# DataCTE/SDXL-Training-Improvements

Hardware: AMD Instinct MI355X
Metric: images/sec/node SDXL-base 1024^2 bf16 fwd+bwd (higher is better)
Workload: dtype bf16; 1 GPU; method=ddpm v_prediction + zero_terminal_snr + MinSNR(5), SDXL-base UNet fwd+bwd, batch 4/GPU, 1024^2 (latent 128x128); global_batch=4, parallelism=dp1, weights=synthetic (counter-hash init of the 2,567,463,684-parameter SDXL-base UNet)

## Files before the change

include/sdxlstep_diag.h:

```cpp
#ifndef SDXLSTEP_DIAG_H
#define SDXLSTEP_DIAG_H
#include "sdxlstep.h"
#ifdef __cplusplus
extern "C" {
#endif

SDXL_API int sdxl_probe_layout(void* out_dev, void* stream);
SDXL_API int sdxl_set_gemm_mode(int mode);
SDXL_API int sdxl_debug_act_checksums(sdxl_handle* h, unsigned long long* out_host, int cap, int* n_out, int grads);

SDXL_API int sdxl_op_exchange_shadow(void* buf, size_t bytes, int workgroups, int lds_bytes, float busy_us, void* stream);

SDXL_API int sdxl_op_gemm_ld(int form, const void* A, const void* B, void* C, int M, int N, int K, long lda, long ldb, long ldc, const void* bias,
                    const void* resid, long ldr, int cfg, void* stream);
SDXL_API int sdxl_op_linear_dgrad_delta(const void* dy, const void* w, const void* o, const void* addend, void* d_o, float* delta, int B, int Nq,
                               int N, int K, void* stream);

SDXL_API int sdxl_op_sampler_step(float* x, const void* pred, void* x_in, int B, int H, int W, const sdxl_sampler_step* s, void* stream);

SDXL_API int sdxl_op_cond_dgrad(int n, const void* const* A, const long* lda, const void* const* W, const long* ldb, const int* K, float* C,
                       long ldc, int M, int N, void* stream);

SDXL_API int sdxl_debug_cond_operands(sdxl_handle* h, int which, int g, int* n_groups, size_t* a_ws_byte_off, long* lda, size_t* w_elem_off,
                             long* ldb, int* K);

SDXL_API int sdxl_op_lora_merge(const void* base, const void* A, const void* B, void* w, int out, int in, int rank, float scale, void* stream);
SDXL_API int sdxl_op_lora_project(const float* dw, const void* A, const void* B, float* dA, float* dB, int out, int in, int rank, float scale,
                         void* stream);
SDXL_API int sdxl_op_lora_merge_layout(const void* base, const void* A, const void* B, void* w, int out, int in, int rank, float scale, int kind,
                              int cg, int native_rows, void* stream);
SDXL_API int sdxl_op_lora_project_layout(const float* dw, const void* A, const void* B, float* dA, float* dB, int out, int in, int rank,
                                float scale, int kind, int cg, int native_rows, void* stream);
SDXL_API int sdxl_op_lora_grad(const void* x, long ldx, const void* dy, long ldy, const void* A, const void* B, float* dA, float* dB, int M, int out,
                               int in, int rank, float scale, int accumulate, void* stream);

typedef struct sdxl_gemm_desc {
  int form, taps, M, N, K, splitk, group, cfg, geglu, geglu_group, Hm, Wm, Hs, Ws, sm, sd, up2, emit_bf16, delta, bias_grad;
} sdxl_gemm_desc;
typedef struct sdxl_gemm_route { int kernel, cfg, fast, post; } sdxl_gemm_route;
SDXL_API int sdxl_debug_gemm_route(const sdxl_gemm_desc* problem, sdxl_gemm_route* out);

SDXL_API int sdxl_op_linear_dgrad_ln_bwd(const void* dy, const void* w, const void* x, const float* stats, const void* gamma, const void* addend,
                                void* dx, void* dy_out, float* pcol, int M, int N, int K, void* stream);

SDXL_API int sdxl_set_knob(int id, int value);
SDXL_API int sdxl_set_sk_mode(int mode, int workers);
SDXL_API int sdxl_sk_error(void* stream, unsigned* out);
SDXL_API int sdxl_ln_error(unsigned* out);
SDXL_API int sdxl_op_pl_prefetch_b(int form, const void* B, int M, int N, int K, long ldb, int parts, void* stream);
SDXL_API int sdxl_op_gemm_sk(int n, const int* form, const void* const* A, const void* const* B, void* const* C, const int* M,
                    const int* N, const int* K, const void* const* bias, const void* const* resid, const int* accumulate,
                    void* stream);
SDXL_API int sdxl_op_conv3x3_s2_fwd(const void* x, const void* w, const void* bias, void* xplanar, void* y, int B, int H, int W, int Cin,
                           int Cout, void* stream);
SDXL_API int sdxl_op_conv3x3_s2_wgrad(const void* dy, const void* xplanar, float* dw, float* dbias, int accumulate, int B, int H, int W, int Cin,
                             int Cout, int splitk, void* stream);

#ifdef __cplusplus
}
#endif
#endif
```

sdxl-training-improvements_amd/csrc/attention.hip:

```cpp
#include "attn_tiles.h"

#include <type_traits>

#if defined(ATTN_DIAG) && (ATTN_DIAG & 256)
__device__ unsigned long long g_attn_wg[4096 * 3];
extern "C" __attribute__((visibility("default"))) int sdxl_debug_attn_wg(unsigned long long* out) {
  if (hipDeviceSynchronize() != hipSuccess) return 2;
  return hipMemcpyFromSymbol(out, HIP_SYMBOL(g_attn_wg), sizeof(unsigned long long) * 4096 * 3) == hipSuccess ? 0 : 2;
}
#endif
#if defined(ATTN_DIAG) && (ATTN_DIAG & 128)
__device__ unsigned long long g_attn_stamps[4 * 4 * 6];
extern "C" __attribute__((visibility("default"))) int sdxl_debug_attn_stamps(unsigned long long* out) {
  if (hipDeviceSynchronize() != hipSuccess) return 2;
  return hipMemcpyFromSymbol(out, HIP_SYMBOL(g_attn_stamps), sizeof(unsigned long long) * 96) == hipSuccess ? 0 : 2;
}
#endif
__global__ __launch_bounds__(256, 3) void attn_fwd_kernel(const AttnP p) {
#if defined(ATTN_DIAG) && (ATTN_DIAG & 256)
  const unsigned long long wg_t0 = __builtin_amdgcn_s_memrealtime();
#endif
  __shared__ __attribute__((aligned(16))) bf16 sm[4 * TILE_ELEMS];
  const int tid = threadIdx.x, lane = tid & 63, wave = __builtin_amdgcn_readfirstlane(tid >> 6), l16 = lane & 15, g = lane >> 4;
  int qblk, bh;
// ... 159 lines not shown
    else tile(nfull, std::true_type{}, std::true_type{});
  }
  {
    const bool bad = !(lrow[0] < 1e30f) || !(lrow[1] < 1e30f);
    if (__syncthreads_or(bad ? 1 : 0)) {
#pragma unroll
      for (int i = 0; i < 4; ++i)
#pragma unroll
        for (int j = 0; j < 2; ++j) ot[i][j] = (f32x4){0.f, 0.f, 0.f, 0.f};
      mrow[0] = mrow[1] = 0.f;
      lrow[0] = lrow[1] = 0.f;
      buf = 0;
      tile_dma(ksrc, 0, p.Nk, sm, wave);
      tile_dma(vsrc, 0, p.Nk, sm + TILE_ELEMS, wave);
      for (int t = 0; t < nfull; ++t) tile(t, std::false_type{}, std::false_type{});
      if (nfull < ntiles) tile(nfull, std::true_type{}, std::false_type{});
    }
  }
#if defined(ATTN_DIAG) && (ATTN_DIAG & 128)
  acc_ph[4] = __builtin_amdgcn_s_memrealtime() - rt0;
  if (lane == 0 && qblk < 4 && bh == 5)
    for (int i = 0; i < 6; ++i) g_attn_stamps[(qblk * 4 + wave) * 6 + i] = acc_ph[i];
#endif
#pragma unroll
  for (int qb = 0; qb < 2; ++qb) {
    float l = sum_over_g(lrow[qb]);
    float inv = 1.f / l;
    int q = q0 + qb * 16 + l16;
    if (q < p.Nq) {
      bf16* orow = p.O + ((long)b * p.Nq + q) * p.ldo + h * HD;
#pragma unroll
      for (int db = 0; db < 4; ++db) {
        bf16x4 o;
        o[0] = (bf16)(ot[db][qb][0] * inv); o[1] = (bf16)(ot[db][qb][1] * inv);
        o[2] = (bf16)(ot[db][qb][2] * inv); o[3] = (bf16)(ot[db][qb][3] * inv);
        *(bf16x4*)(orow + db * 16 + g * 4) = o;
      }
      if (g == 0 && p.LSE) p.LSE[(long)bh * p.Nq + q] = mrow[qb] * (1.f / LOG2E) + logf(l);
    }
  }
#if defined(ATTN_DIAG) && (ATTN_DIAG & 256)
  if (threadIdx.x == 0) {
    const int id = blockIdx.x;
    if (id < 4096) {
      unsigned hwid, xcc;
      asm volatile("s_getreg_b32 %0, hwreg(HW_REG_HW_ID)" : "=s"(hwid));
      asm volatile("s_getreg_b32 %0, hwreg(HW_REG_XCC_ID)" : "=s"(xcc));
      g_attn_wg[id * 3] = wg_t0; g_attn_wg[id * 3 + 1] = __builtin_amdgcn_s_memrealtime(); g_attn_wg[id * 3 + 2] = ((unsigned long long)xcc << 32) | hwid;
    }
  }
#endif
}

template <bool WRITE_DELTA>
__device__ __forceinline__ void attn_bwd_dq_body(const AttnP& p, bf16* sm, const int bx, const int bh) {
  const int tid = threadIdx.x, lane = tid & 63, wave = __builtin_amdgcn_readfirstlane(tid >> 6), l16 = lane & 15, g = lane >> 4;
  const int b = bh / p.H, h = bh - b * p.H;
  const int q0 = bx * 128 + wave * 32;
  const bf16* Qb = p.Q + (long)b * p.Nq * p.ldq + h * HD;
  const bf16* dOb = p.dO + (long)b * p.Nq * p.lddo + h * HD;
  const bf16* Ob = p.O + (long)b * p.Nq * p.ldo + h * HD;
  const bf16* Kb = p.K + (long)b * p.Nk * p.ldk + h * HD;
  const bf16* Vb = p.V + (long)b * p.Nk * p.ldv + h * HD;

  bf16x8 qf[2][2], df[2][2];
  float lse2[2], delta[2];
#pragma unroll
  for (int qb = 0; qb < 2; ++qb) {
    int q = q0 + qb * 16 + l16;
    bool ok = q < p.Nq;
    float dl = 0.f;
#pragma unroll
    for (int ks = 0; ks < 2; ++ks) {
      qf[qb][ks] = ok ? *(const bf16x8*)(Qb + (long)q * p.ldq + ks * 32 + g * 8) : z8();
      df[qb][ks] = ok ? *(const bf16x8*)(dOb + (long)q * p.lddo + ks * 32 + g * 8) : z8();
      bf16x8 of = ok ? *(const bf16x8*)(Ob + (long)q * p.ldo + ks * 32 + g * 8) : z8();
#pragma unroll
      for (int e = 0; e < 8; ++e) dl += (float)df[qb][ks][e] * (float)of[e];
    }
    dl = sum_over_g(dl);
    lse2[qb] = ok ? p.LSE[(long)bh * p.Nq + q] * LOG2E : 0.f;
    delta[qb] = dl;
    if (WRITE_DELTA && ok && g == 0) p.Delta[(long)bh * p.Nq + q] = dl;
  }
  f32x4 dq[4][2];
#pragma unroll
  for (int i = 0; i < 4; ++i)
#pragma unroll
    for (int j = 0; j < 2; ++j) dq[i][j] = (f32x4){0.f, 0.f, 0.f, 0.f};
  const float c = SCALE * LOG2E;
#pragma unroll
  for (int qb = 0; qb < 2; ++qb) { qf[qb][0] = scale8(qf[qb][0], c); qf[qb][1] = scale8(qf[qb][1], c); }

  const int ntiles = (p.Nk + 63) / 64;
  const TileSrc ksrc = tile_src(Kb, p.ldk, wave, lane), vsrc = tile_src(Vb, p.ldv, wave, lane);
  tile_dma(ksrc, 0, p.Nk, sm, wave);
  tile_dma(vsrc, 0, p.Nk, sm + TILE_ELEMS, wave);
#pragma unroll
  for (int qb = 0; qb < 2; ++qb) { landed(qf[qb][0]); landed(qf[qb][1]); landed(df[qb][0]); landed(df[qb][1]); landed(lse2[qb]); landed(delta[qb]); }
  int buf = 0;
  auto tile = [&](int t, auto MASKC) {
    constexpr bool MASK = decltype(MASKC)::value;
    asm volatile("s_waitcnt vmcnt(0)" ::: "memory");
    __syncthreads();
    if (t + 1 < ntiles) {
      tile_dma(ksrc, t + 1, p.Nk, sm + ((buf ^ 1) * 2) * TILE_ELEMS, wave);
      tile_dma(vsrc, t + 1, p.Nk, sm + ((buf ^ 1) * 2 + 1) * TILE_ELEMS, wave);
    }
    const bf16* Kt = sm + (buf * 2) * TILE_ELEMS;
    const bf16* Vt = Kt + TILE_ELEMS;
    bf16x8 kf[4][2], vf[4][2];
#pragma unroll
    for (int kb = 0; kb < 4; ++kb) {
      kf[kb][0] = ld_frag(Kt, kb * 16 + l16, g * 8); kf[kb][1] = ld_frag(Kt, kb * 16 + l16, 32 + g * 8);
      vf[kb][0] = ld_frag(Vt, kb * 16 + l16, g * 8); vf[kb][1] = ld_frag(Vt, kb * 16 + l16, 32 + g * 8);
    }
    f32x4 st[4][2], dp[4][2];
#pragma unroll
    for (int kb = 0; kb < 4; ++kb)
#pragma unroll
      for (int qb = 0; qb < 2; ++qb) {
        f32x4 a = (f32x4){-lse2[qb], -lse2[qb], -lse2[qb], -lse2[qb]};
        a = __builtin_amdgcn_mfma_f32_16x16x32_bf16(kf[kb][0], qf[qb][0], a, 0, 0, 0);
        a = __builtin_amdgcn_mfma_f32_16x16x32_bf16(kf[kb][1], qf[qb][1], a, 0, 0, 0);
        st[kb][qb] = a;
        f32x4 d = (f32x4){-delta[qb], -delta[qb], -delta[qb], -delta[qb]};
        d = __builtin_amdgcn_mfma_f32_16x16x32_bf16(vf[kb][0], df[qb][0], d, 0, 0, 0);
        d = __builtin_amdgcn_mfma_f32_16x16x32_bf16(vf[kb][1], df[qb][1], d, 0, 0, 0);
        dp[kb][qb] = d;
      }
    bf16x8 ktr[4][2];
#pragma unroll
    for (int db = 0; db < 4; ++db)
#pragma unroll
      for (int t2 = 0; t2 < 2; ++t2) ktr[db][t2] = tr_frag(Kt, t2, db * 16, l16, g);
    __builtin_amdgcn_sched_barrier(0);
    bf16x8 dsf[2][2];
#pragma unroll
    for (int qb = 0; qb < 2; ++qb) {
#pragma unroll
      for (int kb = 0; kb < 4; ++kb)
#pragma unroll
        for (int hh = 0; hh < 2; ++hh) {
          const f32x2 arg = (f32x2){st[kb][qb][2 * hh], st[kb][qb][2 * hh + 1]};
          f32x2 pr = (f32x2){__builtin_amdgcn_exp2f(arg[0]), __builtin_amdgcn_exp2f(arg[1])};
          if (MASK) {
            if (t * 64 + kb * 16 + g * 4 + 2 * hh >= p.Nk) pr[0] = 0.f;
            if (t * 64 + kb * 16 + g * 4 + 2 * hh + 1 >= p.Nk) pr[1] = 0.f;
          }
          const f32x2 ds = pr * (f32x2){dp[kb][qb][2 * hh], dp[kb][qb][2 * hh + 1]};
          st[kb][qb][2 * hh] = ds[0]; st[kb][qb][2 * hh + 1] = ds[1];
        }
      dsf[0][qb] = pack8(st[0][qb], st[1][qb]);
      dsf[1][qb] = pack8(st[2][qb], st[3][qb]);
    }
    __builtin_amdgcn_sched_barrier(0);
#pragma unroll
    for (int db = 0; db < 4; ++db)
#pragma unroll
      for (int t2 = 0; t2 < 2; ++t2)
#pragma unroll
        for (int qb = 0; qb < 2; ++qb)
          dq[db][qb] = __builtin_amdgcn_mfma_f32_16x16x32_bf16(ktr[db][t2], dsf[t2][qb], dq[db][qb], 0, 0, 0);
    buf ^= 1;
  };
  const int nfull = p.Nk / 64;
  for (int t = 0; t < nfull; ++t) tile(t, std::false_type{});
  if (nfull < ntiles) tile(nfull, std::true_type{});
#pragma unroll
  for (int qb = 0; qb < 2; ++qb) {
    int q = q0 + qb * 16 + l16;
    if (q < p.Nq) {
      bf16* row = p.dQ + ((long)b * p.Nq + q) * p.lddq + h * HD;
#pragma unroll
      for (int db = 0; db < 4; ++db) {
        bf16x4 o;
        o[0] = (bf16)(dq[db][qb][0] * SCALE); o[1] = (bf16)(dq[db][qb][1] * SCALE);
        o[2] = (bf16)(dq[db][qb][2] * SCALE); o[3] = (bf16)(dq[db][qb][3] * SCALE);
        *(bf16x4*)(row + db * 16 + g * 4) = o;
      }
    }
  }
}

__global__ __launch_bounds__(256, 2) void attn_bwd_dq_kernel(const AttnP p) {
  set_wave_prio(p.prio);
  __shared__ __attribute__((aligned(16))) bf16 sm[4 * TILE_ELEMS];
  int qblk, bh;
  attn_xcd_map(p, blockIdx.x, (p.Nq + 127) >> 7, qblk, bh);
  attn_bwd_dq_body<true>(p, sm, qblk, bh);
}

template <int KB>
__device__ __forceinline__ void attn_bwd_dkv_body(const AttnP& p, bf16* sm, const int bx, const int bh, const int bz, const int nbh) {
  float (*sstat)[2][64] = (float (*)[2][64])(sm + 4 * TILE_ELEMS);
  const int tid = threadIdx.x, lane = tid & 63, wave = __builtin_amdgcn_readfirstlane(tid >> 6), l16 = lane & 15, g = lane >> 4;
  const int b = bh / p.H, h = bh - b * p.H;
  const int key0 = bx * (64 * KB) + wave * (16 * KB) + l16;
  const bf16* Qb = p.Q + (long)b * p.Nq * p.ldq + h * HD;
  const bf16* dOb = p.dO + (long)b * p.Nq * p.lddo + h * HD;
  const bf16* Kb = p.K + (long)b * p.Nk * p.ldk + h * HD;
  const bf16* Vb = p.V + (long)b * p.Nk * p.ldv + h * HD;
  bool kok[KB];
  bf16x8 kf[KB][2], vf[KB][2];
#pragma unroll
  for (int kb = 0; kb < KB; ++kb) {
    const int key = key0 + kb * 16;
    kok[kb] = key < p.Nk;
#pragma unroll
    for (int ks = 0; ks < 2; ++ks) {
      kf[kb][ks] = kok[kb] ? scale8(*(const bf16x8*)(Kb + (long)key * p.ldk + ks * 32 + g * 8), SCALE * LOG2E) : z8();
      vf[kb][ks] = kok[kb] ? *(const bf16x8*)(Vb + (long)key * p.ldv + ks * 32 + g * 8) : z8();
    }
  }
  f32x4 dk[KB][4], dv[KB][4];
#pragma unroll
  for (int kb = 0; kb < KB; ++kb)
#pragma unroll
    for (int i = 0; i < 4; ++i) { dk[kb][i] = (f32x4){0.f, 0.f, 0.f, 0.f}; dv[kb][i] = (f32x4){0.f, 0.f, 0.f, 0.f}; }

  const int ntiles_all = (p.Nq + 63) / 64;
  const int per = (ntiles_all + p.qsplit - 1) / p.qsplit;
  const int t_begin = bz * per;
  const int ntiles = min(ntiles_all, t_begin + per);
  auto load_stats = [&](int t, int bufi) {
    if (wave < 2) {
      const int q = t * 64 + lane;
      const float* src = (wave == 0 ? p.LSE : p.Delta) + (long)bh * p.Nq + q;
      lds_dma4_global(q < p.Nq ? (const void*)src : (const void*)g_attn_zero16, lds_addr_of(&sstat[bufi][wave][0]));
    }
  };
  const TileSrc qsrc = tile_src(Qb, p.ldq, wave, lane), dsrc = tile_src(dOb, p.lddo, wave, lane);
  tile_dma(qsrc, t_begin, p.Nq, sm, wave);
  tile_dma(dsrc, t_begin, p.Nq, sm + TILE_ELEMS, wave);
  load_stats(t_begin, 0);
#pragma unroll
  for (int kb = 0; kb < KB; ++kb) { landed(kf[kb][0]); landed(kf[kb][1]); landed(vf[kb][0]); landed(vf[kb][1]); }
  int buf = 0;
  auto tile = [&](int t, auto MASKC) {
    constexpr bool MASK = decltype(MASKC)::value;
    const bool more = t + 1 < ntiles;
    asm volatile("s_waitcnt vmcnt(0)" ::: "memory");
    __syncthreads();
// ... 188 lines not shown
  o[0] = (bf16)a[0]; o[1] = (bf16)a[1]; o[2] = (bf16)a[2]; o[3] = (bf16)a[3];
  bf16* dst = which == 0 ? p.dK + ((long)b * p.Nk + key) * p.lddk + h * HD : p.dV + ((long)b * p.Nk + key) * p.lddv + h * HD;
  *(bf16x4*)(dst + v4 * 4) = o;
}

size_t attn_part_floats(int B, int H, int Nk, int qsplit) {
  return qsplit > 1 ? (size_t)qsplit * B * H * ((Nk + 63) / 64) * 64 * 2 * 64 : 0;
}
int attn_pick_qsplit(int B, int H, int Nq, int Nk) {
  long blocks = (long)((Nk + 63) / 64) * B * H;
  int qt = (Nq + 63) / 64;
  int s = (int)((KNOB(36) > 0 ? KNOB(36) : 160) / blocks);
  if (s < 1) s = 1;
  if (s > qt / 2) s = qt / 2 > 0 ? qt / 2 : 1;
  if (s > 16) s = 16;
  return s;
}

static int check_attn(const AttnP& p) {
  ARG_CHECK(p.B > 0 && p.H > 0 && p.Nq > 0 && p.Nk > 0, "attention: empty problem");
  ARG_CHECK(p.ldq % 8 == 0 && p.ldk % 8 == 0 && p.ldv % 8 == 0 && p.ldo % 4 == 0,
            "attention: row strides must be multiples of 8 elements");
  return 0;
}

int launch_attn_fwd(const AttnP& p, hipStream_t st) {
  if (int e = check_attn(p)) return e;
#ifdef SDXL_DIAG
  if (KNOB(33) == 2 && attn_fwd_pl_applicable(p)) return launch_attn_fwd_pl(p, st);
#endif
  return launch_attn_fwd_tiled(p, st);
}
int launch_attn_fwd_tiled(const AttnP& p, hipStream_t st) {
  if (int e = check_attn(p)) return e;
  if (FILE* f = launch_log()) { fprintf(f, "A,0,%d,%d,%d,%d\n", p.B, p.H, p.Nq, p.Nk); fflush(f); }
  AttnP q = p;
  q.xcd = (p.B * p.H) % 8 == 0 && KNOB(32) != 1;
  hipLaunchKernelGGL(attn_fwd_kernel, dim3(cdiv(p.Nq, 128) * p.B * p.H), dim3(256), 0, st, q);
  HIP_CHECK_RET(hipGetLastError());
  return 0;
}

static int check_attn_bwd(const AttnP& p) {
  if (int e = check_attn(p)) return e;
  ARG_CHECK(p.O && p.dO && p.dQ && p.dK && p.dV && p.LSE && p.Delta, "attention bwd: missing buffers");
  ARG_CHECK(!p.accumulate, "attention bwd: accumulate not implemented");
  return 0;
}
int launch_attn_bwd_dq(const AttnP& p, hipStream_t st) {
  if (int e = check_attn_bwd(p)) return e;
  if (FILE* f = launch_log()) { fprintf(f, "A,1,%d,%d,%d,%d\n", p.B, p.H, p.Nq, p.Nk); fflush(f); }
  AttnP q = p;
  q.xcd = (p.B * p.H) % 8 == 0 && KNOB(32) != 1;
  hipLaunchKernelGGL(attn_bwd_dq_kernel, dim3(cdiv(p.Nq, 128) * p.B * p.H), dim3(256), 0, st, q);
  HIP_CHECK_RET(hipGetLastError());
  return 0;
}
int launch_attn_bwd_dkv(const AttnP& p, hipStream_t st) {
  if (int e = check_attn_bwd(p)) return e;
  if (FILE* f = launch_log()) { fprintf(f, "A,2,%d,%d,%d,%d\n", p.B, p.H, p.Nq, p.Nk); fflush(f); }
  AttnP q = p;
  if (q.qsplit < 1 || !q.part) q.qsplit = 1;
  if (q.qsplit == 1 && (long)cdiv(p.Nk, 128) * p.B * p.H >= 1024)
    hipLaunchKernelGGL(attn_bwd_dkv_kernel<2>, dim3(cdiv(p.Nk, 128), p.B * p.H, 1), dim3(256), 0, st, q);
  else
    hipLaunchKernelGGL(attn_bwd_dkv_kernel<1>, dim3(cdiv(p.Nk, 64), p.B * p.H, q.qsplit), dim3(256), 0, st, q);
  if (q.qsplit > 1) {
    long total = (long)p.B * p.H * p.Nk * 32;
    hipLaunchKernelGGL(attn_dkv_reduce_kernel, dim3(cdiv(total, 256)), dim3(256), 0, st, q);
  }
  HIP_CHECK_RET(hipGetLastError());
  return 0;
}
int launch_attn_bwd_fused(const AttnP& p, hipStream_t st) {
  if (int e = check_attn_bwd(p)) return e;
  ARG_CHECK(p.lddo % 8 == 0 && p.ldo % 8 == 0, "attention bwd (fused): dO / O row strides must be multiples of 8 elements");
  if (FILE* f = launch_log()) { fprintf(f, "A,1,%d,%d,%d,%d\nA,2,%d,%d,%d,%d\n", p.B, p.H, p.Nq, p.Nk, p.B, p.H, p.Nq, p.Nk); fflush(f); }
  AttnP q = p;
  q.qsplit = 1;
  q.xcd = (p.B * p.H) % 8 == 0 && KNOB(32) != 1;
  const long total = (long)p.B * p.Nq * p.H;
  if (!p.delta_ready) hipLaunchKernelGGL(attn_delta_kernel, dim3(cdiv(total, 32)), dim3(256), 0, st, q);
  if (KNOB(35) != 1 && ((p.Nq >= 2048 && p.Nk >= 2048) || KNOB(35) == 2) && attn_bwd_pl_applicable(q)) return launch_attn_bwd_pl(q, st);
  const int nkb = cdiv(p.Nk, 128), nqb = cdiv(p.Nq, 128), nbh = p.B * p.H;
  hipLaunchKernelGGL(attn_bwd_fused_kernel<2>, dim3(nkb * nbh + nqb * nbh), dim3(256), 0, st, q, nkb * nbh, nkb, nqb);
  HIP_CHECK_RET(hipGetLastError());
  return 0;
}
int launch_attn_bwd(const AttnP& p, hipStream_t st) {
  const bool fused = (KNOB(20) != 1 || p.delta_ready) && (p.qsplit <= 1 || !p.part) && p.Nk >= 256 && p.lddo % 8 == 0 && p.ldo % 8 == 0;
  if (fused) return launch_attn_bwd_fused(p, st);
  if (int e = launch_attn_bwd_dq(p, st)) return e;
  return launch_attn_bwd_dkv(p, st);
}
```

sdxl-training-improvements_amd/csrc/capi.hip:

```cpp
#include "capi.h"
#include <functional>

extern "C" {

const char* sdxl_last_error(void) { return sdxl_get_error(); }
int sdxl_version(void) { return 1; }

int sdxl_default_config(sdxl_unet_config* c) {
  ARG_CHECK(c, "null config");
  c->in_channels = 4; c->out_channels = 4;
  c->block_out_channels[0] = 320; c->block_out_channels[1] = 640; c->block_out_channels[2] = 1280;
  c->layers_per_block = 2;
  c->transformer_layers[0] = 0; c->transformer_layers[1] = 2; c->transformer_layers[2] = 10;
  c->head_dim = 64; c->cross_attention_dim = 2048; c->norm_num_groups = 32;
  c->addition_time_embed_dim = 256; c->pooled_dim = 1280;
  c->resnet_eps = 1e-5f; c->tf_gn_eps = 1e-6f; c->ln_eps = 1e-5f;
  return 0;
}

int sdxl_create(const sdxl_unet_config* cfg, int device, sdxl_handle** out) {
  ARG_CHECK(cfg && out, "null argument");
  ARG_CHECK(cfg->head_dim == 64, "head_dim must be 64 (got %d)", cfg->head_dim);
  ARG_CHECK(cfg->in_channels == 4 && cfg->out_channels == 4, "in/out channels must be 4");
  ARG_CHECK(cfg->transformer_layers[0] == 0, "level 0 must not have attention");
  for (int i = 0; i < 3; ++i) {
    int c = cfg->block_out_channels[i];
    ARG_CHECK(c % cfg->norm_num_groups == 0 && c % 8 == 0, "block_out_channels[%d]=%d unsupported", i, c);
    if (cfg->transformer_layers[i] > 0) ARG_CHECK(c % 128 == 0, "attention level width %d must be a multiple of 128", c);
  }
  ARG_CHECK(cfg->cross_attention_dim % 8 == 0 && cfg->pooled_dim % 8 == 0 && cfg->addition_time_embed_dim % 8 == 0,
            "conditioning widths must be multiples of 8");
  int ndev = 0;
  HIP_CHECK_RET(hipGetDeviceCount(&ndev));
  ARG_CHECK(device >= 0 && device < ndev, "device %d out of range (have %d)", device, ndev);
  HIP_CHECK_RET(hipSetDevice(device));
  sdxl_handle* h = new sdxl_handle();
  h->e.cfg = *cfg;
  h->e.device = device;
  h->e.build(nullptr);
  const char* ns = getenv("SDXL_NO_SIDE_STREAM");
  h->e.use_side = !(ns && ns[0] == '1');
  if (h->e.use_side) {
    if (const char* sp = getenv("SDXL_SIDE_PRIO")) {
      HIP_CHECK_RET(hipStreamCreateWithPriority(&h->e.side, hipStreamNonBlocking, atoi(sp)));
    } else
    HIP_CHECK_RET(hipStreamCreateWithFlags(&h->e.side, hipStreamNonBlocking));
    HIP_CHECK_RET(hipStreamCreateWithFlags(&h->e.gstream, hipStreamNonBlocking));
    HIP_CHECK_RET(hipEventCreateWithFlags(&h->e.ev_gin, hipEventDisableTiming));
    HIP_CHECK_RET(hipEventCreateWithFlags(&h->e.ev_gout, hipEventDisableTiming));
    HIP_CHECK_RET(hipEventCreateWithFlags(&h->e.ev_join, hipEventDisableTiming | hipEventDisableSystemFence));
    HIP_CHECK_RET(hipEventCreateWithFlags(&h->e.ev_seg, hipEventDisableTiming | hipEventDisableSystemFence));
    HIP_CHECK_RET(hipEventCreateWithFlags(&h->e.ev_hoist, hipEventDisableTiming | hipEventDisableSystemFence));
  }
  *out = h;
  return 0;
}

int sdxl_destroy(sdxl_handle* h) {
  if (!h) return 0;
  if (h->e.own_weights && h->e.weights) (void)hipFree(h->e.weights);
  if (h->e.own_grads && h->e.grads) (void)hipFree(h->e.grads);
  if (h->e.own_ws && h->e.ws) (void)hipFree(h->e.ws);
  h->e.clear_graphs();
  if (h->e.gstream) (void)hipStreamDestroy(h->e.gstream);
  if (h->e.ev_gin) (void)hipEventDestroy(h->e.ev_gin);
  if (h->e.ev_gout) (void)hipEventDestroy(h->e.ev_gout);
  for (hipEvent_t ev : h->e.ev_pool) (void)hipEventDestroy(ev);
  if (h->e.ev_join) (void)hipEventDestroy(h->e.ev_join);
  if (h->e.ev_seg) (void)hipEventDestroy(h->e.ev_seg);
  if (h->e.ev_hoist) (void)hipEventDestroy(h->e.ev_hoist);
  if (h->e.side) (void)hipStreamDestroy(h->e.side);
  if (h->e.small_ranges_dev) (void)hipFree(h->e.small_ranges_dev);
  if (h->lora.dev) (void)hipFree(h->lora.dev);
  if (h->e.lora.dev) (void)hipFree(h->e.lora.dev);
  delete h;
  return 0;
}

int sdxl_param_bytes(sdxl_handle* h, size_t* wb, size_t* gb) {
  H_CHECK(h);
  if (wb) *wb = h->e.param_elems * sizeof(bf16);
  if (gb) *gb = h->e.param_elems * sizeof(float);
  return 0;
}

int sdxl_bind_params(sdxl_handle* h, void* w, void* g) {
  H_CHECK(h);
  Engine& e = h->e;
  e.clear_graphs();
  if (w) { e.weights = (bf16*)w; e.own_weights = false; }
  else {
    HIP_CHECK_RET(hipMalloc((void**)&e.weights, e.param_elems * sizeof(bf16)));
    HIP_CHECK_RET(hipMemset(e.weights, 0, e.param_elems * sizeof(bf16)));
    e.own_weights = true;
  }
  if (g) { e.grads = (float*)g; e.own_grads = false; }
  else {
    HIP_CHECK_RET(hipMalloc((void**)&e.grads, e.param_elems * sizeof(float)));
    HIP_CHECK_RET(hipMemset(e.grads, 0, e.param_elems * sizeof(float)));
    e.own_grads = true;
  }
  ARG_CHECK(((uintptr_t)e.weights & 255) == 0 && ((uintptr_t)e.grads & 255) == 0, "arenas must be 256-byte aligned");
  return 0;
}

int sdxl_num_params(sdxl_handle* h) { return h ? (int)h->e.src.size() : -1; }

int sdxl_param_info(sdxl_handle* h, int i, char* name, int cap, int* ndim, long shape[4]) {
  H_CHECK(h);
  ARG_CHECK(i >= 0 && i < (int)h->e.src.size(), "parameter index %d out of range", i);
  const SrcParam& s = h->e.src[i];
  if (name && cap > 0) snprintf(name, cap, "%s", s.name.c_str());
  if (ndim) *ndim = s.ndim;
  if (shape) for (int k = 0; k < 4; ++k) shape[k] = s.shape[k];
  return 0;
}

int sdxl_param_range(sdxl_handle* h, int i, size_t* elem_off, size_t* elems) {
  H_CHECK(h);
  ARG_CHECK(i >= 0 && i < (int)h->e.src.size(), "parameter index %d out of range", i);
  const SrcParam& s = h->e.src[i];
  size_t n = 1;
  for (int k = 0; k < s.ndim; ++k) n *= (size_t)s.shape[k];
// ... 455 lines not shown
    CHK(launch_loss_prepare(L, s));
    CHK(run_forward_ops(e, s));
    CHK(launch_loss_fwd(L, s));
    return 0;
  }));
  if (b->per_sample_loss)
    HIP_CHECK_RET(hipMemcpyAsync(b->per_sample_loss, p.F(p.ps_loss_off), sizeof(float) * p.B, hipMemcpyDeviceToDevice, st));
  h->step.lc = full; h->step.b = sb; h->step.valid = true;
  h->step.d_ehs = d_ehs; h->step.d_pool = d_pool;
  h->step.awaiting_bwd = true;
  return 0;
}

int sdxl_num_segments(sdxl_handle* h) { return h ? h->e.nseg : -1; }
int sdxl_set_join_mode(sdxl_handle* h, int mode) {
  H_CHECK(h);
  ARG_CHECK(mode >= 0 && mode <= 2, "join mode %d (0, 1, 2)", mode);
  h->e.join_last_only = mode != 0;
  h->e.seg_on_side = mode == 2 && h->e.use_side && h->e.side;
  return 0;
}
int sdxl_side_stream(sdxl_handle* h, void** stream) {
  H_CHECK(h);
  ARG_CHECK(stream, "null output");
  *stream = h->e.use_side ? (void*)h->e.side : nullptr;
  return 0;
}

int sdxl_segment_range(sdxl_handle* h, int k, size_t* off, size_t* n) {
  H_CHECK(h);
  ARG_CHECK(k >= 0 && k < h->e.nseg, "segment %d out of range", k);
  int s = h->e.nseg - 1 - k;
  if (off) *off = h->e.seg_begin[s];
  if (n) *n = h->e.seg_end[s] - h->e.seg_begin[s];
  return 0;
}

static int run_backward_segment_body(Engine& e, int k, bool first, hipStream_t st);
static int run_backward_segment(Engine& e, int k, bool first, hipStream_t st) {
  if (k == 0) e.drop_pending();
  const int rc = run_backward_segment_body(e, k, first, st);
  if (rc) e.drop_pending();
  return rc;
}
static int run_backward_segment_body(Engine& e, int k, bool first, hipStream_t st) {
  Plan& p = *e.cur;
  int s = e.nseg - 1 - k;
  e.ev_used = 0;
  if (k == 0 && p.tp32_off != NONE) HIP_CHECK_RET(hipMemsetAsync(p.F(p.tp32_off), 0, p.tp32_bytes, st));
  if (k == 0 && p.ln_part_floats) {
    HIP_CHECK_RET(hipMemsetAsync(p.F(p.ln_part_off), 0, p.ln_part_floats * sizeof(float), st));
    p.ln_epoch = 0;
  }
  for (int i = p.seg_last_op[s]; i >= p.seg_first_op[s] && i >= 0; --i) CHK(p.ops[i]->bwd(p, st, first));
  CHK(e.flush_wgrads(p, st));
  CHK(e.flush_ln_params(p, st));
  ARG_CHECK(k != e.nseg - 1 || e.cs_pending.empty(), "backward: %zu per-sample column sums were never reduced", e.cs_pending.size());
  if (e.seg_on_side && !gemm_profiling()) {
    HIP_CHECK_RET(hipEventRecord(e.ev_seg, st));
    HIP_CHECK_RET(hipStreamWaitEvent(e.side, e.ev_seg, 0));
    e.side_dirty = true;
  }
  if (e.side_dirty && !(e.join_last_only && k != e.nseg - 1)) {
    HIP_CHECK_RET(hipEventRecord(e.ev_join, e.side));
    HIP_CHECK_RET(hipStreamWaitEvent(st, e.ev_join, 0));
    e.side_dirty = false;
  }
  if (k == e.nseg - 1 && (e.cond_ehs || e.cond_pool)) CHK(e.launch_cond_grads(p, st));
  return 0;
}

int sdxl_backward_segment(sdxl_handle* h, int k, float grad_scale, int first_micro, void* stp) {
  H_CHECK(h);
  Engine& e = h->e;
  hipStream_t st = (hipStream_t)stp;
  CHK(ready(e));
  ARG_CHECK(k >= 0 && k < e.nseg, "segment %d out of range", k);
  if (k == 0) ARG_CHECK(h->step.valid, "sdxl_backward_segment(0) needs a preceding sdxl_forward_loss");
  set_cond_request(h, true);
  auto body = [&](hipStream_t s) -> int {
    if (k == 0) {
      LossP L;
      fill_loss(e, &h->step.lc, &h->step.b, grad_scale, L);
      CHK(launch_loss_bwd(L, s));
    }
    return run_backward_segment(e, k, first_micro != 0, s);
  };
  if (e.join_last_only) {
    CHK(body(st));
  } else {
    unsigned sbits;
    memcpy(&sbits, &grad_scale, 4);
    Engine::GraphKey key{e.cur, 1, k, first_micro != 0, 0, sbits, loss_cfg_bits(h->step.lc, h->step.b.tag_weights != nullptr),
                        loss_cfg_bits2(h->step.lc, h->step.b) | cond_bits(h->step), loss_huber_bits(h->step.lc, h->step.b)};
    CHK(run_graphed(e, key, st, body));
  }
  if (k == e.nseg - 1) h->step.awaiting_bwd = false;
  return k == e.nseg - 1 ? copy_cond_grads(h, st) : 0;
}

int sdxl_backward_all(sdxl_handle* h, float grad_scale, int first_micro, void* stp) {
  H_CHECK(h);
  Engine& e = h->e;
  hipStream_t st = (hipStream_t)stp;
  CHK(ready(e));
  ARG_CHECK(h->step.valid, "sdxl_backward_all needs a preceding sdxl_forward_loss");
// ... 220 lines not shown
```

sdxl-training-improvements_amd/csrc/engine.h:

```cpp
#pragma once
#include <functional>
#include <map>
#include <memory>
#include <set>
#include <string>
#include <tuple>
#include <vector>

#include "../../include/sdxlstep.h"
#include "kernels.h"

static const size_t NONE = (size_t)-1;

struct Act {
  size_t off = NONE;
  size_t goff = NONE;
  long rows = 0;
  int cols = 0;
  int pad_rows = 0;
  bool need_grad = true;
  Act* parent = nullptr;
  int col0 = 0;
  long ld() const { return parent ? parent->cols : cols; }
};

struct PRef {
  size_t off = NONE;
  size_t numel = 0;
};

struct SrcParam {
  std::string name;
  int ndim;
  long shape[4];
  PRef native;
  int kind;
  size_t elem_off;
  int ci_pad;
};

struct Engine;
struct Plan;

struct Op {
  int seg = 0;
  bool hoist_fwd = false;
  bool needs_hoisted = false;
  virtual ~Op() {}
  virtual int fwd(Plan& p, hipStream_t st) = 0;
  virtual void plan_bwd(Plan& p) = 0;
  virtual int bwd(Plan& p, hipStream_t st, bool first_micro) = 0;
};

struct Plan {
  Engine* eng = nullptr;
  int B = 0, H = 0, W = 0, ctx = 0;
  size_t ws_bytes = 0;
  size_t cursor = 0;
  std::vector<std::unique_ptr<Act>> acts;
  std::vector<std::unique_ptr<Op>> ops;
  std::vector<int> seg_first_op, seg_last_op;
  size_t tp32_off = NONE, tp32_bytes = 0;
  Act *x_in = nullptr, *pred = nullptr, *ehs = nullptr, *aug_in = nullptr, *te_sin = nullptr, *tid_emb = nullptr;
  size_t t_off = NONE, tid_off = NONE, loss_off = NONE, loss_part_off = NONE;
  size_t in_lat_off = NONE, in_noise_off = NONE, in_sig_off = NONE, in_tag_off = NONE;
  size_t in_sw_off = NONE, in_hc_off = NONE;
  size_t ps_loss_off = NONE;
  size_t in_mask_off = NONE, in_nin_off = NONE;
  size_t mask_norm_off = NONE;
  size_t samp_part_off = NONE;
  size_t gn_ws_off = NONE, gn_ws_floats = 0;
  size_t slab_off = NONE, slab_floats = 0;
  size_t slab_main_off = NONE, slab_main_floats = 0;
  size_t apart_off = NONE, apart_floats = 0;
  size_t apart_side_off = NONE, apart_side_floats = 0;
  size_t ln_part_off = NONE, ln_part_floats = 0;
  int ln_epoch = 0;
  struct CondSrc { size_t dy_off = NONE; long lda = 0; PRef w; long ldb = 0; int K = 0; };
  CondSrc cond_kv[2], cond_add;
  int cond_nkv = 0;
  size_t dehs_off = NONE, dpool_off = NONE, cond_slab_off = NONE;
  size_t lg_tu_elems = 0, lg_part_floats = 0, lg_tu_off = NONE, lg_part_off = NONE;

  Act* new_act(long rows, int cols, bool need_grad = true, int pad_rows = 0);
  Act* view(Act* parent, int col0, int cols);
  size_t alloc(size_t bytes);
  struct GradDst { size_t out = NONE, addend = NONE; };
  GradDst grad_dst(Act* a);
  bool grad_alias(Act* x, Act* y);
  bf16* GP(size_t off) const;
  template <class T, class... A>
  T* add(A&&... a);
  bf16* P(const Act* a) const;
  bf16* G(const Act* a) const;
  float* F(size_t off) const;
};

struct Engine {
  sdxl_unet_config cfg;
  int device = 0;
  std::vector<PRef> natives;
  std::vector<SrcParam> src;
  std::map<std::string, int> src_index;
  size_t param_elems = 0;
  bf16* weights = nullptr;
  float* grads = nullptr;
  bool own_weights = false, own_grads = false;
  int nseg = 1;
  std::vector<size_t> seg_begin, seg_end;
  std::map<std::tuple<int, int, int, int>, std::unique_ptr<Plan>> plans;
  Plan* cur = nullptr;
  char* ws = nullptr;
  size_t ws_cap = 0;
  bool own_ws = false;
  hipStream_t side = nullptr;
  hipEvent_t ev_join = nullptr, ev_hoist = nullptr;
  std::vector<hipEvent_t> ev_pool;
  size_t ev_used = 0;
  bool use_side = true;
  bf16* emit_base = nullptr;
  float emit_scale = 1.f;
  bool join_last_only = false;
  bool seg_on_side = false;
  hipEvent_t ev_seg = nullptr;
  hipEvent_t next_event();
  std::vector<std::vector<GemmP>> wg_pending;
  int defer_wgrad(Plan& p, hipStream_t main, const GemmP& g, int grp);
  int flush_wgrads(Plan& p, hipStream_t main);
  std::vector<std::function<int(hipStream_t)>> side_leaves;
  std::vector<LnRedEntry> ln_pending;
  std::vector<LnRedEntry> cs_pending;
  int flush_ln_params(Plan& p, hipStream_t main);
  void drop_pending() { side_leaves.clear(); wg_pending.clear(); ln_pending.clear(); cs_pending.clear(); }
  bool side_dirty = false;
  bool cond_ehs = false, cond_pool = false;
  bool cond_gated = false;
  int launch_cond_grads(Plan& p, hipStream_t st);
  struct LoraOpSel { std::vector<LoraGradTarget> host; const LoraGradTarget* dev = nullptr; int tiles = 0, reds = 0; size_t part_unit = 0; };
  struct LoraSel {
    std::vector<int> params;
    int rank = 0; float scale = 0.f;
    const bf16* adapters = nullptr; float* grads = nullptr;
    std::map<size_t, LoraOpSel> ops;
    LoraGradTarget* dev = nullptr;
  } lora;
  const LoraOpSel* lora_op(PRef w) const {
    if (lora.ops.empty()) return nullptr;
    auto it = lora.ops.find(w.off);
    return it == lora.ops.end() ? nullptr : &it->second;
  }
  std::vector<unsigned char> trainable;
  std::set<size_t> frozen_offs;
  void set_trainable(const unsigned char* flags);
  bool frozen(PRef a, PRef b) const {
    if (frozen_offs.empty()) return false;
    return (a.off == NONE || frozen_offs.count(a.off)) && (b.off == NONE || frozen_offs.count(b.off));
  }
  bool use_graphs = false;
  hipStream_t gstream = nullptr;
  hipEvent_t ev_gin = nullptr, ev_gout = nullptr;
  struct GraphKey {
    const void* plan; int kind, k, first, join; unsigned scale_bits, cfg;
    unsigned cfg2, huber_bits;
    bool operator<(const GraphKey& o) const {
      return std::tie(plan, kind, k, first, join, scale_bits, cfg, cfg2, huber_bits) <
             std::tie(o.plan, o.kind, o.k, o.first, o.join, o.scale_bits, o.cfg, o.cfg2, o.huber_bits);
    }
  };
  struct GraphEntry { hipGraphExec_t exec = nullptr; int seen = 0; };
  std::map<GraphKey, GraphEntry> graphs;
  void clear_graphs() {
    for (auto& kv : graphs) if (kv.second.exec) (void)hipGraphExecDestroy(kv.second.exec);
    graphs.clear();
  }
  bool registering = true;
  size_t native_cursor = 0;
  Plan* bp = nullptr;

  PRef param(size_t numel, bool small = false);
  std::vector<std::pair<size_t, size_t>> small_ranges;
  unsigned long long* small_ranges_dev = nullptr;
  void map_src(const std::string& name, std::vector<long> shape, PRef p, int kind, size_t elem_off, int ci_pad);
  int seg_of(size_t elem_off) const;
  void build(Plan* plan);
  bf16* Wp(PRef p) const { return weights + p.off; }
// ... 18 lines not shown
```

sdxl-training-improvements_amd/csrc/engine.hip:

```cpp
#include "engine.h"

#include <stdarg.h>
#include <stdlib.h>

#ifdef SDXL_DIAG
int g_knobs[SDXL_NKNOBS] = {0};
#endif
static thread_local char g_err[1024] = "";
void sdxl_set_error(const char* fmt, ...) {
  va_list ap;
  va_start(ap, fmt);
  vsnprintf(g_err, sizeof(g_err), fmt, ap);
  va_end(ap);
}
const char* sdxl_get_error() { return g_err; }

#define CHK(x)            \
  do {                    \
    int _r = (x);         \
    if (_r) return _r;    \
  } while (0)

static inline size_t align_up(size_t v, size_t a) { return (v + a - 1) / a * a; }

// ... 56 lines not shown
  HIP_CHECK_RET(hipStreamWaitEvent(e.side, ev, 0));
  e.side_dirty = true;
  if (!e.side_leaves.empty()) {
    std::vector<std::function<int(hipStream_t)>> v;
    v.swap(e.side_leaves);
    for (auto& leaf : v) CHK(leaf(e.side));
  }
  return fn(e.side);
}
template <class F>
static int side_leaf(Plan& p, hipStream_t main, F&& fn) {
  Engine& e = *p.eng;
  if (!e.use_side || !e.side || gemm_profiling() || KNOB(2) == 16) return on_side(p, main, fn);
  e.side_leaves.emplace_back(std::function<int(hipStream_t)>(fn));
  return 0;
}
static int launch_wgrad_bucket(Plan& p, hipStream_t main, std::vector<GemmP>& v) {
  if (v.empty()) return 0;
  GemmP g = v[0];
  if (v.size() > 1) {
    g.splitk = 1;
    gemm_fill_group(g, v.data(), (int)v.size());
  }
  v.clear();
  if (g.splitk > 1) g.anyorder = 0;
  return on_side(p, main, [&g](hipStream_t s2) -> int { return launch_gemm(g, s2); });
}
int Engine::defer_wgrad(Plan& p, hipStream_t main, const GemmP& g, int grp) {
  for (auto& b : wg_pending) {
    if (b.empty() || (b[0].M == g.M && b[0].N == g.N && b[0].K == g.K && b[0].accumulate == g.accumulate)) {
      b.push_back(g);
      if ((int)b.size() >= grp) return launch_wgrad_bucket(p, main, b);
      return 0;
    }
  }
  wg_pending.emplace_back(1, g);
  if (grp <= 1) return launch_wgrad_bucket(p, main, wg_pending.back());
  return 0;
}
int Engine::flush_wgrads(Plan& p, hipStream_t main) {
  if (!side_leaves.empty()) CHK(on_side(p, main, [](hipStream_t) -> int { return 0; }));
  for (auto& b : wg_pending) CHK(launch_wgrad_bucket(p, main, b));
  return 0;
}
int Engine::flush_ln_params(Plan& p, hipStream_t main) {
  size_t i = 0;
  while (i < ln_pending.size()) {
    LnRedBatch b;
    b.n = 0;
    while (i < ln_pending.size() && b.n < LN_RED_MAX) b.e[b.n++] = ln_pending[i++];
    CHK(on_side(p, main, [&b](hipStream_t s2) -> int { return launch_ln_param_reduce(b, s2); }));
  }
  ln_pending.clear();
  return 0;
}
int Engine::launch_cond_grads(Plan& p, hipStream_t st) {
  const float* gate = cond_gated ? p.F(p.loss_off) + 7 : nullptr;
  if (cond_ehs) {
    const int M = p.B * p.ctx, N = cfg.cross_attention_dim;
    if (p.cond_nkv == 0) {
      HIP_CHECK_RET(hipMemsetAsync(p.F(p.dehs_off), 0, sizeof(float) * (size_t)M * N, st));
    } else {
      CondDgradP q;
      memset(&q, 0, sizeof(q));
      q.n = p.cond_nkv;
      for (int g = 0; g < q.n; ++g) {
        const Plan::CondSrc& cs = p.cond_kv[g];
        ARG_CHECK(cs.dy_off != NONE, "conditioning gradients: the K | V projection has no output gradient");
        q.A[g] = p.GP(cs.dy_off); q.lda[g] = cs.lda; q.W[g] = Wp(cs.w); q.ldb[g] = cs.ldb; q.K[g] = cs.K;
      }
      q.C = p.F(p.dehs_off); q.ldc = N; q.M = M; q.N = N; q.slab = p.F(p.cond_slab_off); q.gate = gate;
      CHK(launch_cond_dgrad(q, st));
    }
  }
  if (cond_pool) {
    const Plan::CondSrc& cs = p.cond_add;
    ARG_CHECK(cs.dy_off != NONE, "conditioning gradients: add_embedding.linear_1 has no output gradient");
    CondDgradP q;
    memset(&q, 0, sizeof(q));
    q.n = 1;
    q.A[0] = p.GP(cs.dy_off); q.lda[0] = cs.lda; q.W[0] = Wp(cs.w); q.ldb[0] = cs.ldb; q.K[0] = cs.K;
    q.C = p.F(p.dpool_off); q.ldc = cfg.pooled_dim; q.M = p.B; q.N = cfg.pooled_dim; q.slab = p.F(p.cond_slab_off); q.gate = gate;
    CHK(launch_cond_dgrad(q, st));
  }
  return 0;
}
bool Plan::grad_alias(Act* x, Act* y) {
  if (x->goff == NONE) {
    x->goff = y->goff;
    return true;
  }
  return false;
}

static void want_slab_main(Plan& p, int M, int N, int splitk) {
  size_t need = gemm_slab_floats(M, N, 1, splitk);
  if (need > p.slab_main_floats) p.slab_main_floats = need;
}
static void want_slab(Plan& p, int M, int N, int taps, int splitk) {
  size_t need = gemm_slab_floats(M, N, taps, splitk);
  if (need > p.slab_floats) p.slab_floats = need;
}

struct WgradDst {
  float *C, *bias_grad;
  int accumulate;
  bf16* Cb;
  float cb_scale;
  void to(GemmP& g) const {
    g.C = C; g.bias_grad = bias_grad; g.accumulate = accumulate;
    if (Cb) { g.Cb = Cb; g.cb_scale = cb_scale; }
  }
};
static WgradDst wgrad_dst(Plan& p, PRef w, PRef b, bool first) {
  const Engine& e = *p.eng;
  return {e.Gp(w), b.off != NONE ? e.Gp(b) : nullptr, first ? 0 : 1, e.emit_base ? e.emit_base + w.off : nullptr, e.emit_scale};
}

static int kv_pad_rows(int B, int ctx) { return (int)((64 - ((long)B * ctx) % 64) % 64); }

struct AttnOp;
static void attn_delta_target(AttnOp* a, Plan& p, GemmP& g);
static bool attn_delta_wanted(const AttnOp* a);
static void attn_set_delta_fused(AttnOp* a, bool on);
struct LayerNormOp;
static bool ln_fuse_plan(LayerNormOp* ln, Plan& p, int mode);
static void ln_fuse_target(LayerNormOp* ln, Plan& p, GemmP& g, int mode);
struct LinearOp : Op {
  Act *x, *y, *resid;
  PRef w, b;
  int K, N;
  int resid_alias = 0, splitk = 1, wgroup = 1;
  struct AttnOp* delta_attn = nullptr;
  bool delta_on = false;
  struct LayerNormOp* ln_src = nullptr;
  int ln_mode = 0;
  int crcfg = 0, crsplit = 1;
  int fsplit = 1, dsplit = 1;
  size_t dy32_off = NONE;
  size_t dy_off = NONE;
  Plan::GradDst dx, dres;
  int ggroup = 64;
  Act* gact = nullptr;
  Act* gu = nullptr;
  LinearOp(Act* x_, Act* y_, PRef w_, PRef b_, int K_, int N_, Act* resid_) : x(x_), y(y_), resid(resid_), w(w_), b(b_), K(K_), N(N_) {}
  int fwd(Plan& p, hipStream_t st) override {
    GemmP g = linear_fwd_problem(p.P(x), x->ld(), p.eng->Wp(w), p.P(y), y->ld(), (int)x->rows, N, K, b.off == NONE ? nullptr : p.eng->Wp(b),
                                 resid ? p.P(resid) : nullptr, resid ? resid->ld() : 0);
    if (gact) gemm_attach_geglu_fwd(g, ggroup, p.P(gact), gact->ld());
    if (fsplit > 1 && !hoist_fwd) { g.splitk = fsplit; g.slab = p.F(p.slab_main_off); }
    return launch_gemm(g, st);
  }
  void plan_bwd(Plan& p) override {
    dy_off = y->goff;
    if (resid) {
      resid_alias = p.grad_alias(resid, y) ? 1 : 0;
      if (!resid_alias) dres = p.grad_dst(resid);
    }
    if (gu) dx = p.grad_dst(gu);
    else if (x->need_grad) dx = p.grad_dst(x);
    splitk = linear_wgrad_splitk(N, K, x->rows);
    wgroup = gemm_pick_group(N, K, 1, x->rows, splitk);
    want_slab(p, N, K, 1, splitk);
    crcfg = cr256_wgrad_cfg(N, K, x->rows, b.off != NONE);
    if (crcfg) { crsplit = cr256_pick_splitk(N, K, x->rows, crcfg); want_slab(p, N, K, 1, crsplit); }
    if (!gact) { fsplit = gemm_pick_splitk_small((int)x->rows, N, K, 3); want_slab_main(p, (int)x->rows, N, fsplit); }
    if (const Engine::LoraOpSel* lo = p.eng->lora_op(w)) {
      const size_t tu = lora_grad_tu_elems((int)lo->host.size(), p.eng->lora.rank, (int)x->rows);
      const size_t pf = (size_t)lora_grad_chunks((int)x->rows) * lo->part_unit;
      if (tu > p.lg_tu_elems) p.lg_tu_elems = tu;
      if (pf > p.lg_part_floats) p.lg_part_floats = pf;
    }
    if (delta_attn && !(!gu && x->need_grad)) attn_set_delta_fused(delta_attn, false);
    if (!gu && x->need_grad) {
      dsplit = gemm_pick_splitk_small((int)x->rows, K, N, 2);
      if (KNOB(3) > 1 && N >= (KNOB(4) > 0 ? KNOB(4) : 8192) && N % (64 * KNOB(3)) == 0 && dsplit == 1) dsplit = KNOB(3);
      want_slab_main(p, (int)x->rows, K, dsplit);
      if (delta_attn) {
        delta_on = attn_delta_wanted(delta_attn) && dsplit <= 1 && K % 128 == 0;
        attn_set_delta_fused(delta_attn, delta_on);
      }
      if (SDXL_LN_EPILOGUE && ln_src && KNOB(26) != 0 && dsplit == 1 && dx.addend == NONE && !x->parent && gemm_ln_cfg((int)x->rows, K, N) &&
          ln_fuse_plan(ln_src, p, KNOB(26) == 2 ? 2 : 1))
        ln_mode = KNOB(26) == 2 ? 2 : 1;
    }
  }
  int bwd(Plan& p, hipStream_t st, bool first) override {
    const bf16* dy = p.GP(dy_off);
    const int M = (int)x->rows;
    if (dy32_off != NONE) {
      auto& cs = p.eng->cs_pending;
      for (size_t i = 0; i < cs.size();) {
        LnRedBatch rb;
        rb.n = 0;
        while (i < cs.size() && rb.n < LN_RED_MAX) rb.e[rb.n++] = cs[i++];
        CHK(launch_ln_param_reduce(rb, st));
      }
      cs.clear();
      CHK(launch_f32_to_bf16(p.F(dy32_off), p.GP(dy_off), (long)M * N, 1.f, st));
    }
    if (gu && dx.addend != NONE) { sdxl_set_error("geglu: pre-activation gradient has another writer"); return 3; }
    if (resid && !resid_alias) CHK(launch_add(p.GP(dres.addend), dy, p.GP(dres.out), (long)M * N, st));
    if (const Engine::LoraOpSel* lo = p.eng->lora_op(w)) {
      const Engine::LoraSel& L = p.eng->lora;
      LoraGradP q;
      memset(&q, 0, sizeof(q));
      q.table = lo->dev; q.n = (int)lo->host.size(); q.rank = L.rank; q.scale = L.scale; q.accumulate = first ? 0 : 1;
      q.x = p.P(x); q.ldx = x->ld(); q.dy = dy; q.ldy = y->ld();
      q.M = M; q.Mp = lora_grad_mp(M); q.nchunk = lora_grad_chunks(M); q.tiles = lo->tiles; q.reds = lo->reds;
      q.xvec = ((uintptr_t)q.x % 16 == 0 && q.ldx % 8 == 0) ? 1 : 0;
      q.yvec = ((uintptr_t)q.dy % 16 == 0 && q.ldy % 8 == 0) ? 1 : 0;
      q.a = q.b = L.adapters; q.ga = q.gb = L.grads;
      if (p.lg_tu_off == NONE || p.lg_part_off == NONE) { sdxl_set_error("lora: the plan was built without adapter-gradient scratch"); return 3; }
      q.tu = (bf16*)p.F(p.lg_tu_off); q.part = p.F(p.lg_part_off);
      CHK(on_side(p, st, [&q](hipStream_t s2) -> int { return launch_lora_grad(q, s2); }));
    } else
    if (!p.eng->frozen(w, b)) {
      GemmP g = linear_wgrad_problem(dy, y->ld(), p.P(x), x->ld(), nullptr, N, K, M, nullptr);
      wgrad_dst(p, w, b, first).to(g);
      g.splitk = splitk;
      g.slab = p.F(p.slab_off);
      if (crcfg) { g.cfg = crcfg; if (wgroup <= 1) g.splitk = crsplit; }
      if (KNOB(29) == 1 && M >= 1024 && dy32_off == NONE && (g.splitk <= 1 || wgroup > 1)) g.anyorder = 1;
      const int pad = x->pad_rows < y->pad_rows ? x->pad_rows : y->pad_rows;
      if (pad > 0 && (M + pad) % 64 == 0) {
        g.K = M + pad;
        g.anyorder = 0;
        bf16* dyp = p.GP(dy_off) + (size_t)M * N;
        bf16* xp = p.P(x) + (size_t)M * K;
        const size_t nb_dy = (size_t)pad * N * sizeof(bf16), nb_x = (size_t)pad * K * sizeof(bf16);
        CHK(on_side(p, st, [=](hipStream_t s2) -> int {
          HIP_CHECK_RET(hipMemsetAsync(dyp, 0, nb_dy, s2));
          HIP_CHECK_RET(hipMemsetAsync(xp, 0, nb_x, s2));
          return launch_gemm(g, s2);
        }));
      } else
      if (wgroup > 1) CHK(p.eng->defer_wgrad(p, st, g, wgroup));
      else CHK(on_side(p, st, [&](hipStream_t s2) -> int { return launch_gemm(g, s2); }));
    }
    if (x->need_grad) {
      GemmP g = linear_dgrad_problem(dy, y->ld(), p.eng->Wp(w), p.GP(dx.out), x->ld(), M, K, N, !gu && dx.addend != NONE ? p.GP(dx.addend) : nullptr, x->ld());
      if (gu) gemm_attach_geglu_bwd(g, ggroup, p.P(gu), gu->ld());
      if (dsplit > 1) { g.splitk = dsplit; g.slab = p.F(p.slab_main_off); }
      g.prio = KNOB(0);
      if (KNOB(6) > 0 && !gu && (KNOB(8) <= 0 || N >= KNOB(8))) g.cfg = KNOB(6);
      if (KNOB(22) > 0 && gu) g.cfg = KNOB(22);
      if (delta_on) attn_delta_target(delta_attn, p, g);
      if (ln_mode) ln_fuse_target(ln_src, p, g, ln_mode);
      CHK(launch_gemm(g, st));
    }
    return 0;
  }
};

struct ConvOp : Op {
  Act *x, *y, *resid, *rowvec;
  PRef w, b;
  int Bn, H, W, Cin, Cout, stride, Ho, Wo;
  int resid_alias = 0, splitk = 1;
  int fsplit = 1, dsplit = 1;
  size_t rv32_off = NONE;
  long rv32_ld = 0;
  size_t cs_part_off = NONE;
  size_t dy_off = NONE;
  Plan::GradDst dx, dres, drv;
  Act* x_low = nullptr;
  Plan::GradDst* up_dx = nullptr;
  size_t weff_off = NONE, planar_off = NONE, dweff_off = NONE;
  size_t s2x_off = NONE;
  size_t s2_planar_off = NONE;
  int up_fs = 1, up_ds = 1, up_ws = 1;
  bool up_wg = false;
  bool up2() const { return x_low != nullptr && KNOB(2) != 64; }
  void enable_up2(Plan& p, Act* xl, Plan::GradDst* udx) {
    if (stride != 1 || Cin % 64 || Cout % 64 || resid || rowvec) return;
    x_low = xl; up_dx = udx;
    const long plane = upconv_plane_rows(Bn, H / 2, W / 2);
    weff_off = p.alloc(sizeof(bf16) * (size_t)Cout * 16 * Cin);
    planar_off = p.alloc(sizeof(bf16) * (size_t)4 * plane * (Cout > Cin ? Cout : Cin));
    up_fs = upconv3x3_fwd_splitk(Bn, H / 2, W / 2, Cin, Cout);
    want_slab_main(p, (int)(4 * plane), Cout, up_fs);
    up_ds = upconv3x3_dgrad_splitk(Bn, H / 2, W / 2, Cin, Cout);
    want_slab_main(p, Bn * (H / 2) * (W / 2), Cin, up_ds);
    up_wg = (Bn * (H / 2) * (W / 2)) % 64 == 0;
    if (up_wg) {
      dweff_off = p.alloc(sizeof(float) * (size_t)Cout * 16 * Cin);
      up_ws = gemm_pick_splitk(Cout, Cin, 16, (long)Bn * (H / 2) * (W / 2));
      want_slab(p, Cout, Cin, 16, up_ws);
      cs_part_off = p.alloc(sizeof(float) * colsum_part_floats(1, Bn * H * W, Cout));
    }
  }
  ConvOp(Act* x_, Act* y_, PRef w_, PRef b_, int B_, int H_, int W_, int Cin_, int Cout_, int stride_, Act* resid_,
         Act* rowvec_)
      : x(x_), y(y_), resid(resid_), rowvec(rowvec_), w(w_), b(b_), Bn(B_), H(H_), W(W_), Cin(Cin_), Cout(Cout_),
        stride(stride_) {
    Ho = (H - 1) / stride + 1;
    Wo = (W - 1) / stride + 1;
  }
  int fwd(Plan& p, hipStream_t st) override {
#ifdef SDXL_DIAG
    if (s2x_off != NONE && KNOB(2) == 512)
// ... 85 lines not shown
      GemmP g = conv3x3_dgrad_problem(Bn, H, W, Cin, Cout, stride);
      g.A = dy; g.B = p.eng->Wp(w); g.C = p.GP(dx.out);
      if (dx.addend != NONE) { g.resid = p.GP(dx.addend); g.ldr = Cin; }
      if (dsplit > 1) { g.splitk = dsplit; g.slab = p.F(p.slab_main_off); }
      g.prio = KNOB(0);
      if (KNOB(7) > 0) g.cfg = KNOB(7);
      CHK(launch_gemm(g, st));
    }
    return 0;
  }
};

struct GroupNormOp : Op {
  Act *x, *y;
  PRef gm, bt;
  int Bn, HW, C, G, silu;
  float eps;
  size_t stats_off, prow_off;
  size_t dy_off = NONE;
  Plan::GradDst dx;
  GroupNormOp(Plan& p, Act* x_, Act* y_, PRef g_, PRef b_, int B_, int HW_, int C_, int G_, float eps_, int silu_)
      : x(x_), y(y_), gm(g_), bt(b_), Bn(B_), HW(HW_), C(C_), G(G_), silu(silu_), eps(eps_) {
    stats_off = p.alloc(sizeof(float) * Bn * G * 2);
    prow_off = p.alloc(sizeof(float) * Bn * 2 * C);
    size_t need = groupnorm_ws_floats(Bn, C, G);
    if (need > p.gn_ws_floats) p.gn_ws_floats = need;
  }
  int fwd(Plan& p, hipStream_t st) override {
    if (KNOB(27) & 2) return 0;
    if (KNOB(27) & 128) return launch_silu_fwd(p.P(x), p.P(y), (long)Bn * HW * C, st);
    return launch_groupnorm_fwd(p.P(x), p.P(y), p.eng->Wp(gm), p.eng->Wp(bt), p.F(stats_off), p.F(p.gn_ws_off), Bn, HW, C, G,
                                eps, silu, st);
  }
  void plan_bwd(Plan& p) override { dy_off = y->goff; dx = p.grad_dst(x); }
  int bwd(Plan& p, hipStream_t st, bool) override {
    if (KNOB(27) & 1) return 0;
    LnRedEntry r;
    r.part = p.F(prow_off); r.dgamma = p.eng->Gp(gm); r.dbeta = p.eng->Gp(bt); r.C = C; r.nblk = Bn;
    if (!p.eng->frozen(gm, bt)) p.eng->ln_pending.push_back(r);
    return launch_groupnorm_bwd(p.P(x), p.GP(dy_off), p.eng->Wp(gm), p.eng->Wp(bt), p.F(stats_off), p.GP(dx.out),
                                p.GP(dx.addend), p.eng->Gp(gm), p.eng->Gp(bt), p.F(p.gn_ws_off), Bn, HW, C, G, silu, st, p.F(prow_off));
  }
};

struct LayerNormOp : Op {
  Act *x, *y;
  PRef gm, bt;
  int C;
  float eps;
  size_t stats_off, part_off = NONE;
  size_t dy_off = NONE;
  Plan::GradDst dx;
  int fused = 0;
  LayerNormOp(Plan& p, Act* x_, Act* y_, PRef g_, PRef b_, int C_, float eps_) : x(x_), y(y_), gm(g_), bt(b_), C(C_), eps(eps_) {
    stats_off = p.alloc(sizeof(float) * x->rows * 2);
  }
  int fwd(Plan& p, hipStream_t st) override {
    if (KNOB(27) & 4) return 0;
    if (KNOB(27) & 256) return launch_silu_fwd(p.P(x), p.P(y), (long)x->rows * C, st);
    return launch_layernorm_fwd(p.P(x), p.P(y), p.eng->Wp(gm), p.eng->Wp(bt), p.F(stats_off), (int)x->rows, C, eps, st);
  }
  void plan_bwd(Plan& p) override {
    dy_off = y->goff;
    dx = p.grad_dst(x);
    part_off = p.alloc(sizeof(float) * layernorm_bwd_part_floats((int)x->rows, C));
  }
  int bwd(Plan& p, hipStream_t st, bool) override {
    const bool frozen = p.eng->frozen(gm, bt);
    if (fused) {
      if (frozen) return 0;
      if (fused == 2) {
        const bf16* xp = p.P(x); const bf16* dyp = p.GP(dy_off); const float* sp = p.F(stats_off);
        float* dg = p.eng->Gp(gm); float* db = p.eng->Gp(bt); const int Mr = (int)x->rows, Cc = C;
        return side_leaf(p, st, [=](hipStream_t s2) -> int { return launch_layernorm_param_grads(xp, dyp, sp, dg, db, Mr, Cc, s2); });
      }
      LnRedEntry r;
      r.part = p.F(part_off); r.dgamma = p.eng->Gp(gm); r.dbeta = p.eng->Gp(bt); r.C = C; r.nblk = gemm_ln_rowblocks((int)x->rows);
      p.eng->ln_pending.push_back(r);
      return 0;
    }
    if (KNOB(25) == 2) return 0;
    if (KNOB(10) == 1 || KNOB(10) == 3) {
      if (KNOB(25) != 3)
      CHK(launch_layernorm_bwd(p.P(x), p.GP(dy_off), p.eng->Wp(gm), p.F(stats_off), p.GP(dx.out), p.GP(dx.addend), nullptr, nullptr, (int)x->rows, C, st));
      const bf16* xp = p.P(x); const bf16* dyp = p.GP(dy_off); const float* sp = p.F(stats_off);
      const int Mr = (int)x->rows, Cc = C;
      if (KNOB(25) == 1 || frozen) return 0;
      if (KNOB(10) == 3) {
        float* dg = p.eng->Gp(gm); float* db = p.eng->Gp(bt);
        return side_leaf(p, st, [=](hipStream_t s2) -> int { return launch_layernorm_param_grads(xp, dyp, sp, dg, db, Mr, Cc, s2); });
      }
      float* part = p.F(part_off);
      LnRedEntry r;
      r.part = part; r.dgamma = p.eng->Gp(gm); r.dbeta = p.eng->Gp(bt); r.C = C; r.nblk = layernorm_param_partial_rows(Mr, Cc);
      p.eng->ln_pending.push_back(r);
      return side_leaf(p, st, [=](hipStream_t s2) -> int { return launch_layernorm_param_partials(xp, dyp, sp, part, Mr, Cc, s2); });
    }
    LnRedEntry r;
    r.part = p.F(part_off); r.dgamma = p.eng->Gp(gm); r.dbeta = p.eng->Gp(bt); r.C = C;
    CHK(launch_layernorm_bwd(p.P(x), p.GP(dy_off), p.eng->Wp(gm), p.F(stats_off), p.GP(dx.out), p.GP(dx.addend),
                             p.F(part_off), &r.nblk, (int)x->rows, C, st));
    if (!frozen) p.eng->ln_pending.push_back(r);
    return 0;
  }
};

static bool ln_fuse_plan(LayerNormOp* ln, Plan& p, int mode) {
  const int M = (int)ln->x->rows, C = ln->C;
  if (ln->x->ld() != C || ln->y->ld() != C) return false;
  if (gemm_ln_pcol_floats(M, C) > layernorm_bwd_part_floats(M, C)) return false;
  ln->fused = mode;
  const size_t pf = gemm_ln_part_floats(M, C);
  if (pf > p.ln_part_floats) p.ln_part_floats = pf;
  return true;
}
static void ln_fuse_target(LayerNormOp* ln, Plan& p, GemmP& g, int mode) {
  gemm_attach_ln_bwd(g, p.P(ln->x), ln->x->ld(), p.F(ln->stats_off), p.eng->Wp(ln->gm), p.GP(ln->dx.out), p.GP(ln->dx.addend), p.F(p.ln_part_off),
                     ++p.ln_epoch, mode == 1 ? p.F(ln->part_off) : nullptr);
  if (mode == 1) g.C = nullptr;
}

struct AttnOp : Op {
  Act *q, *kv, *o;
  int Bn, heads, Nq, Nk, C;
  bool self;
  int qsplit = 1;
  size_t lse_off, delta_off;
  AttnOp(Plan& p, Act* q_, Act* kv_, Act* o_, int B_, int heads_, int Nq_, int Nk_, int C_, bool self_)
      : q(q_), kv(kv_), o(o_), Bn(B_), heads(heads_), Nq(Nq_), Nk(Nk_), C(C_), self(self_) {
    lse_off = p.alloc(sizeof(float) * (size_t)Bn * heads * Nq);
    delta_off = p.alloc(sizeof(float) * (size_t)Bn * heads * Nq);
    qsplit = attn_pick_qsplit(Bn, heads, Nq, Nk);
    size_t need = attn_part_floats(Bn, heads, Nk, qsplit);
    if (self) { if (need > p.apart_floats) p.apart_floats = need; }
    else if (need > p.apart_side_floats) p.apart_side_floats = need;
  }
  void fill(Plan& p, AttnP& a, bool grads) {
    memset(&a, 0, sizeof(a));
    a.B = Bn; a.H = heads; a.Nq = Nq; a.Nk = Nk;
    if (self) {
      a.Q = p.P(q); a.K = p.P(q) + C; a.V = p.P(q) + 2 * C;
      a.ldq = a.ldk = a.ldv = 3L * C;
    } else {
      a.Q = p.P(q); a.ldq = C;
      a.K = p.P(kv); a.V = p.P(kv) + C; a.ldk = a.ldv = kv->ld();
    }
    a.O = p.P(o); a.ldo = o->ld();
    a.LSE = p.F(lse_off);
    if (grads) {
      a.dO = p.GP(do_off); a.lddo = o->ld();
      a.Delta = p.F(delta_off);
      a.qsplit = qsplit;
      a.part = p.F(self ? p.apart_off : p.apart_side_off);
      if (self) {
        a.dQ = p.GP(dq.out); a.dK = a.dQ + C; a.dV = a.dQ + 2 * C;
        a.lddq = a.lddk = a.lddv = 3L * C;
      } else {
        a.dQ = p.GP(dq.out); a.lddq = C;
        a.dK = p.GP(dkv.out); a.dV = a.dK + C; a.lddk = a.lddv = kv->ld();
      }
    }
  }
  int fwd(Plan& p, hipStream_t st) override {
    if (KNOB(27) & (self ? 32 : 64)) return 0;
    AttnP a;
    fill(p, a, false);
    return launch_attn_fwd(a, st);
  }
  bool bad = false;
  size_t do_off = NONE;
  Plan::GradDst dq, dkv;
  void plan_bwd(Plan& p) override {
    do_off = o->goff;
    dq = p.grad_dst(q);
    if (dq.addend != NONE) bad = true;
    if (!self) { dkv = p.grad_dst(kv); if (dkv.addend != NONE) bad = true; }
  }
  bool delta_fused = false;
  int bwd(Plan& p, hipStream_t st, bool) override {
    if (bad) { sdxl_set_error("attention: operand gradient has another writer"); return 3; }
    if (KNOB(27) & (self ? 16 : 8)) return 0;
    AttnP a;
    fill(p, a, true);
    a.prio = KNOB(1);
    a.delta_ready = delta_fused ? 1 : 0;
    if (self) return launch_attn_bwd(a, st);
    CHK(launch_attn_bwd_dq(a, st));
    return side_leaf(p, st, [=](hipStream_t s2) -> int { return launch_attn_bwd_dkv(a, s2); });
  }
};

static bool attn_delta_wanted(const AttnOp* a) { return a->self && a->qsplit <= 1 && a->Nk >= 256 && a->C % 128 == 0 && a->delta_fused; }
static void attn_set_delta_fused(AttnOp* a, bool on) { a->delta_fused = on; }
static void attn_delta_target(AttnOp* a, Plan& p, GemmP& g) {
  gemm_attach_delta(g, p.P(a->o), a->o->ld(), p.F(a->delta_off), a->Nq, a->heads);
}

struct SiluOp : Op {
  Act *x, *y;
  size_t dy_off = NONE;
  Plan::GradDst dx;
  SiluOp(Act* x_, Act* y_) : x(x_), y(y_) {}
  int fwd(Plan& p, hipStream_t st) override { return launch_silu_fwd(p.P(x), p.P(y), x->rows * x->cols, st); }
  void plan_bwd(Plan& p) override { dy_off = y->goff; dx = p.grad_dst(x); }
  int bwd(Plan& p, hipStream_t st, bool) override {
    return launch_silu_bwd(p.P(x), p.GP(dy_off), p.GP(dx.out), p.GP(dx.addend), x->rows * x->cols, st);
  }
};

struct ConcatOp : Op {
  Act *a, *b, *o;
  size_t do_off = NONE;
  Plan::GradDst da, db;
  ConcatOp(Act* a_, Act* b_, Act* o_) : a(a_), b(b_), o(o_) {}
  int fwd(Plan& p, hipStream_t st) override { return launch_concat(p.P(a), a->cols, p.P(b), b->cols, p.P(o), a->rows, st); }
  void plan_bwd(Plan& p) override { do_off = o->goff; da = p.grad_dst(a); db = p.grad_dst(b); }
  int bwd(Plan& p, hipStream_t st, bool) override {
    return launch_split_add(p.GP(do_off), p.GP(da.out), a->cols, p.GP(da.addend), p.GP(db.out), b->cols, p.GP(db.addend),
                            a->rows, st);
  }
};

struct UpsampleOp : Op {
  Act *x, *y;
  int Bn, H, W, C;
  size_t dy_off = NONE;
  Plan::GradDst dx;
  ConvOp* fused = nullptr;
  UpsampleOp(Act* x_, Act* y_, int B_, int H_, int W_, int C_) : x(x_), y(y_), Bn(B_), H(H_), W(W_), C(C_) {}
  int fwd(Plan& p, hipStream_t st) override {
    if (fused && fused->up2() && fused->up_wg && KNOB(2) != 128) return 0;
    if (fused && fused->up2() && !p.eng->use_graphs) {
      const bf16* xp = p.P(x); bf16* yp = p.P(y);
      const int b = Bn, h = H, w = W, c = C;
      return on_side(p, st, [=](hipStream_t s2) -> int { return launch_upsample2x(xp, yp, b, h, w, c, s2); });
    }
    return launch_upsample2x(p.P(x), p.P(y), Bn, H, W, C, st);
  }
  void plan_bwd(Plan& p) override { dy_off = y->goff; dx = p.grad_dst(x); }
  int bwd(Plan& p, hipStream_t st, bool) override {
    if (fused && fused->up2() && y->need_grad) return 0;
    return launch_upsample2x_bwd(p.GP(dy_off), p.GP(dx.out), p.GP(dx.addend), Bn, H, W, C, st);
  }
};

struct EmbedInOp : Op {
// ... 134 lines not shown
    Act* y = pl->new_act((long)B * ho * wo, cout);
    tagseg(pl->add<ConvOp>(x, y, w, b, B, h, w_, cin, cout, stride, resid, rowvec), w);
    return y;
  }
  Act* groupnorm(const std::string& name, Act* x, int hw, int C, float eps, int silu) {
    PRef g = e.param(C, true);
    e.map_src(name + ".weight", {C}, g, 0, 0, 0);
    PRef b = e.param(C, true);
    e.map_src(name + ".bias", {C}, b, 0, 0, 0);
    if (!pl) return nullptr;
    Act* y = pl->new_act(x->rows, C);
    tagseg(pl->add<GroupNormOp>(*pl, x, y, g, b, B, hw, C, e.cfg.norm_num_groups, eps, silu), g);
    return y;
  }
  Act* layernorm(const std::string& name, Act* x, int C) {
    PRef g = e.param(C, true);
    e.map_src(name + ".weight", {C}, g, 0, 0, 0);
    PRef b = e.param(C, true);
    e.map_src(name + ".bias", {C}, b, 0, 0, 0);
    if (!pl) return nullptr;
    Act* y = pl->new_act(x->rows, C);
    ln_of[y] = tagseg(pl->add<LayerNormOp>(*pl, x, y, g, b, C, e.cfg.ln_eps), g);
    return y;
  }
  Act* silu(Act* x) {
    if (!pl) return nullptr;
    Act* y = pl->new_act(x->rows, x->cols);
    tagseg(pl->add<SiluOp>(x, y), PRef());
    return y;
  }
  Act* resnet(const std::string& p, Act* x, int h, int w_, int cin, int cout) {
    Act* n1 = groupnorm(p + ".norm1", x, h * w_, cin, e.cfg.resnet_eps, 1);
    Act* tp = pl ? pl->view(tp_all, tp_col.at(p), cout) : nullptr;
    Act* c1 = conv(p + ".conv1", n1, h, w_, cin, cout, 1, nullptr, tp);
    Act* n2 = groupnorm(p + ".norm2", c1, h * w_, cout, e.cfg.resnet_eps, 1);
    Act* sc = x;
    if (cin != cout) sc = linear(p + ".conv_shortcut", x, cin, cout, true, nullptr, true);
    return conv(p + ".conv2", n2, h, w_, cout, cout, 1, sc, nullptr);
  }
  Act* tf_block(const std::string& b, Act* x, Act* ehs, int C, int N) {
    const int heads = C / e.cfg.head_dim, cross = e.cfg.cross_attention_dim;
    Act* l1 = layernorm(b + ".norm1", x, C);
    Act* qkv = linear_fused({b + ".attn1.to_q", b + ".attn1.to_k", b + ".attn1.to_v"}, l1, C, C);
    Act* a1 = nullptr;
    AttnOp* sa = nullptr;
    if (pl) {
      a1 = pl->new_act(x->rows, C);
      sa = tagseg(pl->add<AttnOp>(*pl, qkv, qkv, a1, B, heads, N, N, C, true), PRef());
    }
    LinearOp* o1 = nullptr;
    Act* x1 = linear(b + ".attn1.to_out.0", a1, C, C, true, x, false, 0, &o1);
    if (sa && o1 && KNOB(21) != 1 && C % 128 == 0 && (x->rows / 128) * (C / 160) <= 256 && sa->qsplit <= 1) { sa->delta_fused = true; o1->delta_attn = sa; }
    Act* l2 = layernorm(b + ".norm2", x1, C);
    Act* q = linear(b + ".attn2.to_q", l2, C, C, false, nullptr);
    Act* kv = pl ? pl->view(kv_all.at(C), kv_col.at(b), 2 * C) : nullptr;
    (void)cross;
    Act* a2 = nullptr;
    if (pl) {
      a2 = pl->new_act(x->rows, C);
      tagseg(pl->add<AttnOp>(*pl, q, kv, a2, B, heads, N, ctx, C, false), PRef())->needs_hoisted = true;
    }
    Act* x2 = linear(b + ".attn2.to_out.0", a2, C, C, true, x1);
    Act* l3 = layernorm(b + ".norm3", x2, C);
    const int group = (KNOB(5) == 80 && (4 * C) % 80 == 0) ? 80 : 64;
    LinearOp *ff1 = nullptr, *ff2 = nullptr;
    Act* u = linear(b + ".ff.net.0.proj", l3, C, 8 * C, true, nullptr, false, 2, &ff1, group);
    Act* g = pl ? wide_act(x->rows, 4 * C) : nullptr;
    if (ff1) { ff1->gact = g; ff1->ggroup = group; }
    Act* y = linear(b + ".ff.net.2", g, 4 * C, C, true, x2, false, 0, &ff2);
    if (ff2) { ff2->gu = u; ff2->ggroup = group; }
    return y;
  }
  Act* transformer(const std::string& p, Act* x, Act* ehs, int h, int w_, int C, int depth) {
    Act* n = groupnorm(p + ".norm", x, h * w_, C, e.cfg.tf_gn_eps, 0);
    Act* t = linear(p + ".proj_in", n, C, C, true, nullptr);
    for (int k = 0; k < depth; ++k) t = tf_block(p + ".transformer_blocks." + std::to_string(k), t, ehs, C, h * w_);
    return linear(p + ".proj_out", t, C, C, true, x);
  }
  void run() {
    const sdxl_unet_config& c = e.cfg;
    const int* ch = c.block_out_channels;
    const int temb = ch[0] * 4;
    const int add_in = c.pooled_dim + 6 * c.addition_time_embed_dim;
    Act *x_in = nullptr, *ehs = nullptr, *te_sin = nullptr, *aug_in = nullptr;
    if (pl) {
      pl->x_in = x_in = pl->new_act((long)B * H * W, 8, false);
      pl->ehs = ehs = pl->new_act((long)B * ctx, c.cross_attention_dim, false, kv_pad_rows(B, ctx));
      pl->te_sin = te_sin = pl->new_act(B, ch[0], false);
      pl->tid_emb = pl->new_act((long)B * 6, c.addition_time_embed_dim, false);
      pl->aug_in = aug_in = pl->new_act(B, add_in, false);
      pl->t_off = pl->alloc(sizeof(float) * B);
      pl->tid_off = pl->alloc(sizeof(float) * B * 6);
      pl->loss_off = pl->alloc(sizeof(float) * 8);
      pl->loss_part_off = pl->alloc(sizeof(float) * loss_part_floats(B, H * W));
      pl->in_lat_off = pl->alloc(sizeof(float) * (size_t)B * 4 * H * W);
      pl->in_noise_off = pl->alloc(sizeof(float) * (size_t)B * 4 * H * W);
      pl->in_sig_off = pl->alloc(sizeof(float) * B);
      pl->in_tag_off = pl->alloc(sizeof(float) * B);
      tagseg(pl->add<EmbedInOp>(), PRef());
    }
    auto register_kv = [&](int Cgrp) {
      std::vector<std::pair<std::string, int>> blocks;
      auto add_tf = [&](const std::string& p, int C, int depth) {
        if (C != Cgrp) return;
        for (int k = 0; k < depth; ++k) blocks.emplace_back(p + ".transformer_blocks." + std::to_string(k), C);
      };
      for (int i = 0; i < 3; ++i)
        for (int j = 0; j < c.layers_per_block; ++j)
          if (c.transformer_layers[i] > 0) add_tf("down_blocks." + std::to_string(i) + ".attentions." + std::to_string(j), ch[i], c.transformer_layers[i]);
      add_tf("mid_block.attentions.0", ch[2], c.transformer_layers[2]);
      for (int ui = 0; ui < 3; ++ui)
        for (int j = 0; j < c.layers_per_block + 1; ++j)
          if (c.transformer_layers[2 - ui] > 0) add_tf("up_blocks." + std::to_string(ui) + ".attentions." + std::to_string(j), ch[2 - ui], c.transformer_layers[2 - ui]);
// ... 102 lines not shown
        if (pl) {
          up = pl->new_act((long)B * 4 * h * w, prev);
          uop = tagseg(pl->add<UpsampleOp>(x, up, B, h, w, prev), PRef());
        }
        h *= 2;
        w *= 2;
        x = conv(p + ".upsamplers.0.conv", up, h, w, prev, prev, 1, nullptr, nullptr);
        if (pl) {
          ConvOp* cop = dynamic_cast<ConvOp*>(pl->ops.back().get());
          if (cop) { cop->enable_up2(*pl, xlow, &uop->dx); if (cop->x_low) uop->fused = cop; }
        }
      }
    }
    Act* no = groupnorm("conv_norm_out", x, h * w, prev, c.resnet_eps, 1);
    Act* out = conv("conv_out", no, h, w, prev, 8, 1, nullptr, nullptr, prev, c.out_channels);
    if (pl) pl->pred = out;
  }
};
}

void Engine::build(Plan* plan) {
  registering = plan == nullptr;
  native_cursor = 0;
  Builder b(*this, plan);
  b.run();
  if (registering) {
    const size_t target = 96u << 20;
    seg_begin.clear();
    seg_end.clear();
    size_t start = 0;
    for (size_t i = 0; i < natives.size(); ++i) {
      size_t end = i + 1 < natives.size() ? natives[i + 1].off : param_elems;
      if (natives[i].numel >= target && natives[i].off > start) {
        seg_begin.push_back(start);
        seg_end.push_back(natives[i].off);
        start = natives[i].off;
      }
      if (end - start >= target || i + 1 == natives.size()) {
        seg_begin.push_back(start);
        seg_end.push_back(end);
        start = end;
      }
    }
    nseg = (int)seg_begin.size();
    registering = false;
  } else {
    plan->gn_ws_off = plan->alloc(sizeof(float) * plan->gn_ws_floats);
    plan->grad_dst(plan->pred);
    for (int i = (int)plan->ops.size() - 1; i >= 0; --i) plan->ops[i]->plan_bwd(*plan);
    plan->slab_off = plan->alloc(sizeof(float) * (plan->slab_floats ? plan->slab_floats : 4));
    plan->slab_main_off = plan->alloc(sizeof(float) * (plan->slab_main_floats ? plan->slab_main_floats : 4));
    plan->apart_off = plan->alloc(sizeof(float) * (plan->apart_floats ? plan->apart_floats : 4));
    plan->apart_side_off = plan->alloc(sizeof(float) * (plan->apart_side_floats ? plan->apart_side_floats : 4));
    plan->ln_part_off = plan->alloc(sizeof(float) * (plan->ln_part_floats ? plan->ln_part_floats : 4));
    plan->in_sw_off = plan->alloc(sizeof(float) * plan->B);
    plan->in_hc_off = plan->alloc(sizeof(float) * plan->B);
    plan->ps_loss_off = plan->alloc(sizeof(float) * plan->B);
    plan->samp_part_off = plan->alloc(sizeof(float) * sampler_part_floats(plan->B, plan->H * plan->W));
    plan->in_mask_off = plan->alloc(sizeof(float) * (size_t)plan->B * plan->H * plan->W);
    plan->in_nin_off = plan->alloc(sizeof(float) * (size_t)plan->B * 4 * plan->H * plan->W);
    plan->mask_norm_off = plan->alloc(sizeof(float) * plan->B);
    {
      const sdxl_unet_config& c = cfg;
      const int Mk = plan->B * plan->ctx;
      plan->cond_nkv = 0;
      int Ks[2] = {0, 0};
      for (LinearOp* op : b.kv_ops) {
        if (plan->cond_nkv == 2) break;
        Plan::CondSrc& cs = plan->cond_kv[plan->cond_nkv];
        cs.dy_off = op->dy_off; cs.lda = op->y->ld(); cs.w = op->w; cs.ldb = op->K; cs.K = op->N;
        Ks[plan->cond_nkv++] = op->N;
      }
      if (b.add1_op) {
        Plan::CondSrc& cs = plan->cond_add;
        cs.dy_off = b.add1_op->dy_off; cs.lda = b.add1_op->y->ld(); cs.w = b.add1_op->w; cs.ldb = b.add1_op->K; cs.K = b.add1_op->N;
      }
      plan->dehs_off = plan->alloc(sizeof(float) * (size_t)Mk * c.cross_attention_dim);
      plan->dpool_off = plan->alloc(sizeof(float) * (size_t)plan->B * c.pooled_dim);
      size_t slab = plan->cond_nkv ? cond_dgrad_slab_floats(plan->cond_nkv, Ks, Mk, c.cross_attention_dim) : 0;
      const int Ka[2] = {plan->cond_add.K, 0};
      const size_t slab2 = cond_dgrad_slab_floats(1, Ka, plan->B, c.pooled_dim);
      if (slab2 > slab) slab = slab2;
      plan->cond_slab_off = plan->alloc(sizeof(float) * (slab ? slab : 4));
    }
    if (plan->lg_tu_elems) {
      plan->lg_tu_off = plan->alloc(sizeof(bf16) * plan->lg_tu_elems);
      plan->lg_part_off = plan->alloc(sizeof(float) * (plan->lg_part_floats ? plan->lg_part_floats : 4));
    }
    plan->seg_first_op.assign(nseg, -1);
    plan->seg_last_op.assign(nseg, -2);
    for (int i = 0; i < (int)plan->ops.size(); ++i) {
      int s = plan->ops[i]->seg;
      if (plan->seg_first_op[s] < 0) plan->seg_first_op[s] = i;
      plan->seg_last_op[s] = i;
    }
  }
}

template <typename TS, typename TD>
__global__ void repack_kernel(const TS* __restrict__ src, TD* __restrict__ dst, long n, int kind, int co, int ci,
                              int ci_pad, int to_native) {
  for (long i = (long)blockIdx.x * blockDim.x + threadIdx.x; i < n; i += (long)gridDim.x * blockDim.x) {
    long s = i, d = i;
    if (kind == 1) {
      long o = i / ((long)ci * 9);
      long rem = i - o * (long)ci * 9;
// ... 92 lines not shown
```

sdxl-training-improvements_amd/csrc/gemm.hip:

```cpp
#include "gemm_tiles.h"

#include <stdio.h>
#include <stdlib.h>

#include <type_traits>
#include <vector>

#define BM 128
#ifndef GEMM_DIRECT_EPILOGUE
#define GEMM_DIRECT_EPILOGUE 1
#endif

static int g_mode256 = 1;
static int g_force_cfg = 0;
#ifdef SDXL_DIAG
static int g_sk_mode = 0;
#endif

static constexpr int cdiv_c(int a, int b) { return (a + b - 1) / b; }
__device__ unsigned g_ln_spin_error = 0;
__device__ __forceinline__ float row16_sum(float v) {
  v += __builtin_bit_cast(float, __builtin_amdgcn_update_dpp(0, __builtin_bit_cast(int, v), 0x111, 0xf, 0xf, true));
  v += __builtin_bit_cast(float, __builtin_amdgcn_update_dpp(0, __builtin_bit_cast(int, v), 0x112, 0xf, 0xf, true));
  v += __builtin_bit_cast(float, __builtin_amdgcn_update_dpp(0, __builtin_bit_cast(int, v), 0x114, 0xf, 0xf, true));
// ... 1310 lines not shown
GemmP conv3x3_dgrad_problem(int B, int H, int W, int Cin, int Cout, int stride) {
  GemmP g = conv3x3_problem(GEMM_NN, B * H * W, Cin, Cout, H, W, (H - 1) / stride + 1, (W - 1) / stride + 1, 1, stride);
  g.lda = Cout; g.ldb = 9L * Cin; g.ldc = Cin;
  g.flip = 1; g.b_tap_stride = Cin;
  return g;
}
GemmP conv3x3_wgrad_problem(int B, int H, int W, int Cin, int Cout, int stride) {
  const int Ho = (H - 1) / stride + 1, Wo = (W - 1) / stride + 1;
  GemmP g = conv3x3_problem(GEMM_TN, Cout, Cin, B * Ho * Wo, Ho, Wo, H, W, stride, 1);
  g.lda = Cout; g.ldb = Cin; g.ldc = 9L * Cin;
  g.c_tap_stride = Cin;
  g.out_f32 = 1;
  return g;
}
static GemmP linear_problem(int form, const bf16* A, long lda, const bf16* B, long ldb, void* C, long ldc, int M, int N, int K) {
  GemmP g;
  gemm_defaults(&g);
  g.form = form;
  g.A = A; g.B = B; g.C = C;
  g.M = M; g.N = N; g.K = K;
  g.lda = lda; g.ldb = ldb; g.ldc = ldc;
  return g;
}
GemmP linear_fwd_problem(const bf16* x, long ldx, const bf16* w, void* y, long ldy, int M, int N, int K, const bf16* bias, const bf16* resid, long ldr) {
  GemmP g = linear_problem(GEMM_NT, x, ldx, w, K, y, ldy, M, N, K);
  g.bias = bias;
  if (resid) { g.resid = resid; g.ldr = ldr; }
  return g;
}
GemmP linear_dgrad_problem(const bf16* dy, long ldy, const bf16* w, void* dx, long ldx, int M, int N, int K, const bf16* addend, long ldr) {
  GemmP g = linear_problem(GEMM_NN, dy, ldy, w, N, dx, ldx, M, N, K);
  if (addend) { g.resid = addend; g.ldr = ldr; }
  return g;
}
GemmP linear_wgrad_problem(const bf16* dy, long ldy, const bf16* x, long ldx, float* dw, int Mo, int No, int rows, float* bias_grad) {
  GemmP g = linear_problem(GEMM_TN, dy, ldy, x, ldx, dw, No, Mo, No, rows);
  g.out_f32 = 1;
  g.bias_grad = bias_grad;
  return g;
}
void gemm_attach_geglu_fwd(GemmP& g, int group, bf16* gact, long ldgact) { g.geglu = 1; g.geglu_group = group; g.aux = gact; g.ldaux = ldgact; }
void gemm_attach_geglu_bwd(GemmP& g, int group, bf16* u, long ldu) { g.geglu = 2; g.geglu_group = group; g.aux = u; g.ldaux = ldu; g.ldc = ldu; }
void gemm_attach_delta(GemmP& g, const bf16* o, long ldo, float* delta, int nq, int heads) {
  g.delta_o = o; g.delta_ldo = ldo; g.delta_out = delta; g.delta_nq = nq; g.delta_heads = heads;
  g.cfg = 1;
}
void gemm_attach_ln_bwd(GemmP& g, const bf16* x, long ldx, const float* stats, const bf16* gamma, bf16* dx, const bf16* addend, float* part, int epoch,
                        float* pcol) {
  g.ln_x = x; g.ln_ldx = ldx; g.ln_stats = stats; g.ln_gamma = gamma;
  g.ln_dx = dx; g.ln_addend = addend; g.ln_ldo = ldx;
  g.ln_part = part; g.ln_epoch = epoch; g.ln_pcol = pcol;
  g.cfg = 0; g.resid = nullptr;
}
void gemm_fill_group(GemmP& g, const GemmP* v, int n) {
  g.group = n;
  for (int i = 0; i < n; ++i) { g.gA[i] = v[i].A; g.gB[i] = v[i].B; g.gC[i] = (float*)v[i].C; g.gbias_grad[i] = v[i].bias_grad; g.gCb[i] = v[i].Cb; }
}
void gemm_set_mode(int mode) { g_mode256 = mode & 3; g_force_cfg = mode >> 2; }
static int launch_gemm_impl(const GemmP& pin, hipStream_t st);
template <class F>
static int profiled(hipStream_t st, double flops, const GemmProf::Rec& rec, F launch) {
  if (!g_prof.on) return launch();
  while (g_prof.ev.size() < g_prof.used + 2) {
    hipEvent_t e;
    HIP_CHECK_RET(hipEventCreate(&e));
    g_prof.ev.push_back(e);
  }
  HIP_CHECK_RET(hipEventRecord(g_prof.ev[g_prof.used], st));
  int rc = launch();
  HIP_CHECK_RET(hipEventRecord(g_prof.ev[g_prof.used + 1], st));
  g_prof.used += 2;
  g_prof.flops.push_back(flops);
  g_prof.recs.push_back(rec);
  return rc;
}
#ifdef SDXL_DIAG
void gemm_set_sk_mode(int mode) { g_sk_mode = mode; }
int gemm_sk_mode() { return g_sk_mode; }
bool gemm_use_sk(const GemmP& p) {
  if (!gemm_sk_applicable(p)) return false;
  const long tiles = (long)(p.M / 256) * (p.N / 256), kt = p.K / 64;
  if (tiles * kt < 1024) return false;
  return true;
}
int launch_gemm_multi(const GemmP* ps, int n, hipStream_t st) {
  double f = 0;
  for (int i = 0; i < n; ++i) f += 2.0 * (double)ps[i].M * (double)ps[i].N * (double)ps[i].K;
  return profiled(st, f, {n > 1 ? 3 : ps[0].form, n, ps[0].M, ps[0].N, ps[0].K, 1}, [&] { return launch_gemm_sk(ps, n, st); });
}
#endif
FILE* launch_log() {
  static FILE* f = []() -> FILE* { const char* p = getenv("SDXL_LAUNCH_LOG"); return p ? fopen(p, "w") : nullptr; }();
  return f;
}
int launch_gemm(const GemmP& p, hipStream_t st) {
  if (FILE* f = launch_log()) {
    bool biasg = p.bias_grad;
    for (int i = 0; i < p.group && i < GEMM_MAX_GROUP; ++i) biasg = biasg || p.gbias_grad[i];
    fprintf(f, "G,%d,%d,%d,%d,%d,%d,%d,%d,%d,%d,%d,%d,%d,%d,%d,%d,%d,%d,%d,%d\n", p.form, p.taps, p.M, p.N, p.K, p.splitk, p.group > 1 ? p.group : 1, p.cfg, p.geglu,
            p.geglu_group, p.Hm, p.Wm, p.Hs, p.Ws, p.sm, p.sd, p.up2, p.Cb || (p.group > 1 && p.gCb[0]) ? 1 : 0, p.delta_out ? 1 : 0, biasg ? 1 : 0);
    fflush(f);
  }
  const double flops = 2.0 * (double)p.M * (double)p.N * (double)p.K * (p.up2 == 2 ? 2.25 : (double)p.taps) * (p.group > 1 ? p.group : 1);
  return profiled(st, flops, {p.form, p.taps, p.M, p.N, p.K, p.splitk}, [&] { return launch_gemm_impl(p, st); });
}

// ... 100 lines not shown
    if (!use && fc == 0 && KNOB(30) != 64 && p.taps == 1 && !tn) {
      const int bnp = p.N % 160 == 0 ? 160 : 128;
      const long tiles = (long)cdiv(p.M, BM) * cdiv(p.N, bnp);
      const int k30 = KNOB(30) ? KNOB(30) : 3;
      const bool one_round = tiles <= 256 && tiles > 128;
      use = ((k30 & 1) && p.form == GEMM_NT && one_round) || ((k30 & 2) && p.form == GEMM_NN && one_round) || ((k30 & 512) && p.form == GEMM_NN && one_round && p.K >= 2560) ||
            ((k30 & 16) && tiles > 128 && tiles % 256 == 0) || ((k30 & 1024) && p.form == GEMM_NT && tiles > 256 && tiles % 256 == 0) || (k30 & 32);
    }
    if (use && pl_applicable(p)) return {GEMM_KPL, pl_pf ? 8 : 7, false, GEMM_POST_NONE};
  }
  if (fc >= 31 && fc <= 36 && !p.delta_out && cr256_applicable(p)) {
    bool biasg = tn && p.bias_grad;
    for (int i = 0; tn && i < p.group; ++i) biasg = biasg || p.gbias_grad[i];
    return {GEMM_KCR256, fc == 31 && biasg ? 32 : fc, false, tn ? post : GEMM_POST_NONE};
  }
#ifdef SDXL_DIAG
  if (g_sk_mode && !p.delta_out && !(!tn && split) && (g_sk_mode == 2 ? gemm_sk_applicable(p) : gemm_use_sk(p))) return {GEMM_KSK, 0, false, GEMM_POST_NONE};
#endif
  if (g_mode256 && p.group <= 1 && !p.Cb && !p.delta_out && !(!tn && split) && gemm256_applicable(p)) {
    const bool geglu256 = p.geglu == 1 && p.geglu_group == 64 && (long)(p.M / 256) * (p.N / 256) >= 256;
    if (g_mode256 == 2 || gemm_use256(p.form, p.M, p.N, p.K, p.splitk) || geglu256) return {GEMM_K256, 0, false, post};
  }
  if (tn && p.taps != 1 && conv_wgrad3_applicable(p) && conv_wgrad3_policy(p.M, p.N, p.K, p.Wm, p.sm)) return {GEMM_KCONV_WGRAD3, 0, false, post};
  if (tn && p.taps == 1 && wgrad256_applicable(p) && wgrad256_policy(p.M, p.N, p.K)) return {GEMM_KWGRAD256, 0, false, post};
  return k128();
}
int gemm_route_checked(GemmP p, GemmRoute* r) {
  if (int e = gemm_check(p)) return e;
  *r = gemm_route(p);
  return 0;
}

static int launch_gemm_post(const GemmP& p, int post, hipStream_t st) {
  if (post == GEMM_POST_NONE) return 0;
  const int cols = post == GEMM_POST_REDUCE ? p.N * p.taps : p.N;
  const long nv = (long)p.M * (cols / (post == GEMM_POST_REDUCE ? 4 : 8));
  int g = (int)((nv + 255) / 256);
  if (g > 2048) g = 2048;
  if (post == GEMM_POST_REDUCE)
    hipLaunchKernelGGL(splitk_reduce_kernel, dim3(g), dim3(256), 0, st, p.slab, (float*)p.C, p.M, cols, p.ldc, p.slab_ld, p.splitk, p.accumulate, p.Cb,
                       p.cb_scale, p.up2 == 1 ? nullptr : p.bias_grad);
  else
    hipLaunchKernelGGL(splitk_epilogue_kernel, dim3(g), dim3(256), 0, st, p.slab, (bf16*)p.C, p.M, p.N, p.ldc, p.slab_ld, p.splitk,
                       p.bias, p.resid, p.ldr, p.rowvec, p.ldv, p.rows_per_batch > 0 ? p.rows_per_batch : 1);
  HIP_CHECK_RET(hipGetLastError());
  return 0;
}

static int launch_gemm_impl(const GemmP& pin, hipStream_t st) {
  GemmP p = pin;
  if (int e = gemm_check(p)) return e;
  const GemmRoute r = gemm_route(p);
  const bool conv = p.taps != 1;
  int rc;
  switch (r.kernel) {
    case GEMM_KPL: return launch_pl(p, 0, st, r.cfg == 8);
    case GEMM_KCR256: rc = launch_cr256(p, (r.cfg == 31 || r.cfg == 33 || r.cfg == 36) ? 160 : 128, st, r.cfg == 33 || r.cfg == 34, r.cfg == 35 || r.cfg == 36); break;
#ifdef SDXL_DIAG
    case GEMM_KSK: {
      GemmP q = p;
      q.splitk = 1;
      return launch_gemm_sk(&q, 1, st);
    }
#endif
    case GEMM_K256: rc = launch_gemm256(p, st); break;
    case GEMM_KCONV_WGRAD3: rc = launch_conv_wgrad3(p, st); break;
    case GEMM_KWGRAD256: rc = launch_wgrad256(p, st); break;
    default:
      if (p.form == GEMM_NT) rc = conv ? launch_one<GEMM_NT, true>(p, r, st) : launch_one<GEMM_NT, false>(p, r, st);
      else if (p.form == GEMM_TN) rc = conv ? launch_one<GEMM_TN, true>(p, r, st) : launch_one<GEMM_TN, false>(p, r, st);
      else if (p.form == GEMM_NN) rc = conv ? launch_one<GEMM_NN, true>(p, r, st) : launch_one<GEMM_NN, false>(p, r, st);
      else ARG_CHECK(false, "gemm: unknown form %d", p.form);
  }
  return rc ? rc : launch_gemm_post(p, r.post, st);
}

int launch_upconv3x3_fwd(const bf16* x, const bf16* w, const bf16* bias, bf16* weff, bf16* planar, bf16* y, int B, int H, int W,
                         int Cin, int Cout, int splitk, float* slab, hipStream_t st) {
  if (int e = launch_upconv_fold_weights(w, weff, Cout, Cin, st)) return e;
  GemmP g;
  gemm_defaults(&g);
  g.form = GEMM_NT;
  g.up2 = 1; g.taps = 4;
  g.A = x; g.B = weff; g.C = planar;
  g.up_rows = B * H * W; g.up_plane = (int)upconv_plane_rows(B, H, W);
  g.M = 4 * g.up_plane; g.N = Cout; g.K = Cin;
  g.lda = Cin; g.ldb = 16L * Cin; g.ldc = Cout;
  g.Hm = H; g.Wm = W; g.Hs = H; g.Ws = W;
  g.b_tap_stride = Cin;
  g.bias = bias;
  if (splitk > 1) { g.splitk = splitk; g.slab = slab; }
  if (int e = launch_gemm(g, st)) return e;
  return launch_pixel_shuffle2(planar, y, B, H, W, Cout, 1, st);
}
int launch_upconv3x3_dgrad(const bf16* dy, const bf16* weff, bf16* planar, bf16* dx, const bf16* addend, int B, int H, int W, int Cin,
                           int Cout, int splitk, float* slab, int prio, hipStream_t st) {
  if (dy) { if (int e = launch_pixel_shuffle2(dy, planar, B, H, W, Cout, 0, st)) return e; }
  GemmP g;
  gemm_defaults(&g);
  g.form = GEMM_NN;
  g.up2 = 1; g.taps = 16;
  g.A = planar; g.B = weff; g.C = dx;
  g.up_rows = B * H * W; g.up_plane = (int)upconv_plane_rows(B, H, W);
  g.M = B * H * W; g.N = Cin; g.K = Cout;
  g.lda = Cout; g.ldb = 16L * Cin; g.ldc = Cin;
  g.Hm = H; g.Wm = W; g.Hs = H; g.Ws = W;
// ... 89 lines not shown
```

sdxl-training-improvements_amd/csrc/gemm_pl.hip:

```cpp
#include "gemm_tiles.h"

#include <type_traits>

namespace {

constexpr int PL_BM = 128, PL_BK = 64, PL_S = 4;
constexpr unsigned PL_OOB = 0x80000000u;

#ifndef SDXL_PL_DIAG
#define SDXL_PL_DIAG 0
#endif

template <int BN>
struct PlGeom {
  static constexpr int A_BYTES = PL_BM * PL_BK * 2;
  static constexpr int B_BYTES = BN * PL_BK * 2;
  static constexpr int STAGE = A_BYTES + B_BYTES;
  static constexpr int SMEM = PL_S * STAGE;
  static constexpr int ACH = A_BYTES / 1024 / 4;
  static constexpr int BCH = B_BYTES / 1024 / 4;
  static constexpr int NL = ACH + BCH;
  static constexpr int NP0 = (NL + 1) / 2;
  static constexpr int NJ = BN / 32;
  static constexpr int MI = 4;
  static constexpr int NMF = MI * NJ;
};

#pragma clang diagnostic push
#pragma clang diagnostic ignored "-Winline-asm"
template <int OFF>
__device__ __forceinline__ void pl_dma(i32x4 srd, unsigned voff, unsigned soff, unsigned slot_base) {
  asm volatile("s_add_u32 m0, %3, %4\n\ts_nop 0\n\tbuffer_load_dwordx4 %0, %1, %2 offen lds"
               :: "v"(voff), "s"(srd), "s"(soff), "s"(slot_base), "n"(OFF) : "memory", "scc", "m0");
}
#pragma clang diagnostic pop

__device__ __forceinline__ bf16x8 pl_z8() {
  bf16x8 z;
#pragma unroll
  for (int e = 0; e < 8; ++e) z[e] = (bf16)0.f;
  return z;
}
template <int NJ>
struct PlFrag { bf16x8 a[4], b[NJ]; };

template <typename F, int... I>
__device__ __forceinline__ void pl_static_for_impl(F&& f, std::integer_sequence<int, I...>) { (f(std::integral_constant<int, I>{}), ...); }
template <int N, typename F>
__device__ __forceinline__ void pl_static_for(F&& f) { pl_static_for_impl(f, std::make_integer_sequence<int, N>{}); }

constexpr int PL_PF_LEAD = 10;
template <int FORM, int BN, bool PF>
__global__ __launch_bounds__(PF ? 320 : 256, 2) void pl_kernel(const GemmP p) {
  using G = PlGeom<BN>;
  constexpr bool B_KC = FORM == GEMM_NT;
  constexpr int NJ = G::NJ, MI = G::MI, NL = G::NL, NP0 = G::NP0, NMF = G::NMF;
  constexpr int dbg = SDXL_PL_DIAG;
  static_assert(FORM == GEMM_NT || FORM == GEMM_NN, "pipelined kernel: NT / NN");
  extern __shared__ __attribute__((aligned(16))) char smem[];
  set_wave_prio(p.prio);
  const int tid = threadIdx.x, lane = tid & 63;
  const int wave = __builtin_amdgcn_readfirstlane(tid >> 6);
  const int wm = wave >> 1, wn = wave & 1;
  const int l16 = lane & 15, g = lane >> 4;
  int bx, by;
  xcd_tile_map(p.xcd_px, bx, by);
  const int n0 = (dbg & 8) ? 0 : bx * BN, m0 = (dbg & 8) ? 0 : by * PL_BM;
  const int M = p.M, N = p.N;
  const int lda = (int)p.lda, ldb = (int)p.ldb;
  const int T = p.K / PL_BK;

  if (PF && wave == 4) {
    int tn = 1, tm = 1, ln = 0, lm = 0;
    if (p.xcd_px > 0 && gridDim.x % p.xcd_px == 0 && gridDim.y % (8 / p.xcd_px) == 0) {
      tn = gridDim.x / p.xcd_px; tm = gridDim.y / (8 / p.xcd_px);
      ln = bx % tn; lm = by % tm;
    }
    const int ra_n = (PL_BM + tn - 1) / tn;
    const char* Ab = (const char*)p.A;
    const char* Bb = (const char*)p.B;
    constexpr int B_UNITS = B_KC ? BN : PL_BK * ((BN * 2 + 127) / 128);
    const int rb_n = (B_UNITS + tm - 1) / tm;
    unsigned sink = 0;
    auto touch = [&](int tp) {
      if (tp >= T) return;
      for (int u = lane; u < ra_n; u += 64) {
        const int row = m0 + ln * ra_n + u;
        if (ln * ra_n + u < PL_BM && row < M) {
          asm volatile("global_load_dword %0, %1, off sc1" : "+v"(sink) : "v"(Ab + ((long)row * lda + (long)tp * PL_BK) * 2) : "memory");
        }
      }
      for (int u = lane; u < rb_n; u += 64) {
        const int q = lm * rb_n + u;
        if (q < B_UNITS) {
          const char* src;
          bool ok;
          if (B_KC) { const int row = n0 + q; ok = row < N; src = Bb + ((long)row * ldb + (long)tp * PL_BK) * 2; }
          else { constexpr int LPR = (BN * 2 + 127) / 128; const int kr = q / LPR, li = q - kr * LPR; const int col = n0 + li * 64; ok = col < N; src = Bb + (((long)tp * PL_BK + kr) * ldb + col) * 2; }
          if (ok) {
            asm volatile("global_load_dword %0, %1, off sc1" : "+v"(sink) : "v"(src) : "memory");
          }
        }
      }
    };
    for (int tp = PL_S - 1; tp < PL_PF_LEAD; ++tp) touch(tp);
    __builtin_amdgcn_s_barrier();
    for (int t = 0; t < T; ++t) {
      touch(t + PL_PF_LEAD);
      __builtin_amdgcn_s_barrier();
    }
    asm volatile("s_waitcnt vmcnt(0)" : "+v"(sink) :: "memory");
    return;
  }

  const i32x4 ra = make_srd(p.A, 0x7FFFFFFFu), rb = make_srd(p.B, 0x7FFFFFFFu);
  const unsigned lds_w = lds_addr_of(smem) + (unsigned)wave * 1024u;
  unsigned voA[G::ACH], voB[G::BCH];
  {
    const int kc_row = lane >> 3, kc_vec = (lane & 7) ^ kc_row;
#pragma unroll
    for (int j = 0; j < G::ACH; ++j) {
      const int row = m0 + 8 * (wave + 4 * j) + kc_row;
      voA[j] = row < M ? (unsigned)(((long)row * lda + kc_vec * 8) * 2) : PL_OOB;
    }
#pragma unroll
    for (int j = 0; j < G::BCH; ++j) {
      if (B_KC) {
        const int row = n0 + 8 * (wave + 4 * j) + kc_row;
        voB[j] = row < N ? (unsigned)(((long)row * ldb + kc_vec * 8) * 2) : PL_OOB;
      } else {
        constexpr int V = BN / 8;
        const int q = (wave + 4 * j) * 64 + lane;
        const int krow = q / V, pv = q - krow * V;
        const int n = n0 + (nc_logical<BN>(krow, pv) << 3);
        voB[j] = n < N ? (unsigned)(((long)krow * ldb + n) * 2) : PL_OOB;
      }
    }
  }
  unsigned soA = 0, soB = 0;
  const unsigned stepA = PL_BK * 2, stepB = B_KC ? PL_BK * 2 : (unsigned)(PL_BK * ldb * 2);
  const unsigned oob = PL_OOB;

  auto piece = [&](auto PC, auto LIVE, unsigned sb) {
    constexpr int pc = decltype(PC)::value;
    constexpr bool live = decltype(LIVE)::value;
    if constexpr (pc < G::ACH) pl_dma<pc * 4096>(ra, live ? voA[pc] : oob, soA, sb);
    else pl_dma<G::A_BYTES + (pc - G::ACH) * 4096>(rb, live ? voB[pc - G::ACH] : oob, soB, sb);
  };

  f32x4 acc[MI][NJ];
#pragma unroll
  for (int i = 0; i < MI; ++i)
#pragma unroll
    for (int j = 0; j < NJ; ++j) acc[i][j] = (f32x4){0.f, 0.f, 0.f, 0.f};
  bf16x8 ones;
#pragma unroll
  for (int e = 0; e < 8; ++e) ones[e] = (bf16)1.0f;

  using Frag = PlFrag<NJ>;
  constexpr int NITEM = MI + NJ;
  typedef const __attribute__((address_space(3))) bf16x8 lds_bf16x8;
  typedef __attribute__((address_space(3))) s16x4 lds_s16x4_t;
  constexpr int NBB = B_KC ? 1 : NJ;
  unsigned bA[2], bB[2][NBB];
  {
    const unsigned l0 = lds_addr_of(smem);
#pragma unroll
// ... 30 lines not shown
    else if constexpr (it < NJ) {
      if constexpr (B_KC) {
        f.b[it] = *(lds_bf16x8*)(size_t)(ra_.b[0] + (unsigned)(it * 2048));
      } else {
        const unsigned a0 = ra_.b[it];
        const s16x4 lo = __builtin_amdgcn_ds_read_tr16_b64_v4i16((lds_s16x4_t*)(size_t)a0);
        const s16x4 hi = __builtin_amdgcn_ds_read_tr16_b64_v4i16((lds_s16x4_t*)(size_t)(a0 + 4u * (BN * 2)));
        union { s16x4 s2[2]; bf16x8 v; } u;
        u.s2[0] = lo; u.s2[1] = hi;
        f.b[it] = u.v;
      }
    } else {
      constexpr int i = it - NJ;
      f.a[i] = *(lds_bf16x8*)(size_t)(ra_.a + (unsigned)(i * 2048));
    }
  };
  auto phase = [&](auto PHC, auto LIVE, const Frag& fc, Frag& fn, unsigned rbase, auto RKS, unsigned sb) {
    constexpr int PH = decltype(PHC)::value;
    constexpr int NPP = PH == 0 ? NP0 : NL - NP0;
    static_assert(2 * (NITEM - 1) < NMF && NPP <= NMF / 4, "filler schedule: reads behind the even MFMAs, pieces behind every fourth odd one");
    const RAddr rad = raddr(rbase, RKS);
    pl_static_for<NMF>([&](auto KC) {
      constexpr int k = decltype(KC)::value, i = k / NJ, j = k % NJ;
      if (dbg & 1) acc[i][j][0] += (float)fc.a[i][0] + (float)fc.b[j][0];
      else acc[i][j] = __builtin_amdgcn_mfma_f32_16x16x32_bf16(fc.b[j], fc.a[i], acc[i][j], 0, 0, 0);
      __builtin_amdgcn_sched_barrier(0);
      if constexpr (k % 2 == 0 && k / 2 < NITEM) read_item(rad, fn, std::integral_constant<int, k / 2>{});
      if constexpr (!(dbg & 2) && k % 2 == 1) {
        pl_static_for<NPP>([&](auto QC) {
          constexpr int q = decltype(QC)::value;
          if constexpr (k == 1 + 2 * ((q * (NMF / 2)) / NPP)) piece(std::integral_constant<int, PH * NP0 + q>{}, LIVE, sb);
        });
      }
      __builtin_amdgcn_sched_barrier(0);
    });
  };

  {
    unsigned sb = lds_w;
#pragma unroll
    for (int d = 0; d < PL_S - 1; ++d) {
      if (d < T) pl_static_for<NL>([&](auto PC) { piece(PC, std::true_type{}, sb); });
      else pl_static_for<NL>([&](auto PC) { piece(PC, std::false_type{}, sb); });
      soA += stepA; soB += stepB;
      sb += G::STAGE;
    }
  }
  Frag f0, f1;
  wait_vmcnt<(PL_S - 2) * NL>();
  __builtin_amdgcn_s_barrier();
  {
    const RAddr rad = raddr(0u, std::integral_constant<int, 0>{});
    pl_static_for<NITEM>([&](auto IT) { read_item(rad, f0, IT); });
  }
  int rd = 0, wr = PL_S - 1;
  auto kstep = [&](auto LIVE) {
    const unsigned sb = lds_w + (unsigned)wr * G::STAGE;
    phase(std::integral_constant<int, 0>{}, LIVE, f0, f1, (unsigned)rd * G::STAGE, std::integral_constant<int, 1>{}, sb);
    wait_vmcnt<(PL_S - 3) * NL + NP0>();
    asm volatile("s_waitcnt lgkmcnt(0)" ::: "memory");
    __builtin_amdgcn_sched_barrier(0);
    __builtin_amdgcn_s_barrier();
    const int rn = rd + 1 == PL_S ? 0 : rd + 1;
    phase(std::integral_constant<int, 1>{}, LIVE, f1, f0, (unsigned)rn * G::STAGE, std::integral_constant<int, 0>{}, sb);
    soA += stepA; soB += stepB;
    rd = rn;
    wr = wr + 1 == PL_S ? 0 : wr + 1;
  };
  const int Tlive = T - (PL_S - 1);
  int t = 0;
  for (; t < Tlive; ++t) kstep(std::true_type{});
  for (; t < T; ++t) kstep(std::false_type{});
  constexpr int NP = NJ / 2;
  constexpr bool ODD = (NJ & 1) != 0;
  const int mrow = m0 + wm * 64 + l16;
  const int ncol8 = n0 + wn * (BN / 2) + (g & 1) * 16 + (g >> 1) * 8;
  const int ncol4 = n0 + wn * (BN / 2) + (NJ - 1) * 16 + g * 4;
  bf16x8 res8[MI][NP], bias8[NP];
  bf16x4 res4[MI], bias4;
  const bool has_res = p.resid != nullptr, has_bias = p.bias != nullptr;
  {
    bf16x4 z4; z4[0] = z4[1] = z4[2] = z4[3] = (bf16)0.f;
#pragma unroll
    for (int i = 0; i < MI; ++i) {
#pragma unroll
      for (int jp = 0; jp < NP; ++jp) res8[i][jp] = pl_z8();
      res4[i] = z4;
    }
#pragma unroll
    for (int jp = 0; jp < NP; ++jp) bias8[jp] = pl_z8();
    bias4 = z4;
  }
  if (has_res) {
#pragma unroll
    for (int i = 0; i < MI; ++i) {
      const int m = mrow + 16 * i;
#pragma unroll
      for (int jp = 0; jp < NP; ++jp) {
        const int n = ncol8 + 32 * jp;
        res8[i][jp] = (m < M && n < N) ? *(const bf16x8*)(p.resid + (long)m * p.ldr + n) : pl_z8();
      }
      if (ODD) {
        bf16x4 z; z[0] = z[1] = z[2] = z[3] = (bf16)0.f;
        res4[i] = (m < M && ncol4 < N) ? *(const bf16x4*)(p.resid + (long)m * p.ldr + ncol4) : z;
      }
    }
  }
  if (has_bias) {
#pragma unroll
    for (int jp = 0; jp < NP; ++jp) {
      const int n = ncol8 + 32 * jp;
      bias8[jp] = n < N ? *(const bf16x8*)(p.bias + n) : pl_z8();
    }
    if (ODD) {
      bf16x4 z; z[0] = z[1] = z[2] = z[3] = (bf16)0.f;
      bias4 = ncol4 < N ? *(const bf16x4*)(p.bias + ncol4) : z;
    }
  }
  wait_vmcnt<0>();
  asm volatile("s_nop 7\n\ts_nop 7\n\ts_nop 7" ::: "memory");
#pragma unroll
  for (int i = 0; i < MI; ++i) {
    const int m = mrow + 16 * i;
#pragma unroll
    for (int jp = 0; jp < NP; ++jp) {
      const int j = 2 * jp;
      float x[8];
#pragma unroll
      for (int r = 0; r < 4; ++r) {
        float lo = acc[i][j][r], hi = acc[i][j + 1][r];
        asm volatile("s_nop 1\n\tv_permlane16_swap_b32 %0, %1" : "+v"(lo), "+v"(hi));
        x[r] = lo;
        x[4 + r] = hi;
      }
      const int n = ncol8 + 32 * jp;
#pragma unroll
      for (int e = 0; e < 8; ++e) { x[e] += (float)bias8[jp][e]; x[e] += (float)res8[i][jp][e]; }
      if (m < M && n < N) {
        bf16x8 o;
#pragma unroll
        for (int e = 0; e < 8; ++e) o[e] = (bf16)x[e];
        *(bf16x8*)((bf16*)p.C + (long)m * p.ldc + n) = o;
      }
    }
    if (ODD) {
      float x[4];
#pragma unroll
      for (int r = 0; r < 4; ++r) x[r] = acc[i][NJ - 1][r];
#pragma unroll
      for (int e = 0; e < 4; ++e) { x[e] += (float)bias4[e]; x[e] += (float)res4[i][e]; }
      if (m < M && ncol4 < N) {
        bf16x4 o;
#pragma unroll
        for (int e = 0; e < 4; ++e) o[e] = (bf16)x[e];
        *(bf16x4*)((bf16*)p.C + (long)m * p.ldc + ncol4) = o;
      }
    }
  }
}

template <int FORM, int BN, bool PF>
int launch_pl_k(const GemmP& p, hipStream_t st) {
  static bool attr_set = false;
  if (!attr_set) {
    HIP_CHECK_RET(hipFuncSetAttribute((const void*)pl_kernel<FORM, BN, PF>, hipFuncAttributeMaxDynamicSharedMemorySize, PlGeom<BN>::SMEM));
    attr_set = true;
  }
  dim3 grid(cdiv(p.N, BN), cdiv(p.M, PL_BM), 1);
  GEMM_LAUNCH((pl_kernel<FORM, BN, PF>), grid, dim3(PF ? 320 : 256), PlGeom<BN>::SMEM, st, p);
  HIP_CHECK_RET(hipGetLastError());
  return 0;
}

}

bool pl_applicable(const GemmP& p) {
  if (p.form != GEMM_NT && p.form != GEMM_NN) return false;
  if (p.taps != 1 || p.up2 || p.geglu || p.splitk > 1 || p.group > 1 || p.delta_out || p.ln_x || p.out_f32 || p.Cb || p.rowvec) return false;
  if (p.K % PL_BK || p.N % 8 || p.lda % 8 || p.ldb % 8 || p.ldc % 8) return false;
  const long abytes = 2 * (long)p.M * p.lda;
  const long bbytes = 2 * (p.form == GEMM_NT ? (long)p.N * p.ldb : (long)p.K * p.ldb);
  if (abytes >= (1L << 31) || bbytes >= (1L << 31)) return false;
  return true;
}

#ifdef SDXL_DIAG
__global__ __launch_bounds__(256) void pl_prefetch_b_kernel(const bf16* __restrict__ B, long ldb, int K, int form, int px, int cols_per_xcd,
                                                            int parts, unsigned* sink) {
  const int i = blockIdx.x, xcd = i & 7, part = i >> 3;
  const int n0 = (xcd % px) * cols_per_xcd;
  const long rows = form == GEMM_NT ? cols_per_xcd : K, rowbytes = 2L * (form == GEMM_NT ? K : cols_per_xcd);
  const char* base = (const char*)(form == GEMM_NT ? B + (long)n0 * ldb : B + n0);
  const long vpr = rowbytes / 16, total = rows * vpr;
  unsigned acc = 0;
  for (long v = (long)part * 256 + threadIdx.x; v < total; v += (long)parts * 256) {
    const long r = v / vpr, c = v - r * vpr;
    const uint4 x = *(const uint4*)(base + r * ldb * 2 + c * 16);
    acc ^= x.x ^ x.y ^ x.z ^ x.w;
  }
  if (acc == 0x9e3779b9u && sink) *sink = acc;
}
int launch_pl_prefetch_b(const GemmP& p, int parts, hipStream_t st) {
  const int bn = p.N % 160 == 0 ? 160 : 128;
  const int gx = cdiv(p.N, bn), gy = cdiv(p.M, PL_BM);
  double best = 1e30;
  int bpx = 0;
  for (int px = 1; px <= 8; px *= 2) {
    const int py = 8 / px;
    if (gx % px || gy % py) continue;
    const double cost = (double)p.N / px + (double)p.M / py;
    if (cost < best) { best = cost; bpx = px; }
  }
  if (!bpx) return 0;
  hipLaunchKernelGGL(pl_prefetch_b_kernel, dim3(8 * parts), dim3(256), 0, st, p.B, p.ldb, p.K, p.form, bpx, gx / bpx * bn, parts, (unsigned*)nullptr);
  HIP_CHECK_RET(hipGetLastError());
  return 0;
}
#endif

int launch_pl(const GemmP& pin, int bn, hipStream_t st, bool prefetch) {
  ARG_CHECK(pl_applicable(pin), "gemm_pl: problem %dx%dx%d (form %d) does not fit the pipelined kernel", pin.M, pin.N, pin.K, pin.form);
  GemmP p = pin;
  if (bn != 128 && bn != 160) bn = p.N % 160 == 0 ? 160 : 128;
  {
    const int gx = cdiv(p.N, bn), gy = cdiv(p.M, PL_BM);
    double best = 1e30;
    p.xcd_px = 0;
    for (int px = 1; px <= 8; px *= 2) {
      const int py = 8 / px;
      if (gx % px || gy % py) continue;
      const double cost = (double)p.N / px + (double)p.M / py;
      if (cost < best) { best = cost; p.xcd_px = px; }
    }
  }
#ifdef SDXL_DIAG
  if (prefetch && p.K / PL_BK > PL_PF_LEAD) {
    if (p.form == GEMM_NT) return bn == 160 ? launch_pl_k<GEMM_NT, 160, true>(p, st) : launch_pl_k<GEMM_NT, 128, true>(p, st);
    return bn == 160 ? launch_pl_k<GEMM_NN, 160, true>(p, st) : launch_pl_k<GEMM_NN, 128, true>(p, st);
  }
#endif
  (void)prefetch;
  if (p.form == GEMM_NT) return bn == 160 ? launch_pl_k<GEMM_NT, 160, false>(p, st) : launch_pl_k<GEMM_NT, 128, false>(p, st);
  return bn == 160 ? launch_pl_k<GEMM_NN, 160, false>(p, st) : launch_pl_k<GEMM_NN, 128, false>(p, st);
}
```

sdxl-training-improvements_amd/csrc/hooks.hip:

```cpp
#include "capi.h"

static int hook_scratch(size_t bytes, void** out) {
  static char* buf = nullptr;
  static size_t cap = 0;
  if (bytes > cap) {
    if (buf) { (void)hipFree(buf); buf = nullptr; cap = 0; }
    HIP_CHECK_RET(hipMalloc((void**)&buf, bytes));
    cap = bytes;
  }
  *out = buf;
  return 0;
}
static int hook_floats(size_t n, float** out) { return hook_scratch(n * sizeof(float), (void**)out); }
static int dense_problem(int form, const void* A, const void* B, void* C, int M, int N, int K, const void* bias, const void* resid, int accumulate,
                         GemmP* g) {
  const bf16 *a = (const bf16*)A, *b = (const bf16*)B, *r = (const bf16*)resid;
  ARG_CHECK(form == GEMM_NT || form == GEMM_NN || form == GEMM_TN, "gemm: unknown form %d", form);
  if (form == GEMM_NT) *g = linear_fwd_problem(a, K, b, C, N, M, N, K, (const bf16*)bias, r, N);
  else if (form == GEMM_NN) { *g = linear_dgrad_problem(a, K, b, C, N, M, N, K, r, N); g->bias = (const bf16*)bias; }
  else { *g = linear_wgrad_problem(a, M, b, N, (float*)C, M, N, K, (float*)bias); if (r) { g->resid = r; g->ldr = N; } }
  g->accumulate = accumulate;
  return 0;
}

// ... 291 lines not shown
  L.method = lc->method; L.prediction_type = lc->prediction_type; L.use_min_snr = lc->use_min_snr;
  L.min_snr_gamma = lc->min_snr_gamma; L.use_ztsnr = lc->use_ztsnr;
  L.B = b->B; L.HW = b->H * b->W; L.C = 4;
  L.latents = b->latents; L.noise = b->noise; L.sigma = b->sigma_or_t; L.tag_w = b->tag_weights;
  L.unet_in = (bf16*)unet_in; L.pred = (const bf16*)pred; L.dpred = (bf16*)dpred;
  L.grad_scale = grad_scale; L.out = out8;
  CHK(check_loss_ext(lc, b));
  fill_loss_ext(lc, b, L);
  if (phase == 1 || (phase == 2 && L.mask && L.mask_norm == 1)) {
    ARG_CHECK(L.B > 0 && L.HW > 0, "loss: empty batch");
    CHK(hook_floats(loss_part_floats(L.B, L.HW) + (size_t)L.B, &L.part));
    L.mnorm = L.part + loss_part_floats(L.B, L.HW);
  }
  if (phase == 0) return launch_loss_prepare(L, (hipStream_t)st);
  if (phase == 1) return launch_loss_fwd(L, (hipStream_t)st);
  if (phase == 2) return launch_loss_bwd(L, (hipStream_t)st);
  ARG_CHECK(false, "phase %d", phase);
}

int sdxl_op_sampler_step(float* x, const void* pred, void* x_in, int B, int H, int W, const sdxl_sampler_step* s, void* st) {
  ARG_CHECK(s, "null argument");
  ARG_CHECK(B > 0 && H > 0 && W > 0, "sampler: empty batch");
  sdxl_sampler_step_ext t;
  memset(&t, 0, sizeof(t));
  memcpy(&t, s, (s->init & SDXL_SAMPLER_EXT) ? sizeof(sdxl_sampler_step_ext) : sizeof(sdxl_sampler_step));
  t.base.x = x;
  SamplerP q;
  CHK(fill_sampler(&t.base, s->cfg ? 2 * B : B, H * W, q));
  q.pred = (const bf16*)pred; q.x_in = (bf16*)x_in;
  if (!q.init && q.rescale != 0.f) CHK(hook_floats(sampler_part_floats(B, H * W), &q.part));
  return launch_sampler_step(q, (hipStream_t)st);
}
int sdxl_probe_layout(void* out, void* st) { return probe_layout(out, (hipStream_t)st); }
int sdxl_op_exchange_shadow(void* buf, size_t bytes, int workgroups, int lds_bytes, float busy_us, void* st) {
  return launch_exchange_shadow(buf, bytes, workgroups, lds_bytes, busy_us, (hipStream_t)st);
}
int sdxl_op_gemm_ld(int form, const void* A, const void* B, void* C, int M, int N, int K, long lda, long ldb, long ldc, const void* bias,
                    const void* resid, long ldr, int cfg, void* st) {
  ARG_CHECK(form == GEMM_NT || form == GEMM_NN, "gemm_ld: NT / NN only (form %d)", form);
  GemmP g;
  if (form == GEMM_NT) g = linear_fwd_problem((const bf16*)A, lda, (const bf16*)B, C, ldc, M, N, K, (const bf16*)bias, (const bf16*)resid, ldr);
  else { g = linear_dgrad_problem((const bf16*)A, lda, (const bf16*)B, C, ldc, M, N, K, (const bf16*)resid, ldr); g.bias = (const bf16*)bias; }
  g.ldb = ldb;
  g.cfg = cfg;
  return launch_gemm(g, (hipStream_t)st);
}
int sdxl_op_linear_dgrad_delta(const void* dy, const void* w, const void* o, const void* addend, void* d_o, float* delta, int B, int Nq,
                               int N, int K, void* st) {
  ARG_CHECK(dy && w && o && d_o && delta && B > 0 && Nq > 0 && N % 128 == 0 && K % 64 == 0, "linear_dgrad_delta: B=%d Nq=%d N=%d K=%d", B, Nq, N, K);
  GemmP g = linear_dgrad_problem((const bf16*)dy, K, (const bf16*)w, d_o, N, B * Nq, N, K, (const bf16*)addend, N);
  gemm_attach_delta(g, (const bf16*)o, N, delta, Nq, N / 64);
  return launch_gemm(g, (hipStream_t)st);
}
int sdxl_debug_gemm_route(const sdxl_gemm_desc* d, sdxl_gemm_route* out) {
  ARG_CHECK(d && out, "gemm_route: null argument");
  alignas(16) static float word[4];
  GemmP g;
  CHK(dense_problem(d->form, word, word, word, d->M, d->N, d->K, nullptr, nullptr, 0, &g));
  g.taps = d->taps; g.cfg = d->cfg;
  g.ldb *= d->taps;
  if (d->form == GEMM_TN) g.ldc *= d->taps;
  g.Hm = d->Hm; g.Wm = d->Wm; g.Hs = d->Hs; g.Ws = d->Ws; g.sm = d->sm; g.sd = d->sd;
  g.up2 = d->up2;
  if (d->up2) {
    const int rows = d->form == GEMM_TN ? d->K : d->M;
    const bool planar = d->up2 == 2 || (d->up2 == 1 && d->form == GEMM_NT);
    ARG_CHECK(d->Hm > 0 && d->Wm > 0, "gemm_route: up2 needs the image size");
    g.up_plane = planar ? rows / 4 : (int)upconv_plane_rows(1, 1, rows);
    g.up_rows = planar ? g.up_plane / (d->Hm * d->Wm) * (d->Hm * d->Wm) : rows;
  }
  g.geglu = d->geglu; g.geglu_group = d->geglu_group;
  if (d->geglu) { g.aux = (bf16*)word; g.ldaux = 8; }
  g.splitk = d->splitk; g.slab = word;
  if (d->group > 1) {
    g.group = d->group;
    for (int i = 0; i < d->group && i < GEMM_MAX_GROUP; ++i) { g.gA[i] = g.gB[i] = (const bf16*)word; g.gC[i] = word; g.gCb[i] = d->emit_bf16 ? (bf16*)word : nullptr; g.gbias_grad[i] = d->bias_grad ? word : nullptr; }
  } else if (d->emit_bf16) g.Cb = (bf16*)word;
  if (d->bias_grad) g.bias_grad = word;
  if (d->delta) { g.delta_out = word; g.delta_o = (const bf16*)word; g.delta_nq = d->M; g.delta_heads = d->N / 64; }
  GemmRoute r;
  if (int e = gemm_route_checked(g, &r)) return e;
  out->kernel = r.kernel; out->cfg = r.cfg; out->fast = r.fast; out->post = r.post;
  return 0;
}
int sdxl_profile_gemm_begin(void) { return gemm_profile_begin(); }
int sdxl_set_gemm_mode(int mode) {
  const int cfg = mode >> 2;
  ARG_CHECK(mode >= 0 && (mode & 3) <= 2 && (cfg == 0 || cfg == 1 || cfg == 2 || cfg == 3 || cfg == 5 || cfg == 6 || cfg == 7 || cfg == 8 || cfg == 13 || cfg == 23 || cfg == 43 || cfg == 31 || cfg == 32 || cfg == 33 || cfg == 34 || cfg == 35 || cfg == 36), "gemm mode %d", mode);
  gemm_set_mode(mode);
  return 0;
}
int sdxl_profile_gemm_end(double* flops, double* ms, int* launches) { return gemm_profile_end(flops, ms, launches); }
#ifdef SDXL_DIAG
int sdxl_op_linear_dgrad_ln_bwd(const void* dy, const void* w, const void* x, const float* stats, const void* gamma, const void* addend,
                                void* dx, void* dy_out, float* pcol, int M, int N, int Kr, void* st) {
  ARG_CHECK(gemm_ln_cfg(M, N, Kr) != 0, "linear_dgrad_ln_bwd: M=%d N=%d K=%d does not fit the fused epilogue", M, N, Kr);
  float* part;
  const size_t pbytes = gemm_ln_part_floats(M, N) * sizeof(float);
  CHK(hook_scratch(pbytes, (void**)&part));
  HIP_CHECK_RET(hipMemsetAsync(part, 0, pbytes, (hipStream_t)st));
  GemmP g = linear_dgrad_problem((const bf16*)dy, Kr, (const bf16*)w, dy_out, N, M, N, Kr, nullptr, 0);
  for (int epoch = 1; epoch <= 3; ++epoch) {
    gemm_attach_ln_bwd(g, (const bf16*)x, N, stats, (const bf16*)gamma, (bf16*)dx, (const bf16*)addend, part, epoch, pcol);
    CHK(launch_gemm(g, (hipStream_t)st));
  }
  return 0;
// ... 71 lines not shown
```

sdxl-training-improvements_amd/csrc/kernels.h:

```cpp
#pragma once
#include "common.h"

#define SDXL_NKNOBS 40
#ifdef SDXL_DIAG
extern int g_knobs[SDXL_NKNOBS];
#define KNOB(i) (g_knobs[(i)])
constexpr bool SDXL_DIAG_BUILD = true;
constexpr bool SDXL_UP2_3 = true;
constexpr bool SDXL_LN_EPILOGUE = true;
#else
#define KNOB(i) 0
constexpr bool SDXL_DIAG_BUILD = false;
constexpr bool SDXL_UP2_3 = false;
constexpr bool SDXL_LN_EPILOGUE = false;
#endif

enum { GEMM_NT = 0, GEMM_NN = 1, GEMM_TN = 2 };
#define GEMM_LAUNCH(kernel, grid, block, smem, st, p)                                                          \
  do {                                                                                                         \
    if ((p).anyorder) hipExtLaunchKernelGGL(kernel, grid, block, smem, st, nullptr, nullptr, hipExtAnyOrderLaunch, p); \
    else hipLaunchKernelGGL(kernel, grid, block, smem, st, p);                                                 \
  } while (0)

#define GEMM_MAX_GROUP 4
struct GemmP {
  int form;
  const bf16* A;
  const bf16* B;
  void* C;
  int M, N, K;
  long lda, ldb, ldc;
  int taps;
  int Hm, Wm, Hs, Ws, sm, sd;
  int flip;
  int up2;
  int up_plane, up_rows;
  long b_tap_stride;
  long c_tap_stride;
  const bf16* bias;
  const bf16* resid;
  long ldr;
  const bf16* rowvec;
  long ldv;
  int rows_per_batch;
  int geglu;
  int geglu_group;
  bf16* aux;
  long ldaux;
  int out_f32;
  int accumulate;
  int splitk;
  float* slab;
  long slab_ld;
  bf16* Cb;
  float cb_scale;
  float* bias_grad;
  const bf16* delta_o;
  long delta_ldo;
  float* delta_out;
  int delta_nq, delta_heads;
  const bf16* ln_x;
  long ln_ldx;
  const float* ln_stats;
  const bf16* ln_gamma;
  bf16* ln_dx;
  const bf16* ln_addend;
  long ln_ldo;
  float* ln_part;
  int ln_epoch;
  float* ln_pcol;
  int xcd_px;
  int xcd_bh;
  int tail_n0;
  int anyorder;
  int cfg;
  int prio;
  int group;
  const bf16* gA[GEMM_MAX_GROUP];
  const bf16* gB[GEMM_MAX_GROUP];
  float* gC[GEMM_MAX_GROUP];
  float* gbias_grad[GEMM_MAX_GROUP];
  bf16* gCb[GEMM_MAX_GROUP];
};

__device__ __forceinline__ void gemm_bias_out(float* bias_grad, float* slab, long slab_ld, int splitk, int split, int M, int m, float v) {
  if (splitk > 1) slab[(long)splitk * M * slab_ld + (long)split * M + m] = v;
  else atomicAdd(bias_grad + m, v);
}
int gemm_pick_group(int M, int N, int taps, long red, int splitk);
size_t gemm_slab_floats(int M, int N, int taps, int splitk);
void gemm_defaults(GemmP* p);
int launch_gemm(const GemmP& p, hipStream_t st);
enum { GEMM_K128 = 0, GEMM_K256, GEMM_KCR256, GEMM_KPL, GEMM_KWGRAD256, GEMM_KCONV_WGRAD3, GEMM_KSK };
enum { GEMM_POST_NONE = 0, GEMM_POST_REDUCE, GEMM_POST_EPILOGUE };
struct GemmRoute {
  int kernel;
  int cfg;
  bool fast;
  int post;
};
GemmRoute gemm_route(const GemmP& p);
int gemm_route_checked(GemmP p, GemmRoute* r);
bool gemm256_applicable(const GemmP& p);
void gemm_set_mode(int mode);
bool gemm_use256(int form, int M, int N, int K, int splitk);
int gemm_pick_splitk(int M, int N, int taps, long red);
int gemm_pick_splitk_small(int M, int N, int K, int kind = -1);
int linear_wgrad_splitk(int Mo, int No, long rows);
int conv3x3_fwd_splitk(int B, int H, int W, int Cin, int Cout, int stride);
int conv3x3_dgrad_splitk(int B, int H, int W, int Cin, int Cout, int stride);
int conv3x3_wgrad_splitk(int B, int H, int W, int Cin, int Cout, int stride);
int upconv3x3_fwd_splitk(int B, int H, int W, int Cin, int Cout);
int upconv3x3_dgrad_splitk(int B, int H, int W, int Cin, int Cout);
GemmP conv3x3_fwd_problem(int B, int H, int W, int Cin, int Cout, int stride);
GemmP conv3x3_dgrad_problem(int B, int H, int W, int Cin, int Cout, int stride);
GemmP conv3x3_wgrad_problem(int B, int H, int W, int Cin, int Cout, int stride);
GemmP linear_fwd_problem(const bf16* x, long ldx, const bf16* w, void* y, long ldy, int M, int N, int K, const bf16* bias, const bf16* resid, long ldr);
GemmP linear_dgrad_problem(const bf16* dy, long ldy, const bf16* w, void* dx, long ldx, int M, int N, int K, const bf16* addend, long ldr);
GemmP linear_wgrad_problem(const bf16* dy, long ldy, const bf16* x, long ldx, float* dw, int Mo, int No, int rows, float* bias_grad);
void gemm_attach_geglu_fwd(GemmP& g, int group, bf16* gact, long ldgact);
void gemm_attach_geglu_bwd(GemmP& g, int group, bf16* u, long ldu);
void gemm_attach_delta(GemmP& g, const bf16* o, long ldo, float* delta, int nq, int heads);
void gemm_attach_ln_bwd(GemmP& g, const bf16* x, long ldx, const float* stats, const bf16* gamma, bf16* dx, const bf16* addend, float* part, int epoch,
                        float* pcol);
void gemm_fill_group(GemmP& g, const GemmP* v, int n);
int launch_gemm256(const GemmP& p, hipStream_t st);
void gemm256_set_tail(bool on);
#ifdef SDXL_DIAG
bool gemm_sk_applicable(const GemmP& p);
int launch_gemm_sk(const GemmP* problems, int n, hipStream_t st);
int launch_gemm_multi(const GemmP* problems, int n, hipStream_t st);
void gemm_set_sk_mode(int mode);
int gemm_sk_mode();
bool gemm_use_sk(const GemmP& p);
void gemm_sk_set_workers(int n);
int gemm_ln_error(unsigned* out);
int gemm_sk_error(hipStream_t st, unsigned* out);
#endif
bool conv_wgrad3_applicable(const GemmP& p);
bool conv_wgrad3_policy(int M, int N, long red, int Wm, int stride);
int conv_wgrad3_pick_splitk(int M, int N, long red);
int launch_conv_wgrad3(const GemmP& p, hipStream_t st);
void conv_wgrad3_set_enabled(bool on);
bool wgrad256_applicable(const GemmP& p);
bool wgrad256_policy(int M, int N, long red);
int wgrad256_pick_splitk(int M, int N, long red);
int launch_wgrad256(const GemmP& p, hipStream_t st);
void wgrad256_set_enabled(bool on);
bool cr256_applicable(const GemmP& p);
int launch_cr256(const GemmP& p, int bn, hipStream_t st, bool deep = false, bool phased = false);
int cr256_wgrad_cfg(int M, int N, long red, bool bias);
bool pl_applicable(const GemmP& p);
int launch_pl(const GemmP& p, int bn, hipStream_t st, bool prefetch = false);
int launch_pl_prefetch_b(const GemmP& p, int parts, hipStream_t st);
int gemm_ln_cfg(int M, int N, int K);
size_t gemm_ln_part_floats(int M, int N);
size_t gemm_ln_pcol_floats(int M, int N);
int gemm_ln_rowblocks(int M);
int cr256_pick_splitk(int M, int N, long red, int cfg);
int gemm_profile_begin();
FILE* launch_log();
bool gemm_profiling();
int gemm_profile_end(double* flops, double* ms, int* launches);

struct AttnP {
  const bf16 *Q, *K, *V;
  bf16* O;
  float* LSE;
  int B, H, Nq, Nk;
  long ldq, ldk, ldv, ldo;
  const bf16* dO;
  long lddo;
  bf16 *dQ, *dK, *dV;
  long lddq, lddk, lddv;
  float* Delta;
  int accumulate;
  int qsplit;
  float* part;
  int prio;
  int delta_ready;
  int xcd;
};
size_t attn_part_floats(int B, int H, int Nk, int qsplit);
int attn_pick_qsplit(int B, int H, int Nq, int Nk);
int launch_attn_fwd(const AttnP& p, hipStream_t st);
int launch_attn_fwd_tiled(const AttnP& p, hipStream_t st);
bool attn_fwd_pl_applicable(const AttnP& p);
int launch_attn_fwd_pl(const AttnP& p, hipStream_t st);
bool attn_bwd_pl_applicable(const AttnP& p);
int launch_attn_bwd_pl(const AttnP& p, hipStream_t st);
int launch_attn_bwd(const AttnP& p, hipStream_t st);
int launch_attn_bwd_dq(const AttnP& p, hipStream_t st);
int launch_attn_bwd_dkv(const AttnP& p, hipStream_t st);
int launch_attn_bwd_fused(const AttnP& p, hipStream_t st);

size_t groupnorm_ws_floats(int B, int C, int G);
int launch_groupnorm_fwd(const bf16* x, bf16* y, const bf16* gamma, const bf16* beta, float* stats,
                         float* ws, int B, int HW, int C, int G, float eps, int silu,
                         hipStream_t st);
int launch_groupnorm_bwd(const bf16* x, const bf16* dy, const bf16* gamma, const bf16* beta,
                         const float* stats, bf16* dx, const bf16* addend, float* dgamma, float* dbeta, float* ws,
                         int B, int HW, int C, int G, int silu, hipStream_t st, float* prow = nullptr);
int launch_layernorm_fwd(const bf16* x, bf16* y, const bf16* gamma, const bf16* beta, float* stats, int M,
                         int C, float eps, hipStream_t st);
size_t layernorm_bwd_part_floats(int M, int C);
int launch_layernorm_bwd(const bf16* x, const bf16* dy, const bf16* gamma, const float* stats, bf16* dx,
                         const bf16* addend, float* part, int* nblk_out, int M, int C, hipStream_t st);
int launch_layernorm_param_grads(const bf16* x, const bf16* dy, const float* stats, float* dgamma, float* dbeta, int M, int C, hipStream_t st);
int layernorm_param_partial_rows(int M, int C);
int launch_layernorm_param_partials(const bf16* x, const bf16* dy, const float* stats, float* part, int M, int C, hipStream_t st);
#define LN_RED_MAX 64
struct LnRedEntry { const float* part; float* dgamma; float* dbeta; int nblk, C; };
struct LnRedBatch { LnRedEntry e[LN_RED_MAX]; int n; };
int launch_ln_param_reduce(const LnRedBatch& b, hipStream_t st);

int launch_silu_fwd(const bf16* x, bf16* y, long n, hipStream_t st);
int launch_silu_bwd(const bf16* x, const bf16* dy, bf16* dx, const bf16* addend, long n, hipStream_t st);
int launch_add(const bf16* a, const bf16* b, bf16* o, long n, hipStream_t st);
size_t colsum_part_floats(int batches, int rows, int N);
int launch_colsum_f32_batched(const bf16* x, float* out, int batches, int rows, int N, long ldx, long ld_out, float* part, hipStream_t st);
int launch_colsum_partials(const bf16* x, float* out, int batches, int rows, int N, long ldx, long ld_out, float* part, LnRedEntry* entries, hipStream_t st);
int launch_concat(const bf16* a, int Ca, const bf16* b, int Cb, bf16* o, long rows, hipStream_t st);
int launch_split_add(const bf16* g, bf16* ga, int Ca, const bf16* add_a, bf16* gb, int Cb, const bf16* add_b,
                     long rows, hipStream_t st);
int launch_upsample2x(const bf16* x, bf16* y, int B, int H, int W, int C, hipStream_t st);
int launch_upconv_fold_weights(const bf16* w, bf16* weff, int Cout, int Cin, hipStream_t st);
int launch_pixel_shuffle2(const bf16* src, bf16* dst, int B, int H, int W, int C, int to_hi, hipStream_t st, const bf16* addend = nullptr);
static inline long upconv_plane_rows(int B, int H, int W) { return ((long)B * H * W + 127) / 128 * 128; }
int launch_upconv3x3_fwd(const bf16* x, const bf16* w, const bf16* bias, bf16* weff, bf16* planar, bf16* y, int B, int H, int W, int Cin,
                         int Cout, int splitk, float* slab, hipStream_t st);
#ifdef SDXL_DIAG
int launch_conv3x3_s2_fwd(const bf16* x, const bf16* w, const bf16* bias, bf16* xplanar, bf16* y, int B, int H, int W, int Cin, int Cout,
                          hipStream_t st);
int launch_conv3x3_s2_wgrad(const bf16* dy, const bf16* xplanar, float* dw, float* dbias, bf16* emit, float emit_scale, int accumulate, int B,
                            int H, int W, int Cin, int Cout, int splitk, float* slab, hipStream_t st);
#endif
int launch_conv3x3_s2_dgrad(const bf16* dy, const bf16* w, bf16* planar, bf16* dx, const bf16* addend, int B, int H, int W, int Cin,
                            int Cout, int prio, hipStream_t st);
int launch_upconv_unfold_grads(const float* dweff, float* dw, bf16* emit, float emit_scale, int accumulate, int Cout, int Cin, hipStream_t st);
int launch_upconv3x3_wgrad(const bf16* planar, const bf16* x, float* dweff, float* dw, float* dbias, bf16* emit, float emit_scale,
                           int accumulate, int B, int H, int W, int Cin, int Cout, int splitk, float* slab, hipStream_t st);
int launch_upconv3x3_dgrad(const bf16* dy, const bf16* weff, bf16* planar, bf16* dx, const bf16* addend, int B, int H, int W, int Cin,
                           int Cout, int splitk, float* slab, int prio, hipStream_t st);
int launch_upsample2x_bwd(const bf16* dy, bf16* dx, const bf16* addend, int B, int H, int W, int C, hipStream_t st);
int launch_sincos(const float* t, bf16* out, int rows, int dim, long ldo, hipStream_t st);
int launch_copy_cols(const bf16* src, long lds, bf16* dst, long ldd, int rows, int cols, hipStream_t st);
int launch_f32_to_bf16(const float* x, bf16* y, long n, float scale, hipStream_t st);
int launch_bf16_to_f32(const bf16* x, float* y, long n, hipStream_t st);
int launch_sumsq_f32(const float* x, long n, float* out , hipStream_t st);
int launch_sumsq_bf16(const bf16* x, long n, float* out , hipStream_t st);
int launch_clip_coef(const float* sumsq, float max_norm, float* coef, hipStream_t st);
int launch_scale_f32(float* x, long n, const float* scale_dev, hipStream_t st);
int launch_exchange_shadow(void* buf, size_t bytes, int workgroups, int lds_bytes, float busy_us, hipStream_t st);

struct LossP {
  int method;
  int prediction_type;
  int use_min_snr;
  float min_snr_gamma;
  int use_ztsnr;
  int B, HW, C;
  const float* latents;
  const float* noise;
  const float* sigma;
  const float* tag_w;
  bf16* unet_in;
  const bf16* pred;
// ... 179 lines not shown
```

sdxl-training-improvements_amd/csrc/norm.hip:

```cpp
#include "kernels.h"

struct GnGeom {
  int vpr;
  int rpi;
  int threads;
  int chunks;
  int rows_per_chunk;
};
#define GN_MAX_CHUNKS 256
static GnGeom gn_geom(int HW, int C) {
  GnGeom g;
  g.vpr = C / 8;
  g.rpi = g.vpr >= 256 ? 1 : 256 / g.vpr;
  g.threads = g.vpr * g.rpi;
  int chunks = HW / (g.rpi * 8);
  if (chunks < 1) chunks = 1;
  if (chunks > GN_MAX_CHUNKS) chunks = GN_MAX_CHUNKS;
  g.rows_per_chunk = (HW + chunks - 1) / chunks;
  g.chunks = (HW + g.rows_per_chunk - 1) / g.rows_per_chunk;
  return g;
}
size_t groupnorm_ws_floats(int B, int C, int G) {
  size_t fwd = (size_t)GN_MAX_CHUNKS * B * G * 2 + (size_t)B * C * 2;
  size_t bwd = (size_t)GN_MAX_CHUNKS * B * C * 2 + (size_t)B * C * 5;
// ... 733 lines not shown
  if (!params) { iters = 1; nblk = cdiv(M, 256 / lpr); }
  if (nblk_out) *nblk_out = nblk;
  dim3 blk(256), grid(nblk);
#define LN_LAUNCH(NV, LPR)                                                                                               \
  {                                                                                                                      \
    if (!params && KNOB(11) != 1) {                                                                                  \
      if (accumulate) hipLaunchKernelGGL((ln_bwd_lean_kernel<NV, LPR, true>), grid, blk, 0, st, x, dy, gamma, stats, dx, addend, M, KNOB(28));  \
      else hipLaunchKernelGGL((ln_bwd_lean_kernel<NV, LPR, false>), grid, blk, 0, st, x, dy, gamma, stats, dx, addend, M, KNOB(28));            \
    } else if (params) {                                                                                                        \
      if (accumulate) hipLaunchKernelGGL((ln_bwd_dx_kernel<NV, LPR, true, true>), grid, blk, 0, st, x, dy, gamma, stats, dx, addend, part, M, iters); \
      else hipLaunchKernelGGL((ln_bwd_dx_kernel<NV, LPR, false, true>), grid, blk, 0, st, x, dy, gamma, stats, dx, addend, part, M, iters);          \
    } else {                                                                                                             \
      if (accumulate) hipLaunchKernelGGL((ln_bwd_dx_kernel<NV, LPR, true, false>), grid, blk, 0, st, x, dy, gamma, stats, dx, addend, part, M, iters); \
      else hipLaunchKernelGGL((ln_bwd_dx_kernel<NV, LPR, false, false>), grid, blk, 0, st, x, dy, gamma, stats, dx, addend, part, M, iters);          \
    }                                                                                                                    \
  }
  if (lpr == 32) {
    switch (C / 256) {
      case 4: LN_LAUNCH(4, 32) break;
      case 5: LN_LAUNCH(5, 32) break;
      case 8: LN_LAUNCH(8, 32) break;
      case 10: LN_LAUNCH(10, 32) break;
      default: ARG_CHECK(false, "layernorm bwd: C=%d not instantiated", C);
    }
  } else {
    switch (C / 128) {
      case 1: LN_LAUNCH(1, 16) break;
      case 2: LN_LAUNCH(2, 16) break;
      case 3: LN_LAUNCH(3, 16) break;
      case 4: LN_LAUNCH(4, 16) break;
      case 5: LN_LAUNCH(5, 16) break;
      case 6: LN_LAUNCH(6, 16) break;
      case 7: LN_LAUNCH(7, 16) break;
      default: ARG_CHECK(false, "layernorm bwd: C=%d not instantiated", C);
    }
  }
#undef LN_LAUNCH
  HIP_CHECK_RET(hipGetLastError());
  return 0;
}
int launch_ln_param_reduce(const LnRedBatch& b, hipStream_t st) {
  if (b.n <= 0) return 0;
  ARG_CHECK(b.n <= LN_RED_MAX, "ln_param_reduce: %d entries", b.n);
  int cmax = 0, nmax = 0;
  for (int i = 0; i < b.n; ++i) {
    cmax = b.e[i].C > cmax ? b.e[i].C : cmax;
    nmax = b.e[i].nblk > nmax ? b.e[i].nblk : nmax;
  }
  hipLaunchKernelGGL(ln_param_reduce_kernel, dim3(cdiv(2 * cmax, 64), nmax <= 1024 ? 1 : 16, b.n), dim3(256), 0, st, b);
  HIP_CHECK_RET(hipGetLastError());
  return 0;
}

int launch_layernorm_param_grads(const bf16* x, const bf16* dy, const float* stats, float* dgamma, float* dbeta, int M, int C, hipStream_t st) {
  ARG_CHECK(C % 8 == 0, "layernorm param grads: C=%d must be a multiple of 8", C);
  dim3 g2; int rpc;
  col_reduce_geom(M, C, &g2, &rpc);
  hipLaunchKernelGGL(col_reduce_kernel, g2, dim3(256), 0, st, x, dy, (long)C, stats, dgamma, dbeta, M, C, rpc, 0L, 0L, (float*)nullptr);
  HIP_CHECK_RET(hipGetLastError());
  return 0;
}
int launch_layernorm_param_partials(const bf16* x, const bf16* dy, const float* stats, float* part, int M, int C, hipStream_t st) {
  ARG_CHECK(C % 128 == 0, "layernorm param partials: C=%d must be a multiple of 128", C);
  int cv, cb, rpc, chunks;
  ln_partials_geom(M, C, &cv, &cb, &rpc, &chunks);
  if (cv == 32) hipLaunchKernelGGL(ln_param_partials_kernel<32>, dim3(cb, chunks), dim3(256), 0, st, x, dy, stats, part, M, C, rpc);
  else hipLaunchKernelGGL(ln_param_partials_kernel<16>, dim3(cb, chunks), dim3(256), 0, st, x, dy, stats, part, M, C, rpc);
  HIP_CHECK_RET(hipGetLastError());
  return 0;
}
static void colsum_geom(int batches, int rows, int N, dim3* g2, int* rpc) {
  col_reduce_geom(rows, N, g2, rpc);
  if (batches > 1 && g2->y >= 2u * batches) {
    *rpc *= batches;
    g2->y = cdiv(rows, *rpc);
  }
  g2->z = batches;
}
size_t colsum_part_floats(int batches, int rows, int N) {
  dim3 g2; int rpc;
  colsum_geom(batches, rows, N, &g2, &rpc);
  return (size_t)batches * g2.y * N;
}
int launch_colsum_partials(const bf16* x, float* out, int batches, int rows, int N, long ldx, long ld_out, float* part, LnRedEntry* entries,
                           hipStream_t st) {
  ARG_CHECK(N % 8 == 0 && ldx % 8 == 0 && part != nullptr, "colsum: N=%d ld=%ld must be multiples of 8 (and the partial rows given)", N, ldx);
  dim3 g2; int rpc;
  colsum_geom(batches, rows, N, &g2, &rpc);
  hipLaunchKernelGGL(col_reduce_kernel, g2, dim3(256), 0, st, (const bf16*)nullptr, x, ldx, (const float*)nullptr,
                     (float*)nullptr, out, rows, N, rpc, (long)rows * ldx, ld_out, part);
  HIP_CHECK_RET(hipGetLastError());
  for (int b = 0; b < batches; ++b) {
    LnRedEntry& e = entries[b];
    e.part = part + (size_t)b * g2.y * N;
    e.dgamma = out + (size_t)b * ld_out;
    e.dbeta = e.dgamma + N / 2;
    e.nblk = (int)g2.y;
    e.C = N / 2;
  }
  return 0;
}
int launch_colsum_f32_batched(const bf16* x, float* out, int batches, int rows, int N, long ldx, long ld_out, float* part, hipStream_t st) {
  ARG_CHECK(batches >= 1 && batches <= LN_RED_MAX, "colsum: %d batches", batches);
  LnRedBatch rb;
  rb.n = batches;
  if (int e = launch_colsum_partials(x, out, batches, rows, N, ldx, ld_out, part, rb.e, st)) return e;
// ... 3 lines not shown
```

sdxl-training-improvements_amd/lib.py:

```python
from __future__ import annotations

import ctypes as C
from pathlib import Path

import os

HERE = Path(__file__).resolve().parent
DIAG = os.environ.get("SDXL_DIAG", "") == "1"
LIB_PATH = HERE / ("libsdxlstep_diag.so" if DIAG else "libsdxlstep.so")


def use_diag() -> None:
    global DIAG, LIB_PATH
    if _lib is not None and not DIAG:
        raise SdxlError("use_diag() after the product library has been loaded")
    DIAG, LIB_PATH = True, HERE / "libsdxlstep_diag.so"



class SdxlError(RuntimeError):
    pass


class UNetConfig(C.Structure):
# ... 107 lines not shown
    "sdxl_set_graph_mode": [_vp, _i],
    "sdxl_read_loss": [_vp, _P(_f), _vp],
    "sdxl_unet_forward": [_vp, _vp, _P(SamplerBatch), _vp, _vp],
    "sdxl_unet_backward": [_vp, _vp, _i, _vp],
    "sdxl_grads_to_bf16": [_vp, _sz, _sz, _vp, _f, _vp],
    "sdxl_set_grad_emit": [_vp, _vp, _f],
    "sdxl_small_grads_to_bf16": [_vp, _sz, _sz, _vp, _f, _vp],
    "sdxl_grad_sumsq": [_vp, _vp, _vp],
    "sdxl_op_gemm": [_i, _vp, _vp, _vp, _i, _i, _i, _vp, _vp, _i, _i, _vp],
    "sdxl_op_wgrad_group": [_i, _P(_vp), _P(_vp), _P(_vp), _P(_vp), _i, _i, _i, _i, _vp],
    "sdxl_op_conv3x3_fwd": [_vp, _vp, _vp, _vp, _i, _i, _i, _i, _i, _i, _vp],
    "sdxl_op_upconv3x3_fwd": [_vp, _vp, _vp, _vp, _vp, _vp, _i, _i, _i, _i, _i, _vp],
    "sdxl_op_upconv3x3_dgrad": [_vp, _vp, _vp, _vp, _vp, _i, _i, _i, _i, _i, _vp],
    "sdxl_op_conv3x3_s2_dgrad": [_vp, _vp, _vp, _vp, _vp, _i, _i, _i, _i, _i, _vp],
    "sdxl_op_upconv3x3_wgrad": [_vp, _vp, _vp, _vp, _vp, _i, _i, _i, _i, _i, _i, _i, _vp],
    "sdxl_op_conv3x3_dgrad": [_vp, _vp, _vp, _i, _i, _i, _i, _i, _i, _vp],
    "sdxl_op_conv3x3_wgrad": [_vp, _vp, _vp, _i, _i, _i, _i, _i, _i, _i, _vp],
    "sdxl_op_conv3x3_wgrad2": [_vp, _vp, _vp, _vp, _i, _i, _i, _i, _i, _i, _i, _i, _vp],
    "sdxl_op_attention_fwd": [_vp, _vp, _vp, _vp, _vp, _i, _i, _i, _i, _l, _l, _l, _l, _vp],
    "sdxl_op_attention_bwd": [_vp, _vp, _vp, _vp, _vp, _vp, _vp, _vp, _vp, _vp, _i, _i, _i, _i, _l, _l, _l, _l, _vp],
    "sdxl_op_groupnorm_fwd": [_vp, _vp, _vp, _vp, _vp, _vp, _i, _i, _i, _i, _f, _i, _vp],
    "sdxl_op_groupnorm_bwd": [_vp, _vp, _vp, _vp, _vp, _vp, _vp, _vp, _vp, _i, _i, _i, _i, _i, _i, _vp],
    "sdxl_op_layernorm_fwd": [_vp, _vp, _vp, _vp, _vp, _i, _i, _f, _vp],
    "sdxl_op_layernorm_bwd": [_vp, _vp, _vp, _vp, _vp, _vp, _vp, _i, _i, _i, _vp],
    "sdxl_set_join_mode": [_vp, _i],
    "sdxl_side_stream": [_vp, _P(_vp)],
    "sdxl_sumsq": [_vp, _i, _sz, _vp, _vp],
    "sdxl_clip_coef": [_vp, _f, _vp, _vp],
    "sdxl_param_range": [_vp, _i, _P(_sz), _P(_sz)],
    "sdxl_adamw_default_config": [C.POINTER(AdamWConfig)],
    "sdxl_adamw_bf16_step": [_vp, _vp, _i, _vp, _vp, _vp, _sz, C.POINTER(AdamWConfig), _vp, _vp, _vp],
    "sdxl_adamw_decay": [_vp, _vp, _sz, _f, _vp],
    "sdxl_op_ff_geglu_fwd": [_vp, _vp, _vp, _vp, _vp, _i, _i, _i, _i, _vp],
    "sdxl_op_ff_geglu_bwd": [_vp, _vp, _vp, _vp, _i, _i, _i, _i, _vp],
    "sdxl_op_loss": [_P(LossConfig), _P(Batch), _vp, _vp, _vp, _f, _vp, _i, _vp],
    "sdxl_profile_gemm_begin": [],
    "sdxl_profile_gemm_end": [_P(C.c_double), _P(C.c_double), _P(_i)],
}
TEST_HOOK_SIGNATURES = {
    "sdxl_probe_layout": [_vp, _vp],
    "sdxl_set_gemm_mode": [_i],
    "sdxl_debug_act_checksums": [_vp, _P(C.c_ulonglong), _i, _P(_i), _i],
    "sdxl_op_exchange_shadow": [_vp, _sz, _i, _i, _f, _vp],
    "sdxl_op_gemm_ld": [_i, _vp, _vp, _vp, _i, _i, _i, C.c_long, C.c_long, C.c_long, _vp, _vp, C.c_long, _i, _vp],
    "sdxl_op_linear_dgrad_delta": [_vp, _vp, _vp, _vp, _vp, _vp, _i, _i, _i, _i, _vp],
    "sdxl_op_sampler_step": [_vp, _vp, _vp, _i, _i, _i, _P(SamplerStep), _vp],
    "sdxl_debug_cond_operands": [_vp, _i, _i, _P(_i), _P(_sz), _P(_l), _P(_sz), _P(_l), _P(_i)],
    "sdxl_op_cond_dgrad": [_i, _P(_vp), _P(_l), _P(_vp), _P(_l), _P(_i), _vp, _l, _i, _i, _vp],
    "sdxl_op_lora_merge": [_vp, _vp, _vp, _vp, _i, _i, _i, _f, _vp],
    "sdxl_op_lora_project": [_vp, _vp, _vp, _vp, _vp, _i, _i, _i, _f, _vp],
    "sdxl_op_lora_merge_layout": [_vp, _vp, _vp, _vp, _i, _i, _i, _f, _i, _i, _i, _vp],
    "sdxl_op_lora_project_layout": [_vp, _vp, _vp, _vp, _vp, _i, _i, _i, _f, _i, _i, _i, _vp],
    "sdxl_op_lora_grad": [_vp, _l, _vp, _l, _vp, _vp, _vp, _vp, _i, _i, _i, _i, _f, _i, _vp],
    "sdxl_debug_gemm_route": [_P(_i), _P(_i)],
}
GEMM_DESC_FIELDS = ("form", "taps", "M", "N", "K", "splitk", "group", "cfg", "geglu", "geglu_group", "Hm", "Wm", "Hs", "Ws", "sm", "sd", "up2", "emit_bf16", "delta", "bias_grad")
GEMM_ROUTE_FIELDS = ("kernel", "cfg", "fast", "post")
GEMM_KERNELS = ("128-row", "256x256", "cr256", "pipelined", "wgrad256", "conv_wgrad3", "stream-K")
GEMM_POSTS = ("none", "splitk_reduce", "splitk_epilogue")


def gemm_route(**problem) -> dict:
    d = dict(dict.fromkeys(GEMM_DESC_FIELDS, 0), taps=1, splitk=1, group=1, sm=1, sd=1)
    assert set(problem) <= set(d), set(problem) - set(d)
    d.update(problem)
    out = (_i * len(GEMM_ROUTE_FIELDS))()
    check(load().sdxl_debug_gemm_route((_i * len(GEMM_DESC_FIELDS))(*[int(d[k]) for k in GEMM_DESC_FIELDS]), out), "sdxl_debug_gemm_route")
    r = dict(zip(GEMM_ROUTE_FIELDS, out))
    return dict(r, kernel=GEMM_KERNELS[r["kernel"]], post=GEMM_POSTS[r["post"]], fast=bool(r["fast"]))


DIAG_SIGNATURES = {
    "sdxl_op_linear_dgrad_ln_bwd": [_vp, _vp, _vp, _P(_f), _vp, _vp, _vp, _vp, _P(_f), _i, _i, _i, _vp],
    "sdxl_set_knob": [_i, _i],
    "sdxl_set_sk_mode": [_i, _i],
    "sdxl_sk_error": [_vp, _P(C.c_uint)],
    "sdxl_ln_error": [_P(C.c_uint)],
    "sdxl_op_pl_prefetch_b": [_i, _vp, _i, _i, _i, C.c_long, _i, _vp],
    "sdxl_op_gemm_sk": [_i, _P(_i), _P(_vp), _P(_vp), _P(_vp), _P(_i), _P(_i), _P(_i), _P(_vp), _P(_vp), _P(_i), _vp],
    "sdxl_op_conv3x3_s2_fwd": [_vp, _vp, _vp, _vp, _vp, _i, _i, _i, _i, _i, _vp],
    "sdxl_op_conv3x3_s2_wgrad": [_vp, _vp, _vp, _vp, _i, _i, _i, _i, _i, _i, _i, _vp],
}

_lib = None


def load() -> C.CDLL:
    global _lib
    if _lib is not None:
        return _lib
    if not LIB_PATH.exists():
        raise SdxlError(f"{LIB_PATH} is missing -- build it with `python {HERE / 'build.py'}{' --diag' if DIAG else ''}` "
                        "(there is no PyTorch/CPU fallback for the training step)")
    lib = C.CDLL(str(LIB_PATH))
    lib.sdxl_last_error.restype = C.c_char_p
    lib.sdxl_last_error.argtypes = []
    sigs = dict(SIGNATURES)
    sigs.update(TEST_HOOK_SIGNATURES)
    if DIAG:
        sigs.update(DIAG_SIGNATURES)
    for name, args in sigs.items():
        fn = getattr(lib, name)
        fn.argtypes = args
        fn.restype = C.c_int
    _lib = lib
    if DIAG:
# ... 17 lines not shown
```

Baseline: 38.07 images/sec.

## Fold LayerNorm backward row sums into attention dQ epilogue for cross-attn to_q

Precomputes per-layer fold vectors (W·gamma and W·beta+bias) on the side stream at the start of backward. The cross-attention dQ kernel then emits per-row partial dot products of dQ with q and those fold vectors, so the to_q dgrad GEMM can finish the LayerNorm backward in its epilogue without a separate row-reduction pass over dy. The aim is to remove the extra memory traffic and kernel work of the norm2 LayerNorm backward. In exchange it adds a fold kernel, a new dQ kernel variant with extra LDS and registers at lower occupancy, a row-sum buffer, and a cross-stream event dependency.

Result: no change. 38.23 images/sec (median of 6 runs) (+0.4%).

```diff
diff --git a/include/sdxlstep_diag.h b/include/sdxlstep_diag.h
--- a/include/sdxlstep_diag.h
+++ b/include/sdxlstep_diag.h
@@ -15,6 +15,14 @@
                     const void* resid, long ldr, int cfg, void* stream);
 SDXL_API int sdxl_op_linear_dgrad_delta(const void* dy, const void* w, const void* o, const void* addend, void* d_o, float* delta, int B, int Nq,
                                int N, int K, void* stream);
+
+SDXL_API int sdxl_op_ln_fold(const void* w, const void* gamma, const void* beta, const void* bias, float* a, int K, int C, void* stream);
+SDXL_API int sdxl_op_attention_bwd_rowsums(const void* q, const void* k, const void* v, const void* o, const void* d_o, const float* lse, float* delta,
+                                  void* dq, void* dk, void* dv, const float* a, float* rs, int B, int heads, int Nq, int Nk, long ldq, long ldk,
+                                  long ldv, long ldo, void* stream);
+SDXL_API int sdxl_op_linear_dgrad_ln_rowsums(const void* dz, const void* w, const float* rs, int nparts, const void* x, const float* stats,
+                                    const void* gamma, const void* addend, void* dx, float* dgamma, float* dbeta, int M, int C, int K,
+                                    void* stream);
 
 SDXL_API int sdxl_op_sampler_step(float* x, const void* pred, void* x_in, int B, int H, int W, const sdxl_sampler_step* s, void* stream);
 
diff --git a/sdxl-training-improvements_amd/csrc/attention.hip b/sdxl-training-improvements_amd/csrc/attention.hip
--- a/sdxl-training-improvements_amd/csrc/attention.hip
+++ b/sdxl-training-improvements_amd/csrc/attention.hip
@@ -235,8 +235,9 @@
 #endif
 }
 
-template <bool WRITE_DELTA>
-__device__ __forceinline__ void attn_bwd_dq_body(const AttnP& p, bf16* sm, const int bx, const int bh) {
+constexpr int DQ_RS_LDS = 2 * HD * 4;
+template <bool WRITE_DELTA, bool RS = false>
+__device__ __forceinline__ void attn_bwd_dq_body(const AttnP& p, bf16* sm, const int bx, const int bh, char* rsl = nullptr) {
   const int tid = threadIdx.x, lane = tid & 63, wave = __builtin_amdgcn_readfirstlane(tid >> 6), l16 = lane & 15, g = lane >> 4;
   const int b = bh / p.H, h = bh - b * p.H;
   const int q0 = bx * 128 + wave * 32;
@@ -272,6 +273,21 @@
 #pragma unroll
     for (int j = 0; j < 2; ++j) dq[i][j] = (f32x4){0.f, 0.f, 0.f, 0.f};
   const float c = SCALE * LOG2E;
+  float* rs_av = (float*)rsl;
+  bf16x4 rqv[RS ? 2 : 1][RS ? 4 : 1];
+  if constexpr (RS) {
+#pragma unroll
+    for (int qb = 0; qb < 2; ++qb) {
+      const int q = q0 + qb * 16 + l16;
+      const int qc = q < p.Nq ? q : p.Nq - 1;
+#pragma unroll
+      for (int db = 0; db < 4; ++db) rqv[qb][db] = *(const bf16x4*)(Qb + (long)qc * p.ldq + db * 16 + g * 4);
+    }
+    if (tid < 32) {
+      const int half = tid >> 4, v = tid & 15;
+      *(f32x4*)(rs_av + half * HD + v * 4) = *(const f32x4*)(p.rs_a + (long)half * p.H * HD + h * HD + v * 4);
+    }
+  }
 #pragma unroll
   for (int qb = 0; qb < 2; ++qb) { qf[qb][0] = scale8(qf[qb][0], c); qf[qb][1] = scale8(qf[qb][1], c); }
 
@@ -350,9 +366,18 @@
   const int nfull = p.Nk / 64;
   for (int t = 0; t < nfull; ++t) tile(t, std::false_type{});
   if (nfull < ntiles) tile(nfull, std::true_type{});
+  f32x4 ra1[RS ? 4 : 1], ra2[RS ? 4 : 1];
+  if constexpr (RS) {
+#pragma unroll
+    for (int db = 0; db < 4; ++db) {
+      ra1[db] = *(const f32x4*)(rs_av + db * 16 + g * 4);
+      ra2[db] = *(const f32x4*)(rs_av + HD + db * 16 + g * 4);
+    }
+  }
 #pragma unroll
   for (int qb = 0; qb < 2; ++qb) {
     int q = q0 + qb * 16 + l16;
+    float rq = 0.f, r1 = 0.f, r2 = 0.f;
     if (q < p.Nq) {
       bf16* row = p.dQ + ((long)b * p.Nq + q) * p.lddq + h * HD;
 #pragma unroll
@@ -361,7 +386,15 @@
         o[0] = (bf16)(dq[db][qb][0] * SCALE); o[1] = (bf16)(dq[db][qb][1] * SCALE);
         o[2] = (bf16)(dq[db][qb][2] * SCALE); o[3] = (bf16)(dq[db][qb][3] * SCALE);
         *(bf16x4*)(row + db * 16 + g * 4) = o;
-      }
+        if constexpr (RS) {
+#pragma unroll
+          for (int e = 0; e < 4; ++e) { const float d = (float)o[e]; rq += d * (float)rqv[qb][db][e]; r1 += d * ra1[db][e]; r2 += d * ra2[db][e]; }
+        }
+      }
+    }
+    if constexpr (RS) {
+      rq = sum_over_g(rq); r1 = sum_over_g(r1); r2 = sum_over_g(r2);
+      if (q < p.Nq && g == 0) *(f32x4*)(p.rs_out + (((long)b * p.Nq + q) * p.H + h) * 4) = (f32x4){rq, r1, r2, 0.f};
     }
   }
 }
@@ -372,6 +405,14 @@
   int qblk, bh;
   attn_xcd_map(p, blockIdx.x, (p.Nq + 127) >> 7, qblk, bh);
   attn_bwd_dq_body<true>(p, sm, qblk, bh);
+}
+__global__ __launch_bounds__(256, 2) void attn_bwd_dq_rs_kernel(const AttnP p) {
+  set_wave_prio(p.prio);
+  __shared__ __attribute__((aligned(16))) bf16 sm[4 * TILE_ELEMS];
+  int qblk, bh;
+  attn_xcd_map(p, blockIdx.x, (p.Nq + 127) >> 7, qblk, bh);
+  __shared__ __attribute__((aligned(16))) char rsl[DQ_RS_LDS];
+  attn_bwd_dq_body<true, true>(p, sm, qblk, bh, rsl);
 }
 
 template <int KB>
@@ -666,6 +707,10 @@
   if (FILE* f = launch_log()) { fprintf(f, "A,1,%d,%d,%d,%d\n", p.B, p.H, p.Nq, p.Nk); fflush(f); }
   AttnP q = p;
   q.xcd = (p.B * p.H) % 8 == 0 && KNOB(32) != 1;
+  if (p.rs_out) {
+    ARG_CHECK(p.rs_a && (((uintptr_t)p.rs_a | (uintptr_t)p.rs_out) & 15) == 0 && p.ldq % 4 == 0, "attention dQ: row-sum output needs its fold vectors, 16-byte aligned");
+    hipLaunchKernelGGL(attn_bwd_dq_rs_kernel, dim3(cdiv(p.Nq, 128) * p.B * p.H), dim3(256), 0, st, q);
+  } else
   hipLaunchKernelGGL(attn_bwd_dq_kernel, dim3(cdiv(p.Nq, 128) * p.B * p.H), dim3(256), 0, st, q);
   HIP_CHECK_RET(hipGetLastError());
   return 0;
diff --git a/sdxl-training-improvements_amd/csrc/capi.hip b/sdxl-training-improvements_amd/csrc/capi.hip
--- a/sdxl-training-improvements_amd/csrc/capi.hip
+++ b/sdxl-training-improvements_amd/csrc/capi.hip
@@ -51,6 +51,7 @@
     HIP_CHECK_RET(hipEventCreateWithFlags(&h->e.ev_join, hipEventDisableTiming | hipEventDisableSystemFence));
     HIP_CHECK_RET(hipEventCreateWithFlags(&h->e.ev_seg, hipEventDisableTiming | hipEventDisableSystemFence));
     HIP_CHECK_RET(hipEventCreateWithFlags(&h->e.ev_hoist, hipEventDisableTiming | hipEventDisableSystemFence));
+    HIP_CHECK_RET(hipEventCreateWithFlags(&h->e.ev_fold, hipEventDisableTiming | hipEventDisableSystemFence));
   }
   *out = h;
   return 0;
@@ -69,6 +70,7 @@
   if (h->e.ev_join) (void)hipEventDestroy(h->e.ev_join);
   if (h->e.ev_seg) (void)hipEventDestroy(h->e.ev_seg);
   if (h->e.ev_hoist) (void)hipEventDestroy(h->e.ev_hoist);
+  if (h->e.ev_fold) (void)hipEventDestroy(h->e.ev_fold);
   if (h->e.side) (void)hipStreamDestroy(h->e.side);
   if (h->e.small_ranges_dev) (void)hipFree(h->e.small_ranges_dev);
   if (h->lora.dev) (void)hipFree(h->lora.dev);
@@ -630,6 +632,7 @@
     HIP_CHECK_RET(hipMemsetAsync(p.F(p.ln_part_off), 0, p.ln_part_floats * sizeof(float), st));
     p.ln_epoch = 0;
   }
+  if (k == 0) CHK(e.launch_folds(p, st));
   for (int i = p.seg_last_op[s]; i >= p.seg_first_op[s] && i >= 0; --i) CHK(p.ops[i]->bwd(p, st, first));
   CHK(e.flush_wgrads(p, st));
   CHK(e.flush_ln_params(p, st));
diff --git a/sdxl-training-improvements_amd/csrc/engine.h b/sdxl-training-improvements_amd/csrc/engine.h
--- a/sdxl-training-improvements_amd/csrc/engine.h
+++ b/sdxl-training-improvements_amd/csrc/engine.h
@@ -76,6 +76,9 @@
   size_t apart_side_off = NONE, apart_side_floats = 0;
   size_t ln_part_off = NONE, ln_part_floats = 0;
   int ln_epoch = 0;
+  struct FoldSrc { PRef w, gm, bt, bias; size_t a_off = NONE; int K = 0, C = 0; };
+  std::vector<FoldSrc> folds;
+  size_t rs_off = NONE, rs_floats = 0;
   struct CondSrc { size_t dy_off = NONE; long lda = 0; PRef w; long ldb = 0; int K = 0; };
   CondSrc cond_kv[2], cond_add;
   int cond_nkv = 0;
@@ -131,6 +134,10 @@
   std::vector<LnRedEntry> ln_pending;
   std::vector<LnRedEntry> cs_pending;
   int flush_ln_params(Plan& p, hipStream_t main);
+  hipEvent_t ev_fold = nullptr;
+  bool fold_wait = false;
+  int launch_folds(Plan& p, hipStream_t main);
+  int fold_ready(hipStream_t main);
   void drop_pending() { side_leaves.clear(); wg_pending.clear(); ln_pending.clear(); cs_pending.clear(); }
   bool side_dirty = false;
   bool cond_ehs = false, cond_pool = false;
diff --git a/sdxl-training-improvements_amd/csrc/engine.hip b/sdxl-training-improvements_amd/csrc/engine.hip
--- a/sdxl-training-improvements_amd/csrc/engine.hip
+++ b/sdxl-training-improvements_amd/csrc/engine.hip
@@ -132,6 +132,32 @@
     CHK(on_side(p, main, [&b](hipStream_t s2) -> int { return launch_ln_param_reduce(b, s2); }));
   }
   ln_pending.clear();
+  return 0;
+}
+int Engine::launch_folds(Plan& p, hipStream_t main) {
+  fold_wait = false;
+  if (p.folds.empty() || (KNOB(26) & 16)) return 0;
+  size_t i = 0;
+  while (i < p.folds.size()) {
+    LnFoldBatch b;
+    b.n = 0;
+    while (i < p.folds.size() && b.n < LN_FOLD_MAX) {
+      const Plan::FoldSrc& f = p.folds[i++];
+      LnFoldEntry& en = b.e[b.n++];
+      en.w = Wp(f.w); en.gamma = Wp(f.gm); en.beta = Wp(f.bt); en.bias = f.bias.off == NONE ? nullptr : Wp(f.bias);
+      en.a = p.F(f.a_off); en.ldw = f.C; en.K = f.K; en.C = f.C;
+    }
+    CHK(on_side(p, main, [&b](hipStream_t s2) -> int { return launch_ln_fold(b, s2); }));
+  }
+  if (use_side && side && !gemm_profiling()) {
+    HIP_CHECK_RET(hipEventRecord(ev_fold, side));
+    fold_wait = true;
+  }
+  return 0;
+}
+int Engine::fold_ready(hipStream_t main) {
+  if (fold_wait) HIP_CHECK_RET(hipStreamWaitEvent(main, ev_fold, 0));
+  fold_wait = false;
   return 0;
 }
 int Engine::launch_cond_grads(Plan& p, hipStream_t st) {
@@ -206,6 +232,10 @@
 struct LayerNormOp;
 static bool ln_fuse_plan(LayerNormOp* ln, Plan& p, int mode);
 static void ln_fuse_target(LayerNormOp* ln, Plan& p, GemmP& g, int mode);
+struct LinearOp;
+static bool ln_rs_plan(LayerNormOp* ln, LinearOp* by, Plan& p, PRef* gm, PRef* bt);
+static void ln_rs_target(LayerNormOp* ln, Plan& p, GemmP& g, int nparts);
+static bool attn_rs_plan(AttnOp* a, LinearOp* to, int N);
 struct LinearOp : Op {
   Act *x, *y, *resid;
   PRef w, b;
@@ -215,6 +245,11 @@
   bool delta_on = false;
   struct LayerNormOp* ln_src = nullptr;
   int ln_mode = 0;
+  struct AttnOp* rs_attn = nullptr;
+  bool rs_on = false;
+  size_t rs_a_off = NONE;
+  PRef rs_gm, rs_bt;
+  bool rs_live(const Plan& p) const { return rs_on && !(KNOB(26) & 16) && !p.eng->frozen(rs_gm, rs_bt); }
   int crcfg = 0, crsplit = 1;
   int fsplit = 1, dsplit = 1;
   size_t dy32_off = NONE;
@@ -260,9 +295,24 @@
         delta_on = attn_delta_wanted(delta_attn) && dsplit <= 1 && K % 128 == 0;
         attn_set_delta_fused(delta_attn, delta_on);
       }
-      if (SDXL_LN_EPILOGUE && ln_src && KNOB(26) != 0 && dsplit == 1 && dx.addend == NONE && !x->parent && gemm_ln_cfg((int)x->rows, K, N) &&
-          ln_fuse_plan(ln_src, p, KNOB(26) == 2 ? 2 : 1))
-        ln_mode = KNOB(26) == 2 ? 2 : 1;
+      if (rs_attn && ln_src && dsplit == 1 && dx.addend == NONE && !x->parent && !y->parent && !p.eng->lora_op(w) && KNOB(6) <= 0 &&
+          gemm_ln_rowsums_ok((int)x->rows, K, N)) {
+        alignas(16) static float word[4];
+        GemmP g = linear_dgrad_problem((const bf16*)word, y->ld(), (const bf16*)word, word, x->ld(), (int)x->rows, K, N, nullptr, x->ld());
+        GemmRoute r;
+        if (gemm_route_checked(g, &r) == 0 && r.kernel == GEMM_KPL && attn_rs_plan(rs_attn, this, N) && ln_rs_plan(ln_src, this, p, &rs_gm, &rs_bt)) {
+          rs_on = true;
+          rs_a_off = p.alloc(sizeof(float) * 2 * N);
+          Plan::FoldSrc f;
+          f.w = w; f.gm = rs_gm; f.bt = rs_bt; f.bias = b; f.a_off = rs_a_off; f.K = N; f.C = K;
+          p.folds.push_back(f);
+          const size_t rf = (size_t)x->rows * (N / 64) * 4;
+          if (rf > p.rs_floats) p.rs_floats = rf;
+        }
+      }
+      if (SDXL_LN_EPILOGUE && !rs_on && ln_src && (KNOB(26) & 3) != 0 && dsplit == 1 && dx.addend == NONE && !x->parent && gemm_ln_cfg((int)x->rows, K, N) &&
+          ln_fuse_plan(ln_src, p, (KNOB(26) & 3) == 2 ? 2 : 1))
+        ln_mode = (KNOB(26) & 3) == 2 ? 2 : 1;
     }
   }
   int bwd(Plan& p, hipStream_t st, bool first) override {
@@ -327,6 +377,7 @@
       if (KNOB(22) > 0 && gu) g.cfg = KNOB(22);
       if (delta_on) attn_delta_target(delta_attn, p, g);
       if (ln_mode) ln_fuse_target(ln_src, p, g, ln_mode);
+      if (rs_live(p)) ln_rs_target(ln_src, p, g, N / 64);
       CHK(launch_gemm(g, st));
     }
     return 0;
@@ -518,6 +569,7 @@
   size_t dy_off = NONE;
   Plan::GradDst dx;
   int fused = 0;
+  LinearOp* rs_by = nullptr;
   LayerNormOp(Plan& p, Act* x_, Act* y_, PRef g_, PRef b_, int C_, float eps_) : x(x_), y(y_), gm(g_), bt(b_), C(C_), eps(eps_) {
     stats_off = p.alloc(sizeof(float) * x->rows * 2);
   }
@@ -533,9 +585,10 @@
   }
   int bwd(Plan& p, hipStream_t st, bool) override {
     const bool frozen = p.eng->frozen(gm, bt);
-    if (fused) {
+    const int fz = fused == 3 ? (rs_by->rs_live(p) ? 1 : 0) : fused;
+    if (fz) {
       if (frozen) return 0;
-      if (fused == 2) {
+      if (fz == 2) {
         const bf16* xp = p.P(x); const bf16* dyp = p.GP(dy_off); const float* sp = p.F(stats_off);
         float* dg = p.eng->Gp(gm); float* db = p.eng->Gp(bt); const int Mr = (int)x->rows, Cc = C;
         return side_leaf(p, st, [=](hipStream_t s2) -> int { return launch_layernorm_param_grads(xp, dyp, sp, dg, db, Mr, Cc, s2); });
@@ -584,6 +637,20 @@
   gemm_attach_ln_bwd(g, p.P(ln->x), ln->x->ld(), p.F(ln->stats_off), p.eng->Wp(ln->gm), p.GP(ln->dx.out), p.GP(ln->dx.addend), p.F(p.ln_part_off),
                      ++p.ln_epoch, mode == 1 ? p.F(ln->part_off) : nullptr);
   if (mode == 1) g.C = nullptr;
+}
+
+static bool ln_rs_plan(LayerNormOp* ln, LinearOp* by, Plan& p, PRef* gm, PRef* bt) {
+  const int M = (int)ln->x->rows, C = ln->C;
+  if (ln->x->ld() != C || ln->y->ld() != C || ln->fused) return false;
+  if (gemm_ln_pcol_floats(M, C) > layernorm_bwd_part_floats(M, C)) return false;
+  ln->fused = 3;
+  ln->rs_by = by;
+  *gm = ln->gm; *bt = ln->bt;
+  return true;
+}
+static void ln_rs_target(LayerNormOp* ln, Plan& p, GemmP& g, int nparts) {
+  gemm_attach_ln_rowsums(g, p.F(p.rs_off), nparts, p.P(ln->x), ln->x->ld(), p.F(ln->stats_off), p.eng->Wp(ln->gm), p.GP(ln->dx.out), p.GP(ln->dx.addend),
+                         ln->x->ld(), p.F(ln->part_off));
 }
 
 struct AttnOp : Op {
@@ -643,6 +710,7 @@
     if (!self) { dkv = p.grad_dst(kv); if (dkv.addend != NONE) bad = true; }
   }
   bool delta_fused = false;
+  LinearOp* rs_to = nullptr;
   int bwd(Plan& p, hipStream_t st, bool) override {
     if (bad) { sdxl_set_error("attention: operand gradient has another writer"); return 3; }
     if (KNOB(27) & (self ? 16 : 8)) return 0;
@@ -650,6 +718,11 @@
     fill(p, a, true);
     a.prio = KNOB(1);
     a.delta_ready = delta_fused ? 1 : 0;
+    if (rs_to && rs_to->rs_live(p)) {
+      CHK(p.eng->fold_ready(st));
+      a.rs_a = p.F(rs_to->rs_a_off);
+      a.rs_out = p.F(p.rs_off);
+    }
     if (self) return launch_attn_bwd(a, st);
     CHK(launch_attn_bwd_dq(a, st));
     return side_leaf(p, st, [=](hipStream_t s2) -> int { return launch_attn_bwd_dkv(a, s2); });
@@ -658,6 +731,11 @@
 
 static bool attn_delta_wanted(const AttnOp* a) { return a->self && a->qsplit <= 1 && a->Nk >= 256 && a->C % 128 == 0 && a->delta_fused; }
 static void attn_set_delta_fused(AttnOp* a, bool on) { a->delta_fused = on; }
+static bool attn_rs_plan(AttnOp* a, LinearOp* to, int N) {
+  if (a->self || a->bad || a->C != N || a->heads * 64 != N || a->q->parent || a->q->ld() != N) return false;
+  a->rs_to = to;
+  return true;
+}
 static void attn_delta_target(AttnOp* a, Plan& p, GemmP& g) {
   gemm_attach_delta(g, p.P(a->o), a->o->ld(), p.F(a->delta_off), a->Nq, a->heads);
 }
@@ -898,13 +976,16 @@
     Act* x1 = linear(b + ".attn1.to_out.0", a1, C, C, true, x, false, 0, &o1);
     if (sa && o1 && KNOB(21) != 1 && C % 128 == 0 && (x->rows / 128) * (C / 160) <= 256 && sa->qsplit <= 1) { sa->delta_fused = true; o1->delta_attn = sa; }
     Act* l2 = layernorm(b + ".norm2", x1, C);
-    Act* q = linear(b + ".attn2.to_q", l2, C, C, false, nullptr);
+    LinearOp* toq = nullptr;
+    Act* q = linear(b + ".attn2.to_q", l2, C, C, false, nullptr, false, 0, &toq);
     Act* kv = pl ? pl->view(kv_all.at(C), kv_col.at(b), 2 * C) : nullptr;
     (void)cross;
     Act* a2 = nullptr;
     if (pl) {
       a2 = pl->new_act(x->rows, C);
-      tagseg(pl->add<AttnOp>(*pl, q, kv, a2, B, heads, N, ctx, C, false), PRef())->needs_hoisted = true;
+      AttnOp* xa = tagseg(pl->add<AttnOp>(*pl, q, kv, a2, B, heads, N, ctx, C, false), PRef());
+      xa->needs_hoisted = true;
+      if (toq && e.cfg.head_dim == 64) toq->rs_attn = xa;
     }
     Act* x2 = linear(b + ".attn2.to_out.0", a2, C, C, true, x1);
     Act* l3 = layernorm(b + ".norm3", x2, C);
@@ -1113,6 +1194,7 @@
     plan->slab_main_off = plan->alloc(sizeof(float) * (plan->slab_main_floats ? plan->slab_main_floats : 4));
     plan->apart_off = plan->alloc(sizeof(float) * (plan->apart_floats ? plan->apart_floats : 4));
     plan->apart_side_off = plan->alloc(sizeof(float) * (plan->apart_side_floats ? plan->apart_side_floats : 4));
+    if (plan->rs_floats) plan->rs_off = plan->alloc(sizeof(float) * plan->rs_floats);
     plan->ln_part_off = plan->alloc(sizeof(float) * (plan->ln_part_floats ? plan->ln_part_floats : 4));
     plan->in_sw_off = plan->alloc(sizeof(float) * plan->B);
     plan->in_hc_off = plan->alloc(sizeof(float) * plan->B);
diff --git a/sdxl-training-improvements_amd/csrc/gemm.hip b/sdxl-training-improvements_amd/csrc/gemm.hip
--- a/sdxl-training-improvements_amd/csrc/gemm.hip
+++ b/sdxl-training-improvements_amd/csrc/gemm.hip
@@ -1386,6 +1386,13 @@
   g.ln_part = part; g.ln_epoch = epoch; g.ln_pcol = pcol;
   g.cfg = 0; g.resid = nullptr;
 }
+void gemm_attach_ln_rowsums(GemmP& g, const float* part, int nparts, const bf16* x, long ldx, const float* stats, const bf16* gamma, bf16* dx,
+                            const bf16* addend, long ldo, float* pcol) {
+  g.rs_part = part; g.rs_nparts = nparts; g.rs_x = x; g.rs_ldx = ldx; g.rs_stats = stats; g.rs_gamma = gamma;
+  g.rs_dx = dx; g.rs_addend = addend; g.rs_ldo = ldo; g.rs_pcol = pcol;
+  g.C = nullptr; g.resid = nullptr;
+}
+bool gemm_ln_rowsums_ok(int M, int N, int K) { return M > 0 && N % 160 == 0 && K % 64 == 0; }
 void gemm_fill_group(GemmP& g, const GemmP* v, int n) {
   g.group = n;
   for (int i = 0; i < n; ++i) { g.gA[i] = v[i].A; g.gB[i] = v[i].B; g.gC[i] = (float*)v[i].C; g.gbias_grad[i] = v[i].bias_grad; g.gCb[i] = v[i].Cb; }
@@ -1592,6 +1599,7 @@
   if (int e = gemm_check(p)) return e;
   const GemmRoute r = gemm_route(p);
   const bool conv = p.taps != 1;
+  ARG_CHECK(!p.rs_part || r.kernel == GEMM_KPL, "gemm: the LayerNorm row-sum epilogue needs the pipelined kernel (%dx%dx%d routes to kernel %d)", p.M, p.N, p.K, r.kernel);
   int rc;
   switch (r.kernel) {
     case GEMM_KPL: return launch_pl(p, 0, st, r.cfg == 8);
diff --git a/sdxl-training-improvements_amd/csrc/gemm_pl.hip b/sdxl-training-improvements_amd/csrc/gemm_pl.hip
--- a/sdxl-training-improvements_amd/csrc/gemm_pl.hip
+++ b/sdxl-training-improvements_amd/csrc/gemm_pl.hip
@@ -50,8 +50,8 @@
 __device__ __forceinline__ void pl_static_for(F&& f) { pl_static_for_impl(f, std::make_integer_sequence<int, N>{}); }
 
 constexpr int PL_PF_LEAD = 10;
-template <int FORM, int BN, bool PF>
-__global__ __launch_bounds__(PF ? 320 : 256, 2) void pl_kernel(const GemmP p) {
+template <int FORM, int BN, bool PF, bool RS>
+__device__ __forceinline__ void pl_body(const GemmP& p) {
   using G = PlGeom<BN>;
   constexpr bool B_KC = FORM == GEMM_NT;
   constexpr int NJ = G::NJ, MI = G::MI, NL = G::NL, NP0 = G::NP0, NMF = G::NMF;
@@ -113,6 +113,21 @@
     return;
   }
 
+  constexpr int RS_NP = 20;
+  f32x4 rsv[RS ? RS_NP : 1];
+  float rs_mean = 0.f, rs_rstd = 0.f, rs_s1 = 0.f, rs_s2 = 0.f;
+  const f32x4* rs_row = nullptr;
+  if constexpr (RS) {
+    static_assert(FORM == GEMM_NN && BN == 160 && !PF, "row-sum epilogue: NN, 160-column tiles");
+    const int row = m0 + wm * 64 + lane;
+    const int rr = row < M ? row : M - 1;
+    rs_row = (const f32x4*)p.rs_part + (long)rr * p.rs_nparts;
+#pragma unroll
+    for (int u = 0; u < RS_NP; ++u) rsv[u] = u < p.rs_nparts ? rs_row[u] : (f32x4){0.f, 0.f, 0.f, 0.f};
+    rs_mean = p.rs_stats[2 * (long)rr];
+    rs_rstd = p.rs_stats[2 * (long)rr + 1];
+  }
+
   const i32x4 ra = make_srd(p.A, 0x7FFFFFFFu), rb = make_srd(p.B, 0x7FFFFFFFu);
   const unsigned lds_w = lds_addr_of(smem) + (unsigned)wave * 1024u;
   unsigned voA[G::ACH], voB[G::BCH];
@@ -249,6 +264,17 @@
   {
     const RAddr rad = raddr(0u, std::integral_constant<int, 0>{});
     pl_static_for<NITEM>([&](auto IT) { read_item(rad, f0, IT); });
+  }
+  if constexpr (RS) {
+    __builtin_amdgcn_sched_barrier(0);
+    float d = 0.f, e = 0.f;
+#pragma unroll
+    for (int u = 0; u < RS_NP; ++u) { e += rsv[u][1]; d += rsv[u][0] - rsv[u][2]; }
+    for (int q = RS_NP; q < p.rs_nparts; ++q) { const f32x4 v = rs_row[q]; e += v[1]; d += v[0] - v[2]; }
+    const float inv = 1.f / (float)N;
+    rs_s1 = e * inv;
+    rs_s2 = d * inv;
+    __builtin_amdgcn_sched_barrier(0);
   }
   int rd = 0, wr = PL_S - 1;
   auto kstep = [&](auto LIVE) {
@@ -273,6 +299,112 @@
   const int mrow = m0 + wm * 64 + l16;
   const int ncol8 = n0 + wn * (BN / 2) + (g & 1) * 16 + (g >> 1) * 8;
   const int ncol4 = n0 + wn * (BN / 2) + (NJ - 1) * 16 + g * 4;
+  if constexpr (RS) {
+    bf16x8 x8[MI][NP], a8[MI][NP], g8[NP];
+    bf16x4 x4[MI], a4[MI], g4;
+    bf16x4 z4; z4[0] = z4[1] = z4[2] = z4[3] = (bf16)0.f;
+    const bool has_add = p.rs_addend != nullptr;
+#pragma unroll
+    for (int i = 0; i < MI; ++i) {
+      const int m = mrow + 16 * i;
+#pragma unroll
+      for (int jp = 0; jp < NP; ++jp) {
+        const int n = ncol8 + 32 * jp;
+        const bool ok = m < M && n < N;
+        x8[i][jp] = ok ? *(const bf16x8*)(p.rs_x + (long)m * p.rs_ldx + n) : pl_z8();
+        a8[i][jp] = (ok && has_add) ? *(const bf16x8*)(p.rs_addend + (long)m * p.rs_ldo + n) : pl_z8();
+      }
+      const bool ok4 = m < M && ncol4 < N;
+      x4[i] = ok4 ? *(const bf16x4*)(p.rs_x + (long)m * p.rs_ldx + ncol4) : z4;
+      a4[i] = (ok4 && has_add) ? *(const bf16x4*)(p.rs_addend + (long)m * p.rs_ldo + ncol4) : z4;
+    }
+#pragma unroll
+    for (int jp = 0; jp < NP; ++jp) {
+      const int n = ncol8 + 32 * jp;
+      g8[jp] = n < N ? *(const bf16x8*)(p.rs_gamma + n) : pl_z8();
+    }
+    g4 = ncol4 < N ? *(const bf16x4*)(p.rs_gamma + ncol4) : z4;
+    wait_vmcnt<0>();
+    asm volatile("s_waitcnt lgkmcnt(0)" ::: "memory");
+    __builtin_amdgcn_s_barrier();
+    asm volatile("s_nop 7\n\ts_nop 7\n\ts_nop 7" ::: "memory");
+    float cg8[NP][8], cb8[NP][8], cg4[4], cb4[4];
+#pragma unroll
+    for (int jp = 0; jp < NP; ++jp)
+#pragma unroll
+      for (int e = 0; e < 8; ++e) { cg8[jp][e] = 0.f; cb8[jp][e] = 0.f; }
+#pragma unroll
+    for (int e = 0; e < 4; ++e) { cg4[e] = 0.f; cb4[e] = 0.f; }
+#pragma unroll
+    for (int i = 0; i < MI; ++i) {
+      const int m = mrow + 16 * i;
+      const int src = 16 * i + l16;
+      const float mean = __shfl(rs_mean, src), rstd = __shfl(rs_rstd, src), s1 = __shfl(rs_s1, src), s2 = __shfl(rs_s2, src);
+#pragma unroll
+      for (int jp = 0; jp < NP; ++jp) {
+        const int j = 2 * jp;
+        float dy[8];
+#pragma unroll
+        for (int r = 0; r < 4; ++r) {
+          float lo = acc[i][j][r], hi = acc[i][j + 1][r];
+          asm volatile("s_nop 1\n\tv_permlane16_swap_b32 %0, %1" : "+v"(lo), "+v"(hi));
+          dy[r] = lo;
+          dy[4 + r] = hi;
+        }
+        const int n = ncol8 + 32 * jp;
+        bf16x8 o;
+#pragma unroll
+        for (int e = 0; e < 8; ++e) {
+          const float xh = ((float)x8[i][jp][e] - mean) * rstd;
+          cg8[jp][e] += dy[e] * xh;
+          cb8[jp][e] += dy[e];
+          o[e] = (bf16)(rstd * (dy[e] * (float)g8[jp][e] - s1 - xh * s2) + (float)a8[i][jp][e]);
+        }
+        if (m < M && n < N) *(bf16x8*)(p.rs_dx + (long)m * p.rs_ldo + n) = o;
+      }
+      {
+        bf16x4 o;
+#pragma unroll
+        for (int e = 0; e < 4; ++e) {
+          const float dy = acc[i][NJ - 1][e];
+          const float xh = ((float)x4[i][e] - mean) * rstd;
+          cg4[e] += dy * xh;
+          cb4[e] += dy;
+          o[e] = (bf16)(rstd * (dy * (float)g4[e] - s1 - xh * s2) + (float)a4[i][e]);
+        }
+        if (m < M && ncol4 < N) *(bf16x4*)(p.rs_dx + (long)m * p.rs_ldo + ncol4) = o;
+      }
+    }
+    float* red = (float*)smem;
+    constexpr int NV = NP * 8 + 4;
+#pragma unroll
+    for (int jp = 0; jp < NP; ++jp)
+#pragma unroll
+      for (int e = 0; e < 8; ++e) { red[(jp * 8 + e) * 256 + tid] = cg8[jp][e]; red[(NV + jp * 8 + e) * 256 + tid] = cb8[jp][e]; }
+#pragma unroll
+    for (int e = 0; e < 4; ++e) { red[(NP * 8 + e) * 256 + tid] = cg4[e]; red[(NV + NP * 8 + e) * 256 + tid] = cb4[e]; }
+    __syncthreads();
+    if (tid < BN) {
+      const int cwn = tid / (BN / 2), c = tid - cwn * (BN / 2);
+      int v, cgp;
+      if (c < 32 * NP) { const int jp = c >> 5, r = c & 31; cgp = (r >> 4) + 2 * ((r >> 3) & 1); v = jp * 8 + (r & 7); }
+      else { const int c2 = c - 32 * NP; cgp = c2 >> 2; v = NP * 8 + (c2 & 3); }
+      float sg = 0.f, sb = 0.f;
+#pragma unroll
+      for (int w2 = 0; w2 < 2; ++w2) {
+        const float* rg = red + v * 256 + (w2 * 2 + cwn) * 64 + cgp * 16;
+        const float* rbp = rg + NV * 256;
+#pragma unroll
+        for (int l = 0; l < 16; ++l) { sg += rg[l]; sb += rbp[l]; }
+      }
+      const int n = n0 + tid;
+      if (n < N) {
+        p.rs_pcol[((long)by * 2) * N + n] = sg;
+        p.rs_pcol[((long)by * 2 + 1) * N + n] = sb;
+      }
+    }
+    return;
+  }
   bf16x8 res8[MI][NP], bias8[NP];
   bf16x4 res4[MI], bias4;
   const bool has_res = p.resid != nullptr, has_bias = p.bias != nullptr;
@@ -354,6 +486,24 @@
       }
     }
   }
+}
+
+template <int FORM, int BN, bool PF>
+__global__ __launch_bounds__(PF ? 320 : 256, 2) void pl_kernel(const GemmP p) {
+  pl_body<FORM, BN, PF, false>(p);
+}
+__global__ __launch_bounds__(256, 2) void pl_rs_kernel(const GemmP p) { pl_body<GEMM_NN, 160, false, true>(p); }
+
+int launch_pl_rs(const GemmP& p, hipStream_t st) {
+  static bool attr_set = false;
+  if (!attr_set) {
+    HIP_CHECK_RET(hipFuncSetAttribute((const void*)pl_rs_kernel, hipFuncAttributeMaxDynamicSharedMemorySize, PlGeom<160>::SMEM));
+    attr_set = true;
+  }
+  dim3 grid(cdiv(p.N, 160), cdiv(p.M, PL_BM), 1);
+  GEMM_LAUNCH(pl_rs_kernel, grid, dim3(256), PlGeom<160>::SMEM, st, p);
+  HIP_CHECK_RET(hipGetLastError());
+  return 0;
 }
 
 template <int FORM, int BN, bool PF>
@@ -437,6 +587,13 @@
   }
 #endif
   (void)prefetch;
+  if (p.rs_part) {
+    ARG_CHECK(p.form == GEMM_NN && bn == 160 && p.N % 160 == 0 && !p.bias && !p.resid && !p.C, "gemm_pl: row-sum epilogue: NN, N %% 160 == 0, no bias / residual / C (form %d N=%d)", p.form, p.N);
+    ARG_CHECK(p.rs_nparts > 0 && p.rs_x && p.rs_stats && p.rs_gamma && p.rs_dx && p.rs_pcol && p.rs_ldx % 8 == 0 && p.rs_ldo % 8 == 0 &&
+              (((uintptr_t)p.rs_part | (uintptr_t)p.rs_x | (uintptr_t)p.rs_dx | (uintptr_t)p.rs_addend | (uintptr_t)p.rs_gamma) & 15) == 0,
+              "gemm_pl: row-sum epilogue: missing or misaligned buffers");
+    return launch_pl_rs(p, st);
+  }
   if (p.form == GEMM_NT) return bn == 160 ? launch_pl_k<GEMM_NT, 160, false>(p, st) : launch_pl_k<GEMM_NT, 128, false>(p, st);
   return bn == 160 ? launch_pl_k<GEMM_NN, 160, false>(p, st) : launch_pl_k<GEMM_NN, 128, false>(p, st);
 }
diff --git a/sdxl-training-improvements_amd/csrc/hooks.hip b/sdxl-training-improvements_amd/csrc/hooks.hip
--- a/sdxl-training-improvements_amd/csrc/hooks.hip
+++ b/sdxl-training-improvements_amd/csrc/hooks.hip
@@ -367,6 +367,43 @@
   gemm_attach_delta(g, (const bf16*)o, N, delta, Nq, N / 64);
   return launch_gemm(g, (hipStream_t)st);
 }
+int sdxl_op_ln_fold(const void* w, const void* gamma, const void* beta, const void* bias, float* a, int K, int C, void* st) {
+  LnFoldBatch b;
+  b.n = 1;
+  b.e[0].w = (const bf16*)w; b.e[0].gamma = (const bf16*)gamma; b.e[0].beta = (const bf16*)beta; b.e[0].bias = (const bf16*)bias;
+  b.e[0].a = a; b.e[0].ldw = C; b.e[0].K = K; b.e[0].C = C;
+  return launch_ln_fold(b, (hipStream_t)st);
+}
+int sdxl_op_attention_bwd_rowsums(const void* q, const void* k, const void* v, const void* o, const void* d_o, const float* lse, float* delta,
+                                  void* dq, void* dk, void* dv, const float* a, float* rs, int B, int heads, int Nq, int Nk, long ldq, long ldk,
+                                  long ldv, long ldo, void* st) {
+  ARG_CHECK(a && rs, "attention_bwd_rowsums: fold vectors and row-sum output");
+  AttnP p;
+  memset(&p, 0, sizeof(p));
+  p.Q = (const bf16*)q; p.K = (const bf16*)k; p.V = (const bf16*)v; p.O = (bf16*)o; p.LSE = (float*)lse;
+  p.B = B; p.H = heads; p.Nq = Nq; p.Nk = Nk; p.ldq = ldq; p.ldk = ldk; p.ldv = ldv; p.ldo = ldo;
+  p.dO = (const bf16*)d_o; p.lddo = ldo; p.Delta = delta;
+  p.dQ = (bf16*)dq; p.dK = (bf16*)dk; p.dV = (bf16*)dv; p.lddq = ldq; p.lddk = ldk; p.lddv = ldv;
+  p.qsplit = attn_pick_qsplit(B, heads, Nq, Nk);
+  if (p.qsplit > 1) CHK(hook_floats(attn_part_floats(B, heads, Nk, p.qsplit), &p.part));
+  p.rs_a = a; p.rs_out = rs;
+  CHK(launch_attn_bwd_dq(p, (hipStream_t)st));
+  return launch_attn_bwd_dkv(p, (hipStream_t)st);
+}
+int sdxl_op_linear_dgrad_ln_rowsums(const void* dz, const void* w, const float* rs, int nparts, const void* x, const float* stats,
+                                    const void* gamma, const void* addend, void* dx, float* dgamma, float* dbeta, int M, int C, int K, void* st) {
+  ARG_CHECK(gemm_ln_rowsums_ok(M, C, K) && dgamma && dbeta, "linear_dgrad_ln_rowsums: M=%d C=%d K=%d does not fit the row-sum epilogue", M, C, K);
+  LnRedBatch b;
+  b.n = 1;
+  float* part;
+  CHK(hook_floats(gemm_ln_pcol_floats(M, C), &part));
+  GemmP g = linear_dgrad_problem((const bf16*)dz, K, (const bf16*)w, nullptr, C, M, C, K, nullptr, C);
+  gemm_attach_ln_rowsums(g, rs, nparts, (const bf16*)x, C, stats, (const bf16*)gamma, (bf16*)dx, (const bf16*)addend, C, part);
+  g.cfg = 7;
+  CHK(launch_gemm(g, (hipStream_t)st));
+  b.e[0].part = part; b.e[0].dgamma = dgamma; b.e[0].dbeta = dbeta; b.e[0].C = C; b.e[0].nblk = gemm_ln_rowblocks(M);
+  return launch_ln_param_reduce(b, (hipStream_t)st);
+}
 int sdxl_debug_gemm_route(const sdxl_gemm_desc* d, sdxl_gemm_route* out) {
   ARG_CHECK(d && out, "gemm_route: null argument");
   alignas(16) static float word[4];
diff --git a/sdxl-training-improvements_amd/csrc/kernels.h b/sdxl-training-improvements_amd/csrc/kernels.h
--- a/sdxl-training-improvements_amd/csrc/kernels.h
+++ b/sdxl-training-improvements_amd/csrc/kernels.h
@@ -69,6 +69,16 @@
   float* ln_part;
   int ln_epoch;
   float* ln_pcol;
+  const float* rs_part;
+  int rs_nparts;
+  const bf16* rs_x;
+  long rs_ldx;
+  const float* rs_stats;
+  const bf16* rs_gamma;
+  bf16* rs_dx;
+  const bf16* rs_addend;
+  long rs_ldo;
+  float* rs_pcol;
   int xcd_px;
   int xcd_bh;
   int tail_n0;
@@ -123,6 +133,9 @@
 void gemm_attach_delta(GemmP& g, const bf16* o, long ldo, float* delta, int nq, int heads);
 void gemm_attach_ln_bwd(GemmP& g, const bf16* x, long ldx, const float* stats, const bf16* gamma, bf16* dx, const bf16* addend, float* part, int epoch,
                         float* pcol);
+void gemm_attach_ln_rowsums(GemmP& g, const float* part, int nparts, const bf16* x, long ldx, const float* stats, const bf16* gamma, bf16* dx,
+                            const bf16* addend, long ldo, float* pcol);
+bool gemm_ln_rowsums_ok(int M, int N, int K);
 void gemm_fill_group(GemmP& g, const GemmP* v, int n);
 int launch_gemm256(const GemmP& p, hipStream_t st);
 void gemm256_set_tail(bool on);
@@ -180,6 +193,8 @@
   int prio;
   int delta_ready;
   int xcd;
+  const float* rs_a;
+  float* rs_out;
 };
 size_t attn_part_floats(int B, int H, int Nk, int qsplit);
 int attn_pick_qsplit(int B, int H, int Nq, int Nk);
@@ -213,6 +228,10 @@
 struct LnRedEntry { const float* part; float* dgamma; float* dbeta; int nblk, C; };
 struct LnRedBatch { LnRedEntry e[LN_RED_MAX]; int n; };
 int launch_ln_param_reduce(const LnRedBatch& b, hipStream_t st);
+#define LN_FOLD_MAX 48
+struct LnFoldEntry { const bf16* w; const bf16* gamma; const bf16* beta; const bf16* bias; float* a; long ldw; int K, C; };
+struct LnFoldBatch { LnFoldEntry e[LN_FOLD_MAX]; int n; };
+int launch_ln_fold(const LnFoldBatch& b, hipStream_t st);
 
 int launch_silu_fwd(const bf16* x, bf16* y, long n, hipStream_t st);
 int launch_silu_bwd(const bf16* x, const bf16* dy, bf16* dx, const bf16* addend, long n, hipStream_t st);
diff --git a/sdxl-training-improvements_amd/csrc/norm.hip b/sdxl-training-improvements_amd/csrc/norm.hip
--- a/sdxl-training-improvements_amd/csrc/norm.hip
+++ b/sdxl-training-improvements_amd/csrc/norm.hip
@@ -809,6 +809,39 @@
   return 0;
 }
 
+__global__ __launch_bounds__(256) void ln_fold_kernel(const LnFoldBatch b) {
+  const LnFoldEntry e = b.e[blockIdx.y];
+  const int lane = threadIdx.x & 63, k = blockIdx.x * 4 + (threadIdx.x >> 6);
+  if (k >= e.K) return;
+  const bf16* wr = e.w + (long)k * e.ldw;
+  float s1 = 0.f, s2 = 0.f;
+  for (int c = lane * 8; c < e.C; c += 512) {
+    const bf16x8 w = *(const bf16x8*)(wr + c), gm = *(const bf16x8*)(e.gamma + c), bt = *(const bf16x8*)(e.beta + c);
+#pragma unroll
+    for (int i = 0; i < 8; ++i) { s1 += (float)w[i] * (float)gm[i]; s2 += (float)w[i] * (float)bt[i]; }
+  }
+  s1 = wave_sum(s1);
+  s2 = wave_sum(s2);
+  if (lane == 0) {
+    e.a[k] = s1;
+    e.a[e.K + k] = (e.bias ? (float)e.bias[k] : 0.f) + s2;
+  }
+}
+int launch_ln_fold(const LnFoldBatch& b, hipStream_t st) {
+  if (b.n <= 0) return 0;
+  ARG_CHECK(b.n <= LN_FOLD_MAX, "ln_fold: %d entries", b.n);
+  int kmax = 0;
+  for (int i = 0; i < b.n; ++i) {
+    const LnFoldEntry& e = b.e[i];
+    ARG_CHECK(e.w && e.gamma && e.beta && e.a && e.K > 0 && e.C > 0 && e.C % 8 == 0 && e.ldw % 8 == 0 &&
+              (((uintptr_t)e.w | (uintptr_t)e.gamma | (uintptr_t)e.beta) & 15) == 0, "ln_fold: entry %d: K=%d C=%d ldw=%ld, 16-byte aligned operands", i, e.K, e.C, e.ldw);
+    kmax = e.K > kmax ? e.K : kmax;
+  }
+  hipLaunchKernelGGL(ln_fold_kernel, dim3(cdiv(kmax, 4), b.n), dim3(256), 0, st, b);
+  HIP_CHECK_RET(hipGetLastError());
+  return 0;
+}
+
 int launch_layernorm_param_grads(const bf16* x, const bf16* dy, const float* stats, float* dgamma, float* dbeta, int M, int C, hipStream_t st) {
   ARG_CHECK(C % 8 == 0, "layernorm param grads: C=%d must be a multiple of 8", C);
   dim3 g2; int rpc;
diff --git a/sdxl-training-improvements_amd/lib.py b/sdxl-training-improvements_amd/lib.py
--- a/sdxl-training-improvements_amd/lib.py
+++ b/sdxl-training-improvements_amd/lib.py
@@ -183,6 +183,9 @@
     "sdxl_op_lora_merge_layout": [_vp, _vp, _vp, _vp, _i, _i, _i, _f, _i, _i, _i, _vp],
     "sdxl_op_lora_project_layout": [_vp, _vp, _vp, _vp, _vp, _i, _i, _i, _f, _i, _i, _i, _vp],
     "sdxl_op_lora_grad": [_vp, _l, _vp, _l, _vp, _vp, _vp, _vp, _i, _i, _i, _i, _f, _i, _vp],
+    "sdxl_op_ln_fold": [_vp, _vp, _vp, _vp, _vp, _i, _i, _vp],
+    "sdxl_op_attention_bwd_rowsums": [_vp, _vp, _vp, _vp, _vp, _vp, _vp, _vp, _vp, _vp, _vp, _vp, _i, _i, _i, _i, _l, _l, _l, _l, _vp],
+    "sdxl_op_linear_dgrad_ln_rowsums": [_vp, _vp, _vp, _i, _vp, _vp, _vp, _vp, _vp, _vp, _vp, _i, _i, _i, _vp],
     "sdxl_debug_gemm_route": [_P(_i), _P(_i)],
 }
 GEMM_DESC_FIELDS = ("form", "taps", "M", "N", "K", "splitk", "group", "cfg", "geglu", "geglu_group", "Hm", "Wm", "Hs", "Ws", "sm", "sd", "up2", "emit_bf16", "delta", "bias_grad")
```
